# argsim/argsim

Hardware: AMD Instinct MI355X
Metric: sentences/sec per ELBO step (higher is better)
Workload: dtype f32; 1 GPU; BASELINE configs[1]: 1xMI355X fp32, latent_dim 128, vocab 8k, seq_len 64, batch 256 per GPU; FULL synthetic Zipf batches, dim_emb 512, 3 layers, step 20000; global_batch=256, seq_len=64, parallelism=dp1, gru=persistent

## Files before the change

### argsim_amd/csrc/ctx.h

```cpp
#pragma once
#include "../../include/argsim_vae.h"
#include "kernels.h"

#include <fcntl.h>
#include <sys/file.h>
#include <unistd.h>

#include <algorithm>
#include <cmath>
#include <cstdio>
#include <cstring>
#include <initializer_list>
#include <string>
#include <vector>

#pragma GCC visibility push(hidden)
namespace avae { namespace host {

struct ParamEntry {
    std::string name;
    int64_t offset;
    int ndim;
    int64_t shape[4];
    int g16;
    int bucket;
};

struct GruP { int64_t W, R, bW, bR; };

}}
#pragma GCC visibility pop

struct avae_ctx {
    avae_config cfg{};
    int device = 0;
    hipStream_t stream = nullptr;
    std::string err;
    std::vector<avae::host::ParamEntry> params;
    int64_t numel = 0;
    std::vector<std::pair<int64_t, int64_t>> buckets;
    float *P = nullptr, *G = nullptr, *M = nullptr, *Vv = nullptr;
    int64_t step = 0;
    avae_grad_hook hook = nullptr; void* hook_user = nullptr;
    std::vector<int> hook_pending;
    int persistent = 1;
    bool first_step_checked = false;
    int gru_ablate = 0, gru_force_slow = 0, gru_stagger = 0, gru_item = 2;
    int skinny = 1;
    int score_plan[4] = {0, 0, 0, 0};
    const int* expect_ptr[3] = {nullptr, nullptr, nullptr}; int expect_val[3] = {0, 0, 0};
    int compact = 2;
    int skip_pad = 1;
    int shared_device = 0; int lock_fd = -1;
    int dyn_split = 1;
    int dyn_thin = 1;
    int enc_top1 = 1;
    int table_l1 = 1;
    int bf16_act = 1;
    int bf16_sv = 1;
    int bf16_tn = 1;
    int logits16 = 1;
    int bf16_nt8 = 1;
    int bf16_direct = 0;
    int gru_spec = 2;
    int gru_ring = 1;
    int bwd_rs = 2;
    int knn_chunk = 0;
    int agg_chunk = 0;
    int ward_form = 0;
    int probe_chunk = 0;
    int tsne_chunk = 0;
    int kmeans_chunk = 0;
    int gru_bf16 = 1;
    int64_t oE = 0, oKout = 0, oBout = 0, oWmu = 0, oBmu = 0, oWlv = 0, oBlv = 0, oWex = 0, oBex = 0;
    std::vector<avae::host::GruP> enc;
    std::vector<avae::host::GruP> dec;
    float* losses = nullptr;
    float* acc = nullptr;
    int* errw = nullptr;
    unsigned* counters = nullptr;
    float* scratch = nullptr;
    int64_t scratch_n = 0;
    char* ws = nullptr; size_t ws_cap = 0;
    int B = 0, Ss = 0, St = 0;
    int timing = 0, timing_on = 0;
    unsigned short *bfA = nullptr, *bfB = nullptr; size_t bfA_cap = 0, bfB_cap = 0;
    float* slab = nullptr; size_t slab_floats = 0;
    unsigned short* bfP = nullptr; size_t bfP_cap = 0;
    struct Stamp { hipEvent_t a, b; int cls; double flops; const int* dyn; int dyn_max; };
    std::vector<Stamp> stamps; size_t stamps_used = 0;
    int32_t* hint_dev = nullptr; volatile int32_t* hint_host = nullptr;
    const int32_t *cnt_src = nullptr, *cnt_tgt = nullptr;
};

#pragma GCC visibility push(hidden)
namespace avae { namespace host {

#define AV_CHECK(expr)                                                                              \
    do { hipError_t e_ = (expr); if (e_ != hipSuccess) {                                            \
        char b_[512]; snprintf(b_, sizeof b_, "%s:%d: %s -> %s", __FILE__, __LINE__, #expr, hipGetErrorString(e_)); \
        h->err = b_; return 1; } } while (0)
#define AV_TRY(expr) do { int r_ = (expr); if (r_) return r_; } while (0)

inline int fail(avae_ctx* h, const std::string& m) { h->err = m; return 1; }
inline int check_rows(avae_ctx* h, const char* what, int dim, const char* names, std::initializer_list<const void*> ptrs)
{
    if (dim < 4 || dim > 1024 || (dim & 3)) return fail(h, std::string(what) + ": dim must be a multiple of 4 in [4, 1024]");
    uintptr_t bits = 0;
    for (const void* p : ptrs) bits |= (uintptr_t)p;
    if (bits & 15) return fail(h, std::string(what) + ": " + names + " must be 16-byte aligned");
    return 0;
}

#define AV_GRU(expr)                                                                                                \
    do { hipError_t e_ = (expr);                                                                                    \
         if (e_ == hipErrorCooperativeLaunchTooLarge)                                                               \
             return fail(h, "persistent GRU kernel: its workgroups cannot all be resident on this device at once (occupancy query x CU count < grid); " \
                            "run with avae_set_option(\"persistent\", 0)");                                         \
         if (e_ != hipSuccess) { char b_[512]; snprintf(b_, sizeof b_, "%s:%d: %s -> %s", __FILE__, __LINE__, #expr, hipGetErrorString(e_)); \
             h->err = b_; return 1; } } while (0)

struct DeviceTurn {
    avae_ctx* h; bool held = false;
    explicit DeviceTurn(avae_ctx* h_) : h(h_) {
        if (!h->shared_device || !h->persistent) return;
        if (h->lock_fd < 0) {
            char path[64]; snprintf(path, sizeof path, "/tmp/argsim_vae_dev%d.lock", h->device);
            h->lock_fd = open(path, O_CREAT | O_RDWR, 0666);
        }
        if (h->lock_fd >= 0 && flock(h->lock_fd, LOCK_EX) == 0) held = true;
    }
    ~DeviceTurn() { if (held) { (void)hipStreamSynchronize(h->stream); (void)flock(h->lock_fd, LOCK_UN); } }
};

struct Timed {
    avae_ctx* h; avae_ctx::Stamp* s = nullptr;
    Timed(avae_ctx* h_, int cls, double flops, const int* dyn = nullptr, int dyn_max = 0) : h(h_) {
        if (!h->timing) return;
        if (h->stamps_used == h->stamps.size()) {
            avae_ctx::Stamp n{};
            if (hipEventCreate(&n.a) != hipSuccess || hipEventCreate(&n.b) != hipSuccess) return;
            h->stamps.push_back(n);
        }
        s = &h->stamps[h->stamps_used++];
        s->cls = cls; s->flops = flops; s->dyn = dyn; s->dyn_max = dyn_max;
        (void)hipEventRecord(s->a, h->stream);
    }
    ~Timed() { if (s) (void)hipEventRecord(s->b, h->stream); }
};

struct Ws {
    int32_t *src_tm, *lens_src, *lens_tgt, *lead, *gold, *rank, *cidx, *ntok, *pred;
    float *emb_src, *emb_tgt, *ew, *dew;
    std::vector<float*> e_gi, e_hs, e_sv[2], e_hp[2];
    std::vector<float*> d_gi, d_hd, d_sv, d_hp;
    float *hpick, *mu, *lv, *z, *eps, *kld, *h0;
    float *xlast, *gib, *svb, *dgib, *dghb, *dxl;
    float *hc, *ho, *logits;
    float *loss_samp, *errt_samp;
    float *dho, *dhc, *dhd[2], *dgi_d, *dgh_d, *dh0, *carry, *dh0sum, *dz, *dmu, *dlv, *dhpick;
    float *dhs[2], *dgi_e, *dgh_e, *demb_src, *demb_tgt;
    std::vector<unsigned short*> e_hs16, d_hd16, e_hp16[2], d_hp16;
    std::vector<char> act_e, act_d, acth_e, acth_d;
    std::vector<unsigned short*> x16_e, x16_d;
    const unsigned short* x16_kept_e(int i) const { return x16_valid ? x16_e[i] : nullptr; }
    const unsigned short* x16_kept_d(int i) const { return x16_valid ? x16_d[i] : nullptr; }
    bool x16_valid = false;
    unsigned short *dgi16_d, *dgh16_d, *dgi16_e, *dgh16_e;
    int32_t* scat;
    int32_t *grp_src, *grp_tgt;
    int32_t *tokrow_src, *tokrow_tgt;
    float* xbuf; size_t xbuf_floats;
    int32_t *ord_perm[3], *ord_slens[3]; int ord_T[3], ord_cpj[3]; bool ord_ok[3];
    int32_t *map_src, *nact_src, *nsrc; bool compact;
    int32_t *map_tgt, *nact_tgt, *ntgt; bool compact_d;
    int Bx;
    int bx_enc() const { return compact ? Bx : 0; }
    int bx_dec() const { return compact_d ? Bx : 0; }
};

struct Bump {
    char* base; size_t off = 0;
    template <class T> T* take(size_t n) {
        off = (off + 255) & ~(size_t)255;
        T* p = base ? reinterpret_cast<T*>(base + off) : nullptr;
        off += n * sizeof(T);
        return p;
    }
    template <class T> T* opt(bool on, size_t n) { return on ? take<T>(n) : nullptr; }
};

struct Pair { const float* A; const float* B; float* C; const float* bias; };

struct GemmCall {
    const float* A; int lda; bool a_mc;
    const float* B; int ldb; bool b_nc;
    float* C; int ldc;
    int M, N, K;
    float alpha = 1.f; const float* bias = nullptr; int accumulate = 0;
    const int* dyn = nullptr; int dyn_kind = 0;
    const Pair* pair = nullptr;
    bool wgrad = false;
    bool allow_atomic = false;
    bool rows_are_batch = false;
    int thin = -1, split_k = 0;
    const unsigned short* A16 = nullptr; const unsigned short* B16 = nullptr;
    unsigned short* keep_a16 = nullptr;
    unsigned short* c16 = nullptr;

    GemmCall& scaled(float a) { alpha = a; return *this; }
    GemmCall& biased(const float* b) { bias = b; return *this; }
    GemmCall& plus() { accumulate = 1; return *this; }
    GemmCall& rows(const int* d) { dyn = d; dyn_kind = d ? 1 : 0; return *this; }
    GemmCall& depth(const int* d) { dyn = d; dyn_kind = d ? 2 : 0; return *this; }
    GemmCall& with(const Pair* p) { pair = p; return *this; }
    GemmCall& atomic() { allow_atomic = true; return *this; }
    GemmCall& batch_rows() { rows_are_batch = true; return *this; }
    GemmCall& form(int thin_, int split_k_ = 1) { thin = thin_; split_k = split_k_; return *this; }
    GemmCall& a16(const unsigned short* p) { A16 = p; return *this; }
    GemmCall& b16(const unsigned short* p) { B16 = p; return *this; }
    GemmCall& keep(unsigned short* p) { keep_a16 = p; return *this; }
};
inline GemmCall nt(const float* A, int lda, const float* B, int ldb, float* C, int ldc, int M, int N, int K) { return GemmCall{A, lda, false, B, ldb, false, C, ldc, M, N, K}; }
inline GemmCall nn(const float* A, int lda, const float* B, int ldb, float* C, int ldc, int M, int N, int K) { return GemmCall{A, lda, false, B, ldb, true, C, ldc, M, N, K}; }
inline GemmCall tn_grad(const float* A, int lda, const float* B, int ldb, float* C, int ldc, int M, int N, int K)
{
    GemmCall c{A, lda, true, B, ldb, true, C, ldc, M, N, K};
    c.wgrad = true;
    return c;
}

bool use_table(const avae_ctx* h, int rows, int B);
void layout(avae_ctx* h, Bump& b, Ws& w, int B, int Ss, int St, bool train);
int reserve_ws(avae_ctx* h, size_t need);
inline int reserve_named(avae_ctx* h, size_t need, const char* what)
{
    if (reserve_ws(h, need)) {
        (void)hipGetLastError();
        char b[256]; snprintf(b, sizeof b, "%s: the device cannot give the workspace of %zu bytes this call needs", what, need);
        h->err = b;
        return 1;
    }
    return 0;
}
int get_ws(avae_ctx* h, Ws& w, int B, int Ss, int St, bool train);
int gemm(avae_ctx* h, const GemmCall& c);
int gemm_tn16(avae_ctx* h, const GemmCall& c);
void gru_geometry(int D, int njobs, int B, int* G, int* rpg);
void gru_common(avae_ctx* h, const Ws& w, GruArgs& a, int njobs, int S, int B, int ldg, int ldh, const int32_t* lens, int Bx);
int build_row_orders(avae_ctx* h, Ws& w, int B, int Ss, int T, bool with_dec, bool with_enc = true);
int build_compact_dec(avae_ctx* h, Ws& w, int B, int T);
int run_decoder_rnn(avae_ctx* h, Ws& w, int B, int T, const float* state_in, int64_t state_stride, bool save, const int32_t* ids0 = nullptr, bool compact = false,
                    const int32_t* share_rows = nullptr, int share_n = 0);
int run_logits_ce(avae_ctx* h, Ws& w, int rt, bool train, float inv_n);
int encode_ws(avae_ctx* h, Ws& w, const int32_t* src, int b, int t);
inline PrepArgs prep_from_ws(const Ws& w)
{
    PrepArgs p{};
    p.src_tm = w.src_tm; p.lens_src = w.lens_src; p.lens_tgt = w.lens_tgt; p.lead = w.lead; p.gold = w.gold;
    p.rank = w.rank; p.cidx = w.cidx; p.ntok = w.ntok; p.chunk_counts = w.ntok + 4;
    return p;
}

int grow_scratch(avae_ctx* h, size_t need, const char* what);
int check_gru_err(avae_ctx* h);
int dyn_fraction(avae_ctx* h, const avae_ctx::Stamp& s, std::vector<std::pair<const int*, int>>& seen, double* f);
inline int check_bound(avae_ctx* h)
{
    if (!h->P || !h->G || !h->M || !h->Vv) return fail(h, "state buffers not bound (avae_bind_state)");
    return 0;
}
template <class F> int place_scratch(avae_ctx* h, const char* what, F lay)
{
    Bump probe{nullptr};
    lay(probe);
    AV_TRY(grow_scratch(h, probe.off, what));
    Bump real{reinterpret_cast<char*>(h->scratch)};
    lay(real);
    return 0;
}
template <class F> int place_ws(avae_ctx* h, const char* what, F lay, size_t from = 0)
{
    Bump probe{nullptr, from};
    lay(probe);
    AV_TRY(reserve_named(h, probe.off + 4096, what));
    Bump real{h->ws, from};
    lay(real);
    return 0;
}

bool sample_params(avae_ctx* h, const avae_sample_config* sc, int V, SampleParams* sp);
bool sample_params_p(avae_ctx* h, const avae_sample_p_config* sc, int V, SampleParams* sp, float* top_p);

}}
#pragma GCC visibility pop
```

### argsim_amd/csrc/gemm_f32.hip

```cpp
#include "kernels.h"
#include "mfma_tile.h"
#include <algorithm>
#include <cstdlib>
#include <type_traits>

namespace avae {

constexpr int BK = kTileBK, LDK = kTileLDK;

template <bool XC, int ROWS>
struct FastTile {
    const float* base; long long step, valid; unsigned voff[ROWS / 32];
    __device__ __forceinline__ void init(const float* P, int ld, int x0, int X, int kb, int ke, int tid)
    {
        if (XC) {
            base = P + (size_t)kb * ld + x0; step = (long long)BK * ld; valid = (long long)(ke - kb) * ld - x0;
#pragma unroll
            for (int rep = 0; rep < ROWS / 32; ++rep) { const int f = tid + 256 * rep; voff[rep] = (unsigned)(((f / (ROWS / 4)) * ld + ((f % (ROWS / 4)) << 2)) * 4); }
        } else {
            base = P + (size_t)x0 * ld + kb; step = BK; valid = (long long)(X - x0) * ld - kb;
#pragma unroll
            for (int rep = 0; rep < ROWS / 32; ++rep) { const int f = tid + 256 * rep; voff[rep] = (unsigned)(((f >> 3) * ld + ((f & 7) << 2)) * 4); }
        }
    }
    __device__ __forceinline__ void load(float4 (&r)[ROWS / 32], int it) const
    {
        const long long rem = valid - it * step;
        const unsigned bytes = rem <= 0 ? 0u : (rem >= (1ll << 30) ? 0xFFFFFFFFu : (unsigned)(rem * 4));
        const __amdgpu_buffer_rsrc_t rs = __builtin_amdgcn_make_buffer_rsrc(const_cast<float*>(base + it * step), 0, (int)bytes, 0x00020000);
#pragma unroll
        for (int rep = 0; rep < ROWS / 32; ++rep) {
            const u32x4 v = __builtin_amdgcn_raw_buffer_load_b128(rs, (int)voff[rep], 0, 0);
            r[rep] = make_float4(__uint_as_float(v.x), __uint_as_float(v.y), __uint_as_float(v.z), __uint_as_float(v.w));
        }
    }
};

template <int MODE>
__device__ __forceinline__ void put(float* c, float v)
{
    if (MODE == 2) atomicAdd(c, v);
    else if (MODE == 1) *c += v;
    else *c = v;
}
template <int TM, int TN, int WN, int MODE>
__device__ __forceinline__ void epilogue_full(const GemmArgs& g, const f32x16 (&acc)[TM][TN], int m0, int n0, int wm, int wn, int h, int l31, bool add_bias)
{
    float bv[TN];
#pragma unroll
    for (int j = 0; j < TN; ++j) bv[j] = add_bias ? g.bias[n0 + 32 * (wn * TN + j) + l31] : 0.f;
#pragma unroll
    for (int j = 0; j < TN; ++j) {
        const int col = n0 + 32 * (wn * TN + j) + l31;
#pragma unroll
        for (int i = 0; i < TM; ++i) {
            float* c = g.C + (size_t)(m0 + 32 * (wm * TM + i) + 4 * h) * g.ldc + col;
#pragma unroll
            for (int r = 0; r < 16; ++r)
                put<MODE>(c + (size_t)mfma32_row(r, 0) * g.ldc, g.alpha * acc[i][j][r] + bv[j]);
        }
    }
}
template <int TM, int TN, int WN>
__device__ __forceinline__ void epilogue(const GemmArgs& g, const f32x16 (&acc)[TM][TN], int M, int m0, int n0, int BM, int BN,
                                         int wm, int wn, int h, int l31, bool atomic, bool add_bias)
{
    if (!atomic && m0 + BM <= M && n0 + BN <= g.N) {
        if (g.accumulate) epilogue_full<TM, TN, WN, 1>(g, acc, m0, n0, wm, wn, h, l31, add_bias);
        else epilogue_full<TM, TN, WN, 0>(g, acc, m0, n0, wm, wn, h, l31, add_bias);
        return;
    }
    epilogue_generic<TM, TN>(acc, g.C, g.ldc, M, g.N, m0 + 32 * wm * TM, n0 + 32 * wn * TN, h, l31, g.alpha, add_bias ? g.bias : nullptr,
                             atomic ? kEpiAtomic : (g.accumulate ? kEpiAccumulate : kEpiStore));
}

template <bool A_MC, bool B_NC, int WM, int WN, int TM, int TN, bool FAST = false, bool DB = false>
__global__ __launch_bounds__(256, DB ? 2 : 3) void gemm_f32_kernel(GemmArgs g)
{
    constexpr int BM = 32 * WM * TM, BN = 32 * WN * TN;
    constexpr int kStage = (BM + BN) * LDK;
    __shared__ __attribute__((aligned(16))) float smem[kStage * (DB ? 2 : 1)];
    float* As = smem;
    float* Bs = smem + BM * LDK;

    const int tid = threadIdx.x, lane = tid & 63, wave = tid >> 6;
    const int h = lane >> 5, l31 = lane & 31;
    const int wm = wave / WN, wn = wave % WN;

    if (blockIdx.y) { g.A = g.A2; g.B = g.B2; g.C = g.C2; g.bias = g.bias2; }
    int M = g.M, K = g.K;
    if (g.dyn_kind == 1) M = min(M, *g.dyn);
    if (g.dyn_kind == 2) K = min(K, *g.dyn);

    const int tiles_n = (g.N + BN - 1) / BN;
    const int nblk = ((M + BM - 1) / BM) * tiles_n;
    const int bid = xcd_tile(blockIdx.x, nblk);
    if (bid < 0) return;
    const int tm = bid / tiles_n, tn = bid - tm * tiles_n;
    const int m0 = tm * BM, n0 = tn * BN;
    if (m0 >= M) return;

    int kb = 0, ke = K;
    if (g.split_k > 1) {
        int ktiles = (K + BK - 1) / BK;
        int per = (ktiles + g.split_k - 1) / g.split_k;
        kb = blockIdx.z * per * BK;
        ke = min(K, kb + per * BK);
        if (kb >= ke) return;
    }

    f32x16 acc[TM][TN];
    zero_acc(acc);

    float4 ra[BM / 32], rb[BN / 32];
    FastTile<A_MC, BM> fa; FastTile<B_NC, BN> fb;
    if (FAST) {
        fa.init(g.A, g.lda, m0, M, kb, ke, tid); fb.init(g.B, g.ldb, n0, g.N, kb, ke, tid);
        fa.load(ra, 0); fb.load(rb, 0);
    } else {
        load_tile<A_MC, BM>(ra, g.A, g.lda, m0, M, kb, ke, tid);
        load_tile<B_NC, BN>(rb, g.B, g.ldb, n0, g.N, kb, ke, tid);
    }

    if (DB) {
        store_tile<A_MC, BM>(As, ra, tid);
        store_tile<B_NC, BN>(Bs, rb, tid);
        __syncthreads();
    }
    for (int k0 = kb; k0 < ke; k0 += BK) {
        auto next_loads = [&]() __attribute__((always_inline)) {
            if (k0 + BK < ke) {
                if (FAST) { const int it = (k0 - kb) / BK + 1; fa.load(ra, it); fb.load(rb, it); }
                else {
                    load_tile<A_MC, BM>(ra, g.A, g.lda, m0, M, k0 + BK, ke, tid);
                    load_tile<B_NC, BN>(rb, g.B, g.ldb, n0, g.N, k0 + BK, ke, tid);
                }
            }
        };
        if (!DB) {
            store_tile<A_MC, BM>(As, ra, tid);
            store_tile<B_NC, BN>(Bs, rb, tid);
            next_loads();
            __syncthreads();
        } else next_loads();
        __builtin_amdgcn_s_setprio(1);
#pragma unroll
        for (int q = 0; q < 4; ++q) {
            float a[TM][4], b[TN][4];
#pragma unroll
            for (int t = 0; t < TM; ++t) {
                if (A_MC) {
#pragma unroll
                    for (int e = 0; e < 4; ++e) a[t][e] = As[(8 * q + 4 * h + e) * BM + 32 * (wm * TM + t) + l31];
                } else {
                    float4 v = *reinterpret_cast<const float4*>(As + (32 * (wm * TM + t) + l31) * LDK + 8 * q + 4 * h);
                    a[t][0] = v.x; a[t][1] = v.y; a[t][2] = v.z; a[t][3] = v.w;
                }
            }
#pragma unroll
            for (int t = 0; t < TN; ++t) {
                if (B_NC) {
#pragma unroll
                    for (int e = 0; e < 4; ++e) b[t][e] = Bs[(8 * q + 4 * h + e) * BN + 32 * (wn * TN + t) + l31];
                } else {
                    float4 v = *reinterpret_cast<const float4*>(Bs + (32 * (wn * TN + t) + l31) * LDK + 8 * q + 4 * h);
                    b[t][0] = v.x; b[t][1] = v.y; b[t][2] = v.z; b[t][3] = v.w;
                }
            }
#pragma unroll
            for (int e = 0; e < 4; ++e)
#pragma unroll
                for (int i = 0; i < TM; ++i)
#pragma unroll
                    for (int j = 0; j < TN; ++j)
                        acc[i][j] = __builtin_amdgcn_mfma_f32_32x32x2f32(a[i][e], b[j][e], acc[i][j], 0, 0, 0);
        }
        __builtin_amdgcn_s_setprio(0);
        if (DB) {
            As = (As == smem) ? smem + kStage : smem;
            Bs = As + BM * LDK;
            if (k0 + BK < ke) {
                store_tile<A_MC, BM>(As, ra, tid);
                store_tile<B_NC, BN>(Bs, rb, tid);
            }
        }
        __syncthreads();
    }

    const bool atomic = g.split_k > 1;
    const bool add_bias = g.bias != nullptr && (!atomic || blockIdx.z == 0);
    epilogue<TM, TN, WN>(g, acc, M, m0, n0, BM, BN, wm, wn, h, l31, atomic, add_bias);
}

template <bool A_MC, bool B_NC, bool FAST>
__global__ __launch_bounds__(256, 3) void gemm_f32_persist_kernel(GemmArgs g)
{
    static_assert(FAST, "buffer-load staging only (register budget of three workgroups per CU)");
    constexpr int TM = 2, TN = 2, WN = 2, BM = 128, BN = 128;
    __shared__ __attribute__((aligned(16))) float smem[(BM + BN) * LDK];
    float* As = smem;
    float* Bs = smem + BM * LDK;
    const int tid = threadIdx.x, lane = tid & 63, wave = tid >> 6;
    const int h = lane >> 5, l31 = lane & 31;
    const int wm = wave / WN, wn = wave % WN;

    int M = g.M;
    const int K = g.K;
    if (g.dyn_kind == 1) M = min(M, *g.dyn);
    const int tiles_n = (g.N + BN - 1) / BN;
    const int nblk = ((M + BM - 1) / BM) * tiles_n;
    const int per_xcd = gridDim.x >> 3;
    int run0, run_n;
    xcd_run(blockIdx.x & 7, nblk, run0, run_n);
    int local = blockIdx.x >> 3;
    if (local >= run_n) return;

    float4 ra[BM / 32], rb[BN / 32];
    FastTile<A_MC, BM> fa; FastTile<B_NC, BN> fb;
    auto first_tile = [&](int bid) __attribute__((always_inline)) {
        const int tm = bid / tiles_n, tn = bid - tm * tiles_n;
        if (FAST) {
            fa.init(g.A, g.lda, tm * BM, M, 0, K, tid); fb.init(g.B, g.ldb, tn * BN, g.N, 0, K, tid);
            fa.load(ra, 0); fb.load(rb, 0);
        } else {
            load_tile<A_MC, BM>(ra, g.A, g.lda, tm * BM, M, 0, K, tid);
            load_tile<B_NC, BN>(rb, g.B, g.ldb, tn * BN, g.N, 0, K, tid);
        }
    };
    first_tile(run0 + local);
    for (; local < run_n; local += per_xcd) {
        const int bid = run0 + local;
        const int tm = bid / tiles_n, tn = bid - tm * tiles_n;
        const int m0 = tm * BM, n0 = tn * BN;
        const bool more = local + per_xcd < run_n;
        f32x16 acc[TM][TN];
        zero_acc(acc);
        for (int k0 = 0; k0 < K; k0 += BK) {
            store_tile<A_MC, BM>(As, ra, tid);
            store_tile<B_NC, BN>(Bs, rb, tid);
            if (k0 + BK < K) {
                if (FAST) { const int it = k0 / BK + 1; fa.load(ra, it); fb.load(rb, it); }
                else {
                    load_tile<A_MC, BM>(ra, g.A, g.lda, m0, M, k0 + BK, K, tid);
                    load_tile<B_NC, BN>(rb, g.B, g.ldb, n0, g.N, k0 + BK, K, tid);
                }
            } else if (more) {
                first_tile(bid + per_xcd);
            }
            __syncthreads();
            __builtin_amdgcn_s_setprio(1);
            mfma_ktile<A_MC, B_NC, TM, TN, BM, BN>(acc, As, Bs, wm, wn, h, l31);
            __builtin_amdgcn_s_setprio(0);
            __syncthreads();
        }
        epilogue<TM, TN, WN>(g, acc, M, m0, n0, BM, BN, wm, wn, h, l31, false, g.bias != nullptr);
    }
}

template <bool B_NC>
__global__ __launch_bounds__(512) void gemm_f32_skinny_kernel(GemmArgs g)
{
    __shared__ float red[7][16][64];
    if (blockIdx.y) { g.A = g.A2; g.B = g.B2; g.C = g.C2; g.bias = g.bias2; }
    const int tid = threadIdx.x, lane = tid & 63, wave = tid >> 6, l31 = lane & 31, h = lane >> 5;
    const int tiles_n = (g.N + 31) / 32, tm = blockIdx.x / tiles_n, tn = blockIdx.x - tm * tiles_n;
    const int m0 = tm * 32, n0 = tn * 32;
    const int kchunk = ((g.K + 63) / 64) * 8;
    const int k0 = wave * kchunk, k1 = min(g.K, k0 + kchunk);
    const float* __restrict__ ap = g.A + (size_t)min(m0 + l31, g.M - 1) * g.lda;
    const int bcol = min(n0 + l31, g.N - 1);
    const float* __restrict__ bp = B_NC ? g.B + bcol : g.B + (size_t)bcol * g.ldb;
    f32x16 acc;
#pragma unroll
    for (int r = 0; r < 16; ++r) acc[r] = 0.f;
    for (int kk = k0; kk < k1; kk += 32) {
        float4 a[4], b[4];
#pragma unroll
        for (int u = 0; u < 4; ++u) {
            const int k = kk + 8 * u + 4 * h;
            a[u] = make_float4(0.f, 0.f, 0.f, 0.f); b[u] = make_float4(0.f, 0.f, 0.f, 0.f);
            if (k < k1) {
                a[u] = *reinterpret_cast<const float4*>(ap + k);
                if constexpr (B_NC) {
                    b[u].x = bp[(size_t)k * g.ldb]; b[u].y = bp[(size_t)(k + 1) * g.ldb]; b[u].z = bp[(size_t)(k + 2) * g.ldb]; b[u].w = bp[(size_t)(k + 3) * g.ldb];
                } else b[u] = *reinterpret_cast<const float4*>(bp + k);
            }
        }
#pragma unroll
        for (int u = 0; u < 4; ++u) {
            if (kk + 8 * u >= k1) break;
            acc = __builtin_amdgcn_mfma_f32_32x32x2f32(a[u].x, b[u].x, acc, 0, 0, 0);
            acc = __builtin_amdgcn_mfma_f32_32x32x2f32(a[u].y, b[u].y, acc, 0, 0, 0);
            acc = __builtin_amdgcn_mfma_f32_32x32x2f32(a[u].z, b[u].z, acc, 0, 0, 0);
            acc = __builtin_amdgcn_mfma_f32_32x32x2f32(a[u].w, b[u].w, acc, 0, 0, 0);
        }
    }
    if (wave > 0) {
#pragma unroll
        for (int r = 0; r < 16; ++r) red[wave - 1][r][lane] = acc[r];
    }
    __syncthreads();
    if (wave > 0) return;
    const int col = n0 + l31;
    if (col >= g.N) return;
    const float bv = g.bias ? g.bias[col] : 0.f;
#pragma unroll
    for (int r = 0; r < 16; ++r) {
        float v = acc[r];
#pragma unroll
        for (int w = 0; w < 7; ++w) v += red[w][r][lane];
        const int row = m0 + mfma32_row(r, h);
        if (row >= g.M) continue;
        float* c = g.C + (size_t)row * g.ldc + col;
        v = g.alpha * v + bv;
        if (g.accumulate) *c += v; else *c = v;
    }
}
static bool skinny_ok(bool a_mc, const GemmArgs& g)
{
    return !a_mc && g.split_k <= 1 && g.dyn_kind == 0 && (g.K & 3) == 0 && (g.lda & 3) == 0 && g.K >= 64;
}
static void launch_skinny(hipStream_t st, bool b_nc, const GemmArgs& g, const GemmF32Form& f)
{
    const dim3 grid(f.gx, f.gy, f.gz);
    if (b_nc) hipLaunchKernelGGL(gemm_f32_skinny_kernel<true>, grid, dim3(512), 0, st, g);
    else      hipLaunchKernelGGL(gemm_f32_skinny_kernel<false>, grid, dim3(512), 0, st, g);
}

template <class F>
static void with_layouts(bool a_mc, bool b_nc, F&& f)
{
    if (!a_mc && !b_nc)      f(std::false_type{}, std::false_type{});
    else if (!a_mc && b_nc)  f(std::false_type{}, std::true_type{});
    else if (a_mc && b_nc)   f(std::true_type{}, std::true_type{});
    else                     f(std::true_type{}, std::false_type{});
}

GemmF32Form gemm_f32_form(bool a_mc, bool b_nc, const GemmArgs& g)
{
    GemmF32Form f{-1, false, false, false, 0, 0, 0, hipSuccess};
    if (g.M <= 0 || g.N <= 0) return f;
    f.err = hipErrorInvalidValue;
    if ((g.lda | g.ldb) & 3) return f;
    if (((uintptr_t)g.A | (uintptr_t)g.B | (uintptr_t)g.A2 | (uintptr_t)g.B2) & 15) return f;
    if (!a_mc && (g.K & 3)) return f;
    if (a_mc && (g.M & 3)) return f;
    if (!b_nc && (g.K & 3)) return f;
    if (b_nc && (g.N & 3)) return f;
    if (g.dyn_kind == 2 && (!a_mc || !b_nc || (g.split_k > 1 && g.bias))) return f;
    f.err = hipSuccess;
    if (g.thin == 3 && skinny_ok(a_mc, g) && (b_nc || (g.ldb & 3) == 0)) {
        f.tile = 3; f.gx = ((g.M + 31) / 32) * ((g.N + 31) / 32); f.gy = g.A2 ? 2 : 1; f.gz = 1;
        return f;
    }
    f.tile = g.thin == 2 ? 2 : (g.thin ? 1 : 0);
    const int BM = f.tile == 0 ? 128 : (f.tile == 1 ? 32 : 64), BN = f.tile == 2 ? 64 : 128;
    const int tiles = ((g.M + BM - 1) / BM) * ((g.N + BN - 1) / BN);
    f.gx = tiles; f.gy = g.A2 ? 2 : 1; f.gz = g.split_k > 1 ? g.split_k : 1;
    static const bool allow_fast = !getenv("AVAE_F32_NOFAST");
    const int k_per_wg = g.split_k > 1 ? (g.K + g.split_k - 1) / g.split_k : g.K;
    f.fast = allow_fast && (a_mc ? (g.M % BM == 0) : (g.K % BK == 0 && g.dyn_kind != 2)) &&
             (b_nc ? (g.N % BN == 0) : (g.K % BK == 0 && g.dyn_kind != 2)) && (a_mc || b_nc || k_per_wg >= 1536);
    if (f.tile == 1) return f;
    static const char* ps_env = getenv("AVAE_F32_PERSIST");
    const bool aligned = (a_mc ? (g.M % BM == 0) : (g.K % BK == 0)) && (b_nc ? (g.N % BN == 0) : (g.K % BK == 0));
    const bool persist = (ps_env ? atoi(ps_env) != 0 : true) && allow_fast && aligned && !g.A2 && g.split_k <= 1 && g.dyn_kind != 2 && tiles > 1024;
    if (persist) {
        f.tile = 0; f.fast = true; f.persist = true; f.gx = 768; f.gy = f.gz = 1;
        return f;
    }
    static const char* db_env = getenv("AVAE_F32_DB");
    const int eff_tiles = (g.dyn_kind == 1 && g.dyn_expect > 0) ? std::min(tiles, ((g.dyn_expect + BM - 1) / BM) * ((g.N + BN - 1) / BN)) : (g.dyn_kind == 1 ? 0 : tiles);
    f.db = db_env ? atoi(db_env) != 0 && !g.A2 : (!g.A2 && g.split_k <= 1 && eff_tiles > 768 && tiles <= 1024);
    return f;
}

template <int WM, int WN, int TM, int TN>
static void launch_variant(hipStream_t st, bool a_mc, bool b_nc, const GemmArgs& g, const GemmF32Form& f)
{
    const dim3 grid(f.gx, f.gy, f.gz);
    if constexpr (WM == 2 && WN == 2) {
        if (f.persist) {
            with_layouts(a_mc, b_nc, [&](auto A, auto B) { hipLaunchKernelGGL((gemm_f32_persist_kernel<decltype(A)::value, decltype(B)::value, true>), grid, dim3(256), 0, st, g); });
            return;
        }
        if (f.db) {
            if (f.fast) {
                with_layouts(a_mc, b_nc, [&](auto A, auto B) { hipLaunchKernelGGL((gemm_f32_kernel<decltype(A)::value, decltype(B)::value, WM, WN, TM, TN, true, true>), grid, dim3(256), 0, st, g); });
            } else {
                with_layouts(a_mc, b_nc, [&](auto A, auto B) { hipLaunchKernelGGL((gemm_f32_kernel<decltype(A)::value, decltype(B)::value, WM, WN, TM, TN, false, true>), grid, dim3(256), 0, st, g); });
            }
            return;
        }
    }
    if (f.fast) {
        with_layouts(a_mc, b_nc, [&](auto A, auto B) { hipLaunchKernelGGL((gemm_f32_kernel<decltype(A)::value, decltype(B)::value, WM, WN, TM, TN, true>), grid, dim3(256), 0, st, g); });
        return;
    }
    with_layouts(a_mc, b_nc, [&](auto A, auto B) { hipLaunchKernelGGL((gemm_f32_kernel<decltype(A)::value, decltype(B)::value, WM, WN, TM, TN>), grid, dim3(256), 0, st, g); });
}

hipError_t gemm_f32(hipStream_t st, bool a_mc, bool b_nc, const GemmArgs& g)
{
    const GemmF32Form f = gemm_f32_form(a_mc, b_nc, g);
    if (f.err != hipSuccess) return f.err;
    if (f.tile < 0) return hipSuccess;
    if (f.tile == 3) launch_skinny(st, b_nc, g, f);
    else if (f.persist) launch_variant<2, 2, 2, 2>(st, a_mc, b_nc, g, f);
    else if (f.tile == 2) launch_variant<2, 2, 1, 1>(st, a_mc, b_nc, g, f);
    else if (f.tile == 1) launch_variant<1, 4, 1, 1>(st, a_mc, b_nc, g, f);
    else launch_variant<2, 2, 2, 2>(st, a_mc, b_nc, g, f);
    return hipGetLastError();
}

}
```

### argsim_amd/csrc/handle.cpp

```cpp
#include "ctx.h"

using namespace avae;
using namespace avae::host;

static std::string g_create_err;

namespace avae { namespace host {

int grow_scratch(avae_ctx* h, size_t need, const char* what)
{
    if (h->scratch_n >= (int64_t)need) return 0;
    AV_CHECK(hipStreamSynchronize(h->stream));
    if (h->scratch) AV_CHECK(hipFree(h->scratch));
    h->scratch = nullptr; h->scratch_n = 0;
    if (hipMalloc(reinterpret_cast<void**>(&h->scratch), need) != hipSuccess) {
        (void)hipGetLastError();
        h->scratch = nullptr;
        char b_[256]; snprintf(b_, sizeof b_, "%s: %.0f MB of scratch could not be allocated on the device", what, (double)need / 1048576.0);
        return fail(h, b_);
    }
    h->scratch_n = (int64_t)need;
    return 0;
}

static void add_param(avae_ctx* h, const std::string& name, std::initializer_list<int64_t> shape, int g16, int bucket, int64_t* off_out)
{
    ParamEntry e; e.name = name; e.offset = h->numel; e.ndim = (int)shape.size(); e.g16 = g16; e.bucket = bucket;
    int64_t n = 1; int k = 0;
    for (int i = 0; i < 4; ++i) e.shape[i] = 1;
    for (auto s : shape) { e.shape[k++] = s; n *= s; }
    if (off_out) *off_out = e.offset;
    h->numel += (n + 3) / 4 * 4;
    h->params.push_back(e);
}

static void build_params(avae_ctx* h)
{
    const int64_t D = h->cfg.dim_emb, V = h->cfg.dim_tgt, R = h->cfg.dim_rep; const int L = h->cfg.rnn_layers;
    h->enc.resize(L); h->dec.resize(L);
    auto close_bucket = [&](int64_t start) { h->buckets.push_back({start, h->numel - start}); };
    int bucket = 0; int64_t start = 0;
    add_param(h, "decode/out/kernel", {D, D}, 0, bucket, &h->oKout);
    add_param(h, "decode/out/bias", {D}, 0, bucket, &h->oBout);
    close_bucket(start);
    for (int i = L - 1; i >= 0; --i) {
        ++bucket; start = h->numel;
        std::string p = "decode/rnn/l" + std::to_string(i + 1) + "/";
        add_param(h, p + "W", {3 * D, D}, 1, bucket, &h->dec[i].W);
        add_param(h, p + "R", {3 * D, D}, 1, bucket, &h->dec[i].R);
        add_param(h, p + "bW", {3 * D}, 1, bucket, &h->dec[i].bW);
        add_param(h, p + "bR", {3 * D}, 1, bucket, &h->dec[i].bR);
        close_bucket(start);
    }
    ++bucket; start = h->numel;
    add_param(h, "latent/ex/kernel", {R, D}, 0, bucket, &h->oWex);
    add_param(h, "latent/ex/bias", {D}, 0, bucket, &h->oBex);
    add_param(h, "latent/mu/kernel", {2 * D, R}, 0, bucket, &h->oWmu);
    add_param(h, "latent/mu/bias", {R}, 0, bucket, &h->oBmu);
    add_param(h, "latent/lv/kernel", {2 * D, R}, 0, bucket, &h->oWlv);
    add_param(h, "latent/lv/bias", {R}, 0, bucket, &h->oBlv);
    close_bucket(start);
    for (int i = L - 1; i >= 0; --i) {
        ++bucket; start = h->numel;
        const int64_t In = i == 0 ? D : 2 * D;
        std::string p = "encode/rnn" + std::to_string(i + 1) + "/";
        int64_t o;
        add_param(h, p + "fwd/W", {3 * D, In}, 1, bucket, &h->enc[i].W);
        add_param(h, p + "bwd/W", {3 * D, In}, 1, bucket, &o);
        add_param(h, p + "fwd/R", {3 * D, D}, 1, bucket, &h->enc[i].R);
        add_param(h, p + "bwd/R", {3 * D, D}, 1, bucket, &o);
        add_param(h, p + "fwd/bW", {3 * D}, 1, bucket, &h->enc[i].bW);
        add_param(h, p + "bwd/bW", {3 * D}, 1, bucket, &o);
        add_param(h, p + "fwd/bR", {3 * D}, 1, bucket, &h->enc[i].bR);
        add_param(h, p + "bwd/bR", {3 * D}, 1, bucket, &o);
        close_bucket(start);
    }
    ++bucket; start = h->numel;
    add_param(h, "embed/embedding", {V, D}, 0, bucket, &h->oE);
    close_bucket(start);
}

static const ParamEntry* find_param(avae_ctx* h, const char* name)
{
    for (auto& e : h->params) if (e.name == name) return &e;
    return nullptr;
}

static float* state_buf(avae_ctx* h, int kind)
{
    switch (kind) { case AVAE_PARAM: return h->P; case AVAE_GRAD: return h->G; case AVAE_ADAM_M: return h->M; case AVAE_ADAM_V: return h->Vv; }
    return nullptr;
}

int check_gru_err(avae_ctx* h)
{
    int e = 0;
    AV_CHECK(hipMemcpyAsync(&e, h->errw, sizeof(int), hipMemcpyDeviceToHost, h->stream));
    AV_CHECK(hipStreamSynchronize(h->stream));
    if (e) {
        (void)hipMemsetAsync(h->errw, 0, sizeof(int), h->stream);
        return fail(h, "GRU persistent kernel: an exchange wait timed out -- its workgroups were not all resident at once.  A persistent "
                       "launch needs every CU of the device (one handle = one GPU = one process, include/argsim_vae.h): another process or "
                       "stream computing on this GPU holds CUs the launch is waiting for.  Give the handle the device to itself, or "
                       "run with avae_set_option(\"persistent\", 0) (one launch per time step)");
    }
    return 0;
}
int dyn_fraction(avae_ctx* h, const avae_ctx::Stamp& s, std::vector<std::pair<const int*, int>>& seen, double* f)
{
    *f = 1.0;
    if (!s.dyn || s.dyn_max <= 0) return 0;
    int c = -1;
    for (auto& e : seen) if (e.first == s.dyn) c = e.second;
    if (c < 0) {
        AV_CHECK(hipMemcpy(&c, s.dyn, sizeof(int), hipMemcpyDeviceToHost));
        if (c < 0) c = 0;
        seen.push_back({s.dyn, c});
    }
    *f = (double)std::min(c, s.dyn_max) / (double)s.dyn_max;
    return 0;
}

}}

extern "C" {

int avae_create(const avae_config* cfg, int device, avae_handle* out)
{
    if (!cfg || !out) { g_create_err = "null argument"; return 1; }
    *out = nullptr;
    if (!gru_dim_supported(cfg->dim_emb)) { g_create_err = "dim_emb must be one of 16, 32, 64, 128, 256, 512 (the GRU kernels are instantiated for these widths only; the reference leaves dim_emb free, config.json uses 512)"; return 1; }
    if (cfg->compute_dtype < 0 || cfg->compute_dtype > 2) { g_create_err = "compute_dtype must be 0 (fp32 MFMA), 1 (bf16 GEMM operands) or 2 (fp32 via split bf16 MFMA)"; return 1; }
    if (cfg->dim_rep % 4 || cfg->dim_tgt % 4 || cfg->rnn_layers < 1 || cfg->rnn_layers > 8) { g_create_err = "dim_rep and dim_tgt must be multiples of 4 (16-byte rows); 1 <= rnn_layers <= 8"; return 1; }
    int ndev = 0;
    if (hipGetDeviceCount(&ndev) != hipSuccess || ndev <= 0) { g_create_err = "no HIP device available: the gfx950 kernels cannot run (no CPU fallback)"; return 1; }
    if (device < 0 || device >= ndev) { g_create_err = "bad device index"; return 1; }
    avae_ctx* h = new avae_ctx();
    h->cfg = *cfg; h->device = device;
    if (h->cfg.kl_beta == 0.f) h->cfg.kl_beta = 1.f;
    build_params(h);
    hipError_t e = hipSetDevice(device);
    if (e == hipSuccess) e = hipMalloc(reinterpret_cast<void**>(&h->losses), 64 * sizeof(float));
    if (e == hipSuccess) e = hipMalloc(reinterpret_cast<void**>(&h->errw), 128 * sizeof(int));
    if (e == hipSuccess) e = hipMalloc(reinterpret_cast<void**>(&h->counters), 2048 * sizeof(unsigned));
    if (e == hipSuccess) e = hipMemset(h->losses, 0, 64 * sizeof(float));
    if (e == hipSuccess) e = hipMemset(h->errw, 0, 128 * sizeof(int));
    if (e == hipSuccess) e = hipMemset(h->counters, 0, 2048 * sizeof(unsigned));
    if (e != hipSuccess) { g_create_err = std::string("hip init failed: ") + hipGetErrorString(e); delete h; return 1; }
    h->acc = h->losses + 8;
    *out = h;
    return 0;
}

void avae_destroy(avae_handle h)
{
    if (!h) return;
    (void)hipSetDevice(h->device);
    if (h->stream) (void)hipStreamSynchronize(h->stream); else (void)hipDeviceSynchronize();
    if (h->ws) (void)hipFree(h->ws);
    if (h->losses) (void)hipFree(h->losses);
    if (h->errw) (void)hipFree(h->errw);
    if (h->hint_host) (void)hipHostFree(const_cast<int32_t*>(h->hint_host));
    if (h->counters) (void)hipFree(h->counters);
    if (h->scratch) (void)hipFree(h->scratch);
    if (h->bfA) (void)hipFree(h->bfA);
    if (h->slab) (void)hipFree(h->slab);
    if (h->bfP) (void)hipFree(h->bfP);
    if (h->bfB) (void)hipFree(h->bfB);
    if (h->lock_fd >= 0) (void)close(h->lock_fd);
    delete h;
}

const char* avae_last_error(avae_handle h) { return h ? h->err.c_str() : g_create_err.c_str(); }

int avae_set_stream(avae_handle h, void* s) { if (!h) return 1; h->stream = reinterpret_cast<hipStream_t>(s); return 0; }

int avae_get_dims(avae_handle h, int32_t* V, int32_t* D, int32_t* R, int32_t* L)
{
    if (!h) return 1;
    if (V) *V = h->cfg.dim_tgt; if (D) *D = h->cfg.dim_emb; if (R) *R = h->cfg.dim_rep; if (L) *L = h->cfg.rnn_layers;
    return 0;
}

int64_t avae_state_numel(avae_handle h) { return h ? h->numel : 0; }

int avae_bind_state(avae_handle h, float* p, float* g, float* m, float* v)
{
    if (!h) return 1;
    if (((uintptr_t)p | (uintptr_t)g | (uintptr_t)m | (uintptr_t)v) & 15) return fail(h, "state buffers must be 16-byte aligned");
    h->P = p; h->G = g; h->M = m; h->Vv = v;
    return 0;
}

int avae_param_count(avae_handle h) { return h ? (int)h->params.size() : 0; }
const char* avae_param_name(avae_handle h, int i) { return (h && i >= 0 && i < (int)h->params.size()) ? h->params[i].name.c_str() : nullptr; }

int avae_param_info(avae_handle h, const char* name, int64_t* offset, int32_t* ndim, int64_t shape[4])
{
    if (!h) return 1;
    const ParamEntry* e = find_param(h, name);
    if (!e) return fail(h, std::string("unknown variable: ") + (name ? name : "(null)"));
    if (offset) *offset = e->offset; if (ndim) *ndim = e->ndim;
    if (shape) for (int i = 0; i < 4; ++i) shape[i] = e->shape[i];
    return 0;
}

static int xfer_tensor(avae_handle h, const char* name, int kind, float* buf, bool get)
{
    if (!h) return 1;
    AV_TRY(check_bound(h));
    const ParamEntry* e = find_param(h, name);
    if (!e) return fail(h, std::string("unknown variable: ") + (name ? name : "(null)"));
    float* base = state_buf(h, kind);
    if (!base) return fail(h, "bad tensor kind");
    float* flat = base + e->offset;
    int64_t n = e->shape[0] * e->shape[1] * e->shape[2] * e->shape[3];
    if (!e->g16) {
        AV_CHECK(hipMemcpyAsync(get ? buf : flat, get ? flat : buf, n * sizeof(float), hipMemcpyDeviceToDevice, h->stream));
    } else {
        int D = h->cfg.dim_emb, cols = (int)(e->ndim == 2 ? e->shape[1] : 1);
        if (get) AV_CHECK(g16_permute(h->stream, buf, flat, D, cols, false));
        else     AV_CHECK(g16_permute(h->stream, flat, buf, D, cols, true));
    }
    return 0;
}
int avae_get_tensor(avae_handle h, const char* name, int kind, float* buf) { return xfer_tensor(h, name, kind, buf, true); }
int avae_set_tensor(avae_handle h, const char* name, int kind, const float* buf) { return xfer_tensor(h, name, kind, const_cast<float*>(buf), false); }

int avae_get_step(avae_handle h, int64_t* s) { if (!h || !s) return 1; *s = h->step; return 0; }
int avae_set_step(avae_handle h, int64_t s) { if (!h) return 1; h->step = s; return 0; }

int avae_set_grad_hook(avae_handle h, avae_grad_hook hook, void* user) { if (!h) return 1; h->hook = hook; h->hook_user = user; return 0; }

int avae_set_option(avae_handle h, const char* key, int value)
{
    if (!h || !key) return 1;
    if (!strcmp(key, "persistent")) { h->persistent = value; return 0; }
    if (!strcmp(key, "gru_item")) { h->gru_item = value; return 0; }
    if (!strcmp(key, "gru_stagger")) { h->gru_stagger = value; return 0; }
    if (!strcmp(key, "gru_force_slow")) { h->gru_force_slow = value; return 0; }
    if (!strcmp(key, "gru_bf16")) { h->gru_bf16 = value != 0; return 0; }
    if (!strcmp(key, "bwd_rs")) { h->bwd_rs = value; return 0; }
    if (!strcmp(key, "dyn_split")) { h->dyn_split = value != 0; return 0; }
    if (!strcmp(key, "shared_device")) { h->shared_device = value != 0; return 0; }
    if (!strcmp(key, "gru_spec")) { h->gru_spec = value; return 0; }
    if (!strcmp(key, "gru_ring")) { h->gru_ring = value != 0; return 0; }
    if (!strcmp(key, "bf16_nt8")) { h->bf16_nt8 = value != 0; return 0; }
    if (!strcmp(key, "logits16")) { h->logits16 = value != 0; return 0; }
    if (!strcmp(key, "bf16_direct")) { h->bf16_direct = value != 0; return 0; }
    if (!strcmp(key, "bf16_tn")) { h->bf16_tn = value != 0; return 0; }
    if (!strcmp(key, "bf16_sv")) { h->bf16_sv = value != 0; return 0; }
    if (!strcmp(key, "bf16_act")) { h->bf16_act = value != 0; return 0; }
    if (!strcmp(key, "table_l1")) { h->table_l1 = value != 0; return 0; }
    if (!strcmp(key, "enc_top1")) { h->enc_top1 = value != 0; return 0; }
    if (!strcmp(key, "dyn_thin")) { h->dyn_thin = value != 0; return 0; }
    if (!strcmp(key, "skip_pad")) { h->skip_pad = value != 0; return 0; }
    if (!strcmp(key, "compact")) { h->compact = value; return 0; }
    if (!strcmp(key, "skinny")) { h->skinny = value; return 0; }
    if (!strcmp(key, "knn_chunk")) { if (value < 0) return fail(h, "knn_chunk must be >= 0"); h->knn_chunk = value; return 0; }
    if (!strcmp(key, "agg_chunk")) { if (value < 0) return fail(h, "agg_chunk must be >= 0"); h->agg_chunk = value; return 0; }
    if (!strcmp(key, "ward_form")) { if (value < 0 || value > 2) return fail(h, "ward_form must be 0 (planner), 1 (one-workgroup) or 2 (launch-per-merge)"); h->ward_form = value; return 0; }
    if (!strcmp(key, "probe_chunk")) { if (value < 0) return fail(h, "probe_chunk must be >= 0"); h->probe_chunk = value; return 0; }
    if (!strcmp(key, "kmeans_chunk")) { if (value < 0) return fail(h, "kmeans_chunk must be >= 0"); h->kmeans_chunk = value; return 0; }
    if (!strcmp(key, "tsne_chunk")) { if (value < 0) return fail(h, "tsne_chunk must be >= 0"); h->tsne_chunk = value; return 0; }
    if (!strcmp(key, "gru_ablate")) {
        if (value && !gru_diag_build()) return fail(h, "gru_ablate needs the diagnostic build of libargsim_vae.so (make -C argsim_amd/csrc DIAG=1)");
        h->gru_ablate = value; return 0;
    }
    if (!strcmp(key, "timing")) { h->timing = value; h->timing_on = value; h->stamps_used = 0; return 0; }
    if (!strcmp(key, "timing_pause")) { h->timing = value ? 0 : h->timing_on; return 0; }
    return fail(h, "unknown option");
}
int avae_timing_collect(avae_handle h, double* out)
{
    if (!h || !out) return 1;
    AV_CHECK(hipStreamSynchronize(h->stream));
    for (int i = 0; i < 9; ++i) out[i] = 0.0;
    std::vector<std::pair<const int*, int>> seen;
    for (size_t i = 0; i < h->stamps_used; ++i) {
        float ms = 0.f;
        AV_CHECK(hipEventElapsedTime(&ms, h->stamps[i].a, h->stamps[i].b));
        double f = 1.0;
        AV_TRY(dyn_fraction(h, h->stamps[i], seen, &f));
        int c = h->stamps[i].cls;
        out[3 * c] += ms; out[3 * c + 1] += 1.0; out[3 * c + 2] += h->stamps[i].flops * f;
    }
    h->stamps_used = 0;
    return 0;
}
int avae_bucket_count(avae_handle h) { return h ? (int)h->buckets.size() : 0; }
int avae_bucket_info(avae_handle h, int i, int64_t* offset, int64_t* count)
{
    if (!h || i < 0 || i >= (int)h->buckets.size()) return 1;
    *offset = h->buckets[i].first; *count = h->buckets[i].second; return 0;
}

}
```

### argsim_amd/csrc/hooks.cpp

```cpp
#include "ctx.h"

using namespace avae;
using namespace avae::host;

extern "C" {

int avae_debug_team_batch(int32_t B) { return B > 0 ? gru_team_batch(B) : 0; }
int avae_debug_gemm_plan(const int32_t* in, int32_t n, int32_t* out)
{
    if (!in || !out || n < 0) return 1;
    for (int r = 0; r < n; ++r, in += 19, out += 15) {
        const GemmShape s{in[0] != 0, in[1] != 0, in[2], in[3], in[4], in[5], in[6], in[7], in[8], in[9], in[10], in[11] != 0, in[12] != 0,
                          in[13] != 0, in[14] != 0, in[15], in[16] != 0, in[17] != 0, in[18] != 0};
        const GemmPlan p = gemm_plan(s);
        out[0] = p.n;
        for (int i = 0; i < 2; ++i) {
            const GemmLaunch l = i < p.n ? p.launch[i] : GemmLaunch{0, 0, 0, 0, 0, 0, 0};
            const int32_t f[7] = {l.row0, l.rows, l.thin, l.split_k, l.accumulate, l.zero, l.dyn};
            std::copy(f, f + 7, out + 1 + 7 * i);
        }
    }
    return 0;
}
int avae_debug_gemm_call(avae_handle h, int a_mc, int b_nc, const float* A, const float* Bm, float* Cm, const float* bias, int M, int N, int K,
                         int lda, int ldb, int ldc, float alpha, int accumulate, int flags, const int* count, int expect,
                         const float* A2, const float* B2, float* C2, unsigned short* keep16)
{
    if (!h) return 1;
    GemmCall c{A, lda, a_mc != 0, Bm, ldb, b_nc != 0, Cm, ldc, M, N, K};
    c.alpha = alpha; c.bias = bias; c.accumulate = accumulate; c.keep_a16 = keep16;
    c.allow_atomic = (flags & 1) != 0; c.rows_are_batch = (flags & 2) != 0; c.wgrad = (flags & 4) != 0;
    if (c.wgrad) c.depth(count); else c.rows(count);
    const Pair second{A2, B2, C2, nullptr};
    if (A2) c.pair = &second;
    const int* const was_ptr = h->expect_ptr[0]; const int was_val = h->expect_val[0];
    h->expect_ptr[0] = count; h->expect_val[0] = expect;
    const int r = gemm(h, c);
    h->expect_ptr[0] = was_ptr; h->expect_val[0] = was_val;
    return r;
}
int avae_debug_gemm_forced(avae_handle h, int a_mc, int b_nc, const float* A, const float* Bm, float* Cm, const float* bias, int M, int N, int K,
                           int lda, int ldb, int ldc, float alpha, int accumulate, int thin, int split_k, const int* count, int dyn_kind, int expect,
                           const float* A2, const float* B2, float* C2, const float* bias2)
{
    if (!h) return 1;
    if (thin < 0 || thin > 3 || split_k < 1 || dyn_kind < 0 || dyn_kind > 2 || (dyn_kind != 0) != (count != nullptr))
        return fail(h, "avae_debug_gemm_forced: thin in 0..3, split_k >= 1, dyn_kind in 0..2 with a count exactly where it is not 0");
    GemmCall c{A, lda, a_mc != 0, Bm, ldb, b_nc != 0, Cm, ldc, M, N, K};
    c.alpha = alpha; c.bias = bias; c.accumulate = accumulate;
    if (dyn_kind == 2) c.depth(count); else c.rows(count);
    c.form(thin, split_k);
    const Pair second{A2, B2, C2, bias2};
    if (A2) c.pair = &second;
    const int* const was_ptr = h->expect_ptr[0]; const int was_val = h->expect_val[0];
    h->expect_ptr[0] = count; h->expect_val[0] = expect;
    const int r = gemm(h, c);
    h->expect_ptr[0] = was_ptr; h->expect_val[0] = was_val;
    return r;
}
int avae_debug_gemm_f32_form(int a_mc, int b_nc, int M, int N, int K, int lda, int ldb, int ldc, int accumulate, int thin, int split_k, int dyn_kind,
                             int expect, int pair, int32_t out[8])
{
    if (!out) return 1;
    alignas(16) static const float other[4] = {0.f, 0.f, 0.f, 0.f};
    const GemmArgs g{nullptr, nullptr, nullptr, nullptr, M, N, K, lda, ldb, ldc, 1.f, accumulate, split_k, nullptr, dyn_kind, expect, thin,
                     pair ? other : nullptr, pair ? other : nullptr, nullptr, nullptr};
    const GemmF32Form f = gemm_f32_form(a_mc != 0, b_nc != 0, g);
    const int32_t v[8] = {f.tile, f.fast, f.db, f.persist, (int32_t)f.gx, (int32_t)f.gy, (int32_t)f.gz, f.err != hipSuccess};
    std::copy(v, v + 8, out);
    return 0;
}
int avae_debug_score_plan(avae_handle h, int32_t out[4])
{
    if (!h || !out) return 1;
    for (int i = 0; i < 4; ++i) out[i] = h->score_plan[i];
    return 0;
}
int avae_debug_present_ids(avae_handle h, int32_t out[2])
{
    if (!h || !out) return 1;
    AV_CHECK(hipStreamSynchronize(h->stream));
    out[0] = out[1] = -1;
    if (h->cnt_src) AV_CHECK(hipMemcpy(&out[0], h->cnt_src, sizeof(int), hipMemcpyDeviceToHost));
    if (h->cnt_tgt) AV_CHECK(hipMemcpy(&out[1], h->cnt_tgt, sizeof(int), hipMemcpyDeviceToHost));
    return 0;
}
int avae_debug_train_ce(avae_handle h, float* out, int32_t max_n, int32_t* n_out)
{
    if (!h || !out || !n_out) return 1;
    if (h->B < 1) return fail(h, "avae_debug_train_ce: no training forward has run on this handle");
    Ws w;
    AV_TRY(get_ws(h, w, h->B, h->Ss, h->St, true));
    int n = 0;
    AV_CHECK(hipMemcpyAsync(&n, w.ntok, sizeof(int), hipMemcpyDeviceToHost, h->stream));
    AV_CHECK(hipStreamSynchronize(h->stream));
    n = std::min(n, (int)max_n);
    AV_CHECK(hipMemcpyAsync(out, w.loss_samp, (size_t)n * sizeof(float), hipMemcpyDeviceToDevice, h->stream));
    *n_out = n;
    return 0;
}
int avae_debug_timing(avae_handle h, double* out, int max_n, int* n)
{
    if (!h || !out || !n) return 1;
    AV_CHECK(hipStreamSynchronize(h->stream));
    *n = (int)std::min<size_t>(h->stamps_used, (size_t)max_n);
    std::vector<std::pair<const int*, int>> seen;
    for (int i = 0; i < *n; ++i) {
        float ms = 0.f;
        AV_CHECK(hipEventElapsedTime(&ms, h->stamps[i].a, h->stamps[i].b));
        double f = 1.0;
        AV_TRY(dyn_fraction(h, h->stamps[i], seen, &f));
        const double fl = h->stamps[i].flops * f;
        out[3 * i] = h->stamps[i].cls; out[3 * i + 1] = ms; out[3 * i + 2] = fl;
    }
    return 0;
}
int avae_debug_stamps(avae_handle h, unsigned long long* out)
{
    if (!h || !out) return 1;
    AV_CHECK(hipStreamSynchronize(h->stream));
    AV_CHECK(hipMemcpy(out, h->errw + 16, 32 * sizeof(unsigned long long), hipMemcpyDeviceToHost));
    AV_CHECK(hipMemset(h->errw + 16, 0, 32 * sizeof(unsigned long long)));
    return 0;
}
int avae_debug_gemm(avae_handle h, int a_mc, int b_nc, const float* A, const float* Bm, float* Cm, const float* bias,
                    int M, int N, int K, int lda, int ldb, int ldc, float alpha, int accumulate, int split_k)
{
    if (!h) return 1;
    GemmCall c{A, lda, a_mc != 0, Bm, ldb, b_nc != 0, Cm, ldc, M, N, K};
    c.alpha = alpha; c.bias = bias; c.accumulate = accumulate;
    return gemm(h, c.form(split_k == -3 ? 3 : (split_k < 0 ? 1 : (split_k >= 1000 ? 2 : 0)), split_k < 0 ? 1 : (split_k >= 1000 ? split_k - 1000 : split_k)));
}
int avae_debug_gemm_dyn(avae_handle h, const float* A, const float* Bm, float* Cm, int M, int N, int K, const int* rows)
{
    if (!h) return 1;
    return gemm(h, nt(A, K, Bm, K, Cm, N, M, N, K).rows(rows).form(0));
}
int avae_debug_gemm_c16(avae_handle h, const float* A, const float* Bm, unsigned short* C16, int M, int N, int K, float alpha, const int* rows)
{
    if (!h) return 1;
    if (h->cfg.compute_dtype != 1 || !gemm_bf16_c16_takes(M, N, K, rows, h->bf16_nt8)) return 3;
    GemmCall c = nt(A, K, Bm, K, nullptr, N, M, N, K).scaled(alpha).rows(rows).form(0);
    c.c16 = C16;
    return gemm(h, c);
}
int avae_debug_gemm_tn16(avae_handle h, const float* A, const float* Bm, float* Cm, int M, int N, int K, int lda, int ldb, int ldc, float alpha)
{
    if (!h) return 1;
    return gemm_tn16(h, tn_grad(A, lda, Bm, ldb, Cm, ldc, M, N, K).scaled(alpha));
}
int avae_debug_softmax_ce(avae_handle h, float* logits, unsigned short* panel, int logits16, const int32_t* gold, const int32_t* cidx,
                          const int32_t* n_dev, int n_max, int V, int write_grad, float inv_n, float* loss_samp, float* errt,
                          int32_t* pred, int* form_out)
{
    if (!h || !form_out) return 1;
    CeArgs c{};
    c.logits = logits; c.gold = gold; c.cidx = cidx; c.n_dev = n_dev; c.n_max = n_max; c.V = V;
    c.write_grad = write_grad; c.inv_n = inv_n;
    c.loss_samp = loss_samp; c.errt_samp = errt; c.pred = pred; c.loss_acc = nullptr;
    c.grad16 = panel; c.logits16 = logits16;
    *form_out = softmax_ce_form(c);
    AV_CHECK(softmax_ce(h->stream, c));
    return 0;
}
int avae_debug_argmax_rows(avae_handle h, const float* logits, int32_t* pred, int n, int V)
{
    if (!h) return 1;
    AV_CHECK(argmax_rows(h->stream, logits, pred, n, V));
    return 0;
}
int avae_debug_op_layout(int64_t n, int64_t V, int64_t out[6])
{
    if (!out || n < 0 || V < 0) return 1;
    int32_t base[1];
    out[0] = (int64_t)embed_scatter_scratch_ints((size_t)n, (size_t)V);
    out[1] = (int64_t)id_groups_ints((size_t)n, (size_t)V);
    out[2] = id_groups_rank(base, (int)n, (int)V) - base;
    out[3] = id_groups_uid(base, (int)n, (int)V) - base;
    out[4] = id_groups_count(base, (int)n, (int)V) - base;
    out[5] = id_groups_supported((int)V) ? 1 : 0;
    return 0;
}
int avae_debug_op(avae_handle h, const char* op, void* const* p, const int64_t* i, const float* f)
{
    if (!h || !op || !p || !i || !f) return 1;
    const std::string o(op);
    hipStream_t st = h->stream;
    auto F = [&](int k) { return static_cast<float*>(p[k]); };
    auto I = [&](int k) { return static_cast<int32_t*>(p[k]); };
    if (o == "prep_ids") {
        PrepArgs a{};
        a.src = I(0); a.tgt = I(1); a.keep_mask = static_cast<const uint8_t*>(p[2]); a.src_tm = I(3); a.lens_src = I(4); a.lens_tgt = I(5);
        a.lead = I(6); a.gold = I(7); a.rank = I(8); a.cidx = I(9); a.ntok = I(10); a.zero2 = F(11); a.chunk_counts = I(12);
        a.B = (int)i[0]; a.Ss = (int)i[1]; a.St = (int)i[2]; a.eos = (int)i[3]; a.bos = (int)i[4]; a.train = (int)i[5]; a.seed = (uint64_t)i[6];
        a.keepwd = f[0];
        AV_CHECK(prep_ids(st, a));
    } else if (o == "embed_gather") AV_CHECK(embed_gather(st, F(0), I(1), F(2), (int)i[0], (int)i[1], (int)i[2]));
    else if (o == "embed_scatter_add2") AV_CHECK(embed_scatter_add2(st, F(0), I(1), F(2), (int)i[0], I(3), F(4), (int)i[1], (int)i[2], (int)i[3], I(5)));
    else if (o == "id_groups_build") AV_CHECK(id_groups_build(st, I(0), (int)i[0], (int)i[1], I(1), i[2] != 0));
    else if (o == "rank_rows") AV_CHECK(rank_rows(st, I(0), I(1), I(2), (int)i[0], (int)i[1]));
    else if (o == "rows_gather_ranked") AV_CHECK(rows_gather_ranked(st, F(0), F(1), I(2), I(3), (int)i[0], (int)i[1], (int)i[2]));
    else if (o == "rows_group_sum") AV_CHECK(rows_group_sum(st, F(0), I(1), F(2), (int)i[0], (int)i[1], (int)i[2], I(3)));
    else if (o == "rows_add_indexed") AV_CHECK(rows_add_indexed(st, F(0), F(1), I(2), I(3), (int)i[0], (int)i[1]));
    else if (o == "rows_gather") AV_CHECK(rows_gather(st, F(0), F(1), I(2), I(3), (int)i[0], (int)i[1], I(4)));
    else if (o == "rows_expand") AV_CHECK(rows_expand(st, F(0), F(1), I(2), (int)i[0], (int)i[1], I(3)));
    else if (o == "zero_rows_dyn") AV_CHECK(zero_rows_dyn(st, F(0), I(1), (int)i[0], (int)i[1]));
    else if (o == "zero_fill") AV_CHECK(zero_fill(st, p[0], (size_t)i[0]));
    else if (o == "row_order") {
        RowOrder ro[4];
        const int n = (int)i[0];
        for (int k = 0; k < std::min(n, 4); ++k) ro[k] = RowOrder{I(3 * k), (int)i[5 + 3 * k], (int)i[6 + 3 * k], (int)i[7 + 3 * k], I(3 * k + 1), I(3 * k + 2)};
        AV_CHECK(row_order(st, ro, n, (int)i[1], (int)i[2], (int)i[3], I(3 * std::min(std::max(n, 0), 4)), (int)i[4]));
    } else if (o == "row_map") AV_CHECK(row_map(st, I(0), (int)i[0], (int)i[1], (int)i[2], I(1), I(2), I(3)));
    else if (o == "pick_last") AV_CHECK(pick_last(st, F(0), F(1), I(2), (int)i[0], (int)i[1], I(3)));
    else if (o == "pick_last16") AV_CHECK(pick_last16(st, F(0), static_cast<const unsigned short*>(p[1]), I(2), (int)i[0], (int)i[1], I(3)));
    else if (o == "pick_last_add") AV_CHECK(pick_last_add(st, F(0), F(1), I(2), (int)i[0], (int)i[1], I(3)));
    else if (o == "pick_last_bwd") AV_CHECK(pick_last_bwd(st, F(0), F(1), I(2), (int)i[0], (int)i[1], (int)i[2]));
    else if (o == "latent_fwd") AV_CHECK(latent_fwd(st, F(0), F(1), F(2), F(3), F(4), F(5), (int)i[0], (int)i[1], (uint64_t)i[2], f[0], F(6)));
    else if (o == "latent_bwd") AV_CHECK(latent_bwd(st, F(0), F(1), F(2), F(3), F(4), F(5), (int)i[0], (int)i[1], f[0], f[1]));
    else if (o == "colsum") AV_CHECK(colsum(st, F(0), (int)i[0], (int)i[1], (int)i[2], F(1), I(2)));
    else if (o == "add3") AV_CHECK(add3(st, F(0), F(1), F(2), F(3), i[0]));
    else if (o == "finalize_losses") AV_CHECK(finalize_losses(st, F(0), F(1), I(2), (int)i[0], F(3), (int)i[1], f[0], f[1], f[2]));
    else if (o == "adam_tf") {
        const AdamArgs a{F(0), F(1), F(2), F(3), i[0], f[0], f[1], f[2], f[3], static_cast<const int*>(p[4])};
        AV_CHECK(adam_tf(st, a));
    } else if (o == "g16_permute") AV_CHECK(g16_permute(st, F(0), F(1), (int)i[0], (int)i[1], i[2] != 0));
    else if (o == "gru_first_step_fwd") AV_CHECK(gru_first_step_fwd(st, F(0), F(1), F(2), (int)i[0], F(3), (int)i[1], (int)i[2], I(4)));
    else if (o == "gru_first_step_bwd") AV_CHECK(gru_first_step_bwd(st, F(0), (int)i[0], F(1), F(2), F(3), (int)i[1], (int)i[2], I(4)));
    else return fail(h, "avae_debug_op: no such launcher: " + o);
    return 0;
}

static void gru_shape(const int64_t* i, GruArgs& a)
{
    a.njobs = (int)i[0]; a.S = (int)i[1]; a.B = (int)i[2]; a.D = (int)i[3]; a.ldg = (int)i[4]; a.ldh = (int)i[5]; a.Bx = (int)i[6];
    a.G = (int)i[7]; a.rows_per_group = (int)i[8]; a.p_begin = (int)i[9]; a.p_end = (int)i[10]; a.item_pipeline = (int)i[11];
    a.bf16 = (int)i[12]; a.bwd_rs = (int)i[13]; a.xbuf_floats = (size_t)std::max<int64_t>(i[14], 0);
    if (a.G == 0 && a.D >= 16 && a.njobs >= 1 && a.B >= 1) gru_geometry(a.D, a.njobs, a.B, &a.G, &a.rows_per_group);
}
static void gru_plan_out(const GruArgs& a, const GruPlan& p, int64_t out[10])
{
    const int64_t v[10] = {(int64_t)p.form, p.T, p.C, p.cpj, p.Bg, p.pipe, a.G, a.rows_per_group, (int64_t)gru_bwd_rs_xbuf_floats(a.njobs, p.Bg), p.ring};
    std::copy(v, v + 10, out);
}
int avae_debug_gru_plan(const int64_t* i, int fwd, int persistent, int64_t out[10])
{
    if (!i || !out) return 1;
    alignas(16) static float dummy[4] = {0.f, 0.f, 0.f, 0.f};
    GruArgs a{};
    gru_shape(i, a);
    a.xbuf = a.xbuf_floats > 0 ? dummy : nullptr; a.ring = 1;
    gru_plan_out(a, gru_plan(a, fwd != 0, persistent != 0), out);
    return 0;
}
int avae_debug_gru(avae_handle h, int fwd, int persistent, const int64_t* i, void* const* jobs, void* const* shared, int64_t plan_out[10])
{
    if (!h || !i || !jobs || !shared || !plan_out) return 1;
    GruArgs a{};
    gru_shape(i, a);
    if (a.njobs < 1 || a.njobs > kMaxGruJobs) return fail(h, "avae_debug_gru: njobs in 1..3");
    if (a.p_begin != 0 || a.p_end != a.S) return fail(h, "avae_debug_gru: whole-sequence launches only (p_begin = 0, p_end = S)");
    a.stagger = (int)i[15]; a.force_slow = (int)i[16]; a.sv16 = (int)i[17]; a.spec = (int)i[18];
    for (int k = 0; k < a.njobs; ++k) {
        void* const* p = jobs + 19 * k;
        auto F = [&](int q) { return static_cast<float*>(p[q]); };
        auto H = [&](int q) { return static_cast<unsigned short*>(p[q]); };
        GruJob& j = a.job[k];
        j.gi = F(0); j.gi_rows = static_cast<const int32_t*>(p[1]); j.R = F(2); j.bR = F(3); j.h0 = F(4); j.hs = F(5); j.sv = F(6); j.hp = F(7);
        j.hs16 = H(8); j.hp16 = H(9); j.dh_out = F(10); j.dgi = F(11); j.dgh = F(12); j.dgi16 = H(13); j.dgh16 = H(14); j.dh0 = F(15);
        j.carry = F(16); j.dbW = F(17); j.dbR = F(18);
        j.reverse = (int)i[19 + 2 * k]; j.dgi_by_pos = (int)i[20 + 2 * k];
    }
    a.lens = static_cast<const int*>(shared[0]); a.slens = static_cast<const int*>(shared[1]); a.perm = static_cast<const int*>(shared[2]);
    a.rowmap = static_cast<const int*>(shared[3]); a.xbuf = static_cast<float*>(shared[4]);
    a.counters = h->counters; a.err = h->errw; a.stamps = reinterpret_cast<unsigned long long*>(h->errw + 16); a.ablate = 0;
    a.ring = h->gru_ring;
    gru_plan_out(a, gru_plan(a, fwd != 0, persistent != 0), plan_out);
    AV_CHECK(hipSetDevice(h->device));
    AV_GRU(fwd ? gru_forward(h->stream, a, persistent != 0) : gru_backward(h->stream, a, persistent != 0));
    return check_gru_err(h);
}

int avae_debug_sample_rows(avae_handle h, const float* logits, int n, int V, int t0, const avae_sample_config* sc, int32_t* pred, float* logp)
{
    if (!h) return 1;
    SampleParams sp{};
    if (!sample_params(h, sc, V, &sp)) return 1;
    if (n < 1 || V < 1 || t0 < 0 || t0 >= (1 << 20)) return fail(h, "sample rows: bad shape or step");
    AV_CHECK(sample_rows(h->stream, logits, n, V, t0, sp, nullptr, h->cfg.eos, pred, logp));
    return 0;
}

int avae_debug_sample_rows_p(avae_handle h, const float* logits, int n, int V, int t0, const avae_sample_p_config* sc, int32_t* pred, float* logp,
                             int32_t* nkept, const int32_t* lead)
{
    if (!h) return 1;
    SampleParams sp{};
    float top_p = 0.f;
    if (!sample_params_p(h, sc, V, &sp, &top_p)) return 1;
    if (n < 1 || V < 1 || t0 < 0 || t0 >= (1 << 20)) return fail(h, "sample rows: bad shape or step");
    if (top_p > 0.f) AV_CHECK(sample_rows_p(h->stream, logits, n, V, t0, sp, top_p, lead, h->cfg.eos, pred, logp, nkept));
    else {
        AV_CHECK(sample_rows(h->stream, logits, n, V, t0, sp, lead, h->cfg.eos, pred, logp));
        if (nkept) AV_CHECK(hipMemsetAsync(nkept, 0xff, (size_t)n * sizeof(int32_t), h->stream));
    }
    return 0;
}

int avae_debug_beam_select(avae_handle h, const float* logits, int n, int width, int V, const float* cum, const int32_t* fin,
                           int32_t* parent, int32_t* token, float* cum_out, int32_t* fin_out)
{
    if (!h) return 1;
    if (!logits || !cum || !fin || !parent || !token || !cum_out || !fin_out) return fail(h, "beam select: every array must be given");
    if (n < 1 || n > (1 << 20) || V < 1 || width < 1 || width > 32 || width > V) return fail(h, "beam select: bad shape or width");
    AV_CHECK(hipSetDevice(h->device));
    const size_t rows = (size_t)n * width;
    float *cand_sc, *lat_cum; int32_t *cand_tok, *cand_cnt, *len_out, *live;
    AV_TRY(place_scratch(h, "beam select", [&](Bump& b) {
        cand_sc = b.take<float>(rows * width); lat_cum = b.take<float>(rows);
        cand_tok = b.take<int32_t>(rows * width); cand_cnt = b.take<int32_t>(rows); len_out = b.take<int32_t>(rows); live = b.take<int32_t>(1);
    }));
    AV_CHECK(beam_rows(h->stream, logits, (int)rows, V, width, cum, fin, h->cfg.eos, cand_sc, cand_tok, cand_cnt));
    BeamStep a{};
    a.n = n; a.Win = width; a.W = width; a.eos = h->cfg.eos;
    a.cand_sc = cand_sc; a.cand_tok = cand_tok; a.cand_cnt = cand_cnt; a.fin_in = fin; a.len_in = nullptr;
    a.lat_parent = parent; a.lat_token = token; a.lat_cum = lat_cum; a.cum_out = cum_out; a.fin_out = fin_out; a.len_out = len_out;
    a.live = live;
    AV_CHECK(hipMemsetAsync(a.live, 0, sizeof(int32_t), h->stream));
    AV_CHECK(beam_select(h->stream, a));
    return 0;
}
int avae_debug_latent_plan(int kind, int64_t n, int64_t N, int k_or_P, int dim, int chunk_opt, int32_t out[5])
{
    if (!out || kind < 0 || kind > 2 || n < 0 || n > 0x7fffffff || N < 0 || N > 0x7fffffff) return 1;
    if (kind == 0) { const KnnPlan p = knn_plan((int)n, (int)N, k_or_P, chunk_opt); const int32_t f[5] = {p.qrows, p.qtiles, 0, p.parts, p.chunk}; std::copy(f, f + 5, out); }
    else if (kind == 1) { const AggPlan p = agg_plan((int)n, (int)N, dim, chunk_opt); const int32_t f[5] = {0, p.qtiles, 0, p.parts, p.chunk}; std::copy(f, f + 5, out); }
    else { const ProbePlan p = probe_plan((int)N, k_or_P, dim, chunk_opt); const int32_t f[5] = {p.ptiles, p.Ppad, p.LD, p.parts, p.chunk}; std::copy(f, f + 5, out); }
    return 0;
}

}
```

### argsim_amd/csrc/kernels.h

```cpp
#pragma once
#include <hip/hip_runtime.h>
#include <stdint.h>

#include "gemm_plan.h"

namespace avae {

struct GemmArgs {
    const float* A; const float* B; float* C; const float* bias;
    int M, N, K, lda, ldb, ldc;
    float alpha;
    int accumulate;
    int split_k;
    const int* dyn; int dyn_kind;
    int dyn_expect;
    int thin;
    const float* A2; const float* B2; float* C2; const float* bias2;
    float* slab = nullptr; size_t slab_floats = 0;
    unsigned short* c16 = nullptr;
    int nt8 = 1;
};
hipError_t gemm_f32(hipStream_t st, bool a_mc, bool b_nc, const GemmArgs& g);
struct GemmF32Form { int tile; bool fast, db, persist; unsigned gx, gy, gz; hipError_t err; };
GemmF32Form gemm_f32_form(bool a_mc, bool b_nc, const GemmArgs& g);
hipError_t gemm_f32s(hipStream_t st, bool a_mc, bool b_nc, const GemmArgs& g);
hipError_t gemm_bf16_direct(hipStream_t st, bool a_mc, bool b_nc, const GemmArgs& g);

hipError_t cvt_bf16(hipStream_t st, const float* src, int ld, bool transpose, int rows_or_K, int cols_or_X,
                    unsigned short* dst, int ldd);
hipError_t gemm_bf16_nt(hipStream_t st, const unsigned short* A, int lda, const unsigned short* B, int ldb, const GemmArgs& g);
bool gemm_bf16_p8_ok(const GemmArgs& g, int lda, int ldb);
hipError_t gemm_bf16_p8(hipStream_t st, const unsigned short* A, int lda, const unsigned short* B, int ldb, const GemmArgs& g, int s2);
bool gemm_bf16_c16_ok(const GemmArgs& g, int lda, int ldb);
bool gemm_bf16_c16_takes(int M, int N, int K, const int* rows, int nt8);
bool gemm_bf16_p8_tn_ok(const GemmArgs& g, int lda, int ldb);
hipError_t gemm_bf16_p8_tn(hipStream_t st, const unsigned short* A, int lda, const unsigned short* B, int ldb, const GemmArgs& g, int s2);
hipError_t gemm_bf16_tn(hipStream_t st, const unsigned short* A, int lda, const unsigned short* B, int ldb, const GemmArgs& g);
hipError_t transpose_bf16(hipStream_t st, const unsigned short* src, int ld, int K, int X, unsigned short* dst, int ldk);

constexpr int kMaxGruJobs = 3;
struct GruJob {
    const float* gi;
    const int32_t* gi_rows;
    const float* R;
    const float* bR;
    const float* h0;
    float* hs;
    float* sv;
    float* hp;
    int reverse;
    unsigned short* hs16;
    unsigned short* hp16;
    const float* dh_out;
    float* dgi;
    float* dgh;
    unsigned short* dgi16;
    unsigned short* dgh16;
    float* dh0;
    float* carry;
    int dgi_by_pos;
    float* dbW;
    float* dbR;
};
struct GruArgs {
    GruJob job[kMaxGruJobs];
    int njobs, S, B, D, ldg, ldh;
    const int* lens;
    const int* slens;
    const int* perm;
    const int* rowmap;
    int Bx;
    int G;
    int rows_per_group;
    int p_begin, p_end;
    unsigned* counters;
    int* err;
    unsigned long long* stamps;
    int item_pipeline;
    float* xbuf;
    size_t xbuf_floats;
    int stagger;
    int force_slow;
    int sv16;
    int bf16;
    int spec;
    int bwd_rs;
    int ring;
    int ablate;
};
constexpr int kGruRing = 4;
enum class GruForm { stepwise, persistent, item, team, team_rs };
struct GruPlan {
    GruForm form;
    int T, C, cpj, Bg;
    bool pipe, diag;
    int ring;
    bool team() const { return form == GruForm::team || form == GruForm::team_rs; }
    bool full() const { return team() && !diag; }
};
GruPlan gru_plan(const GruArgs& a, bool fwd, bool persistent);
hipError_t gru_forward(hipStream_t st, const GruArgs& a, bool persistent);
hipError_t gru_backward(hipStream_t st, const GruArgs& a, bool persistent);
int gru_team_batch(int B);
bool gru_dim_supported(int D);
size_t gru_bwd_rs_xbuf_floats(int njobs, int rows);
hipError_t gru_bwd_rs_launch(hipStream_t st, const GruArgs& a, const GruPlan& p);
hipError_t gru_fwd_team_launch(hipStream_t st, const GruArgs& a, const GruPlan& p);
hipError_t gru_bwd_team_launch(hipStream_t st, const GruArgs& a, const GruPlan& p);
hipError_t gru_reg_launch(hipStream_t st, const GruArgs& a, bool fwd, int grid, bool need_resident);
hipError_t gru_fwd_item_launch(hipStream_t st, const GruArgs& a, int grid);
hipError_t gru_first_step_fwd(hipStream_t st, const float* gi, const float* bR, float* h_out, int ldo, float* sv, int B, int D, const int32_t* lens = nullptr);
hipError_t gru_first_step_bwd(hipStream_t st, const float* dh, int ldd, const float* sv, float* dgi, float* dgh, int B, int D, const int32_t* lens = nullptr);
bool gru_diag_build();

struct PrepArgs {
    const int32_t* src; const int32_t* tgt;
    int B, Ss, St, eos, bos;
    int train; float keepwd; uint64_t seed; const uint8_t* keep_mask;
    int32_t* src_tm;
    int32_t* lens_src;
    int32_t* lens_tgt;
    int32_t* lead;
    int32_t* gold;
    int32_t* rank;
    int32_t* cidx;
    int32_t* ntok;
    float* zero2;
    int32_t* chunk_counts;
};
constexpr int kPrepChunks = 1024;
hipError_t prep_ids(hipStream_t st, const PrepArgs& p);

hipError_t embed_gather(hipStream_t st, const float* E, const int32_t* ids, float* out, int n, int D, int V);
hipError_t embed_scatter_add2(hipStream_t st, float* dE, const int32_t* ids0, const float* dout0, int n0, const int32_t* ids1,
                              const float* dout1, int n1, int D, int V, int32_t* scratch);
bool id_groups_supported(int V);
inline size_t id_groups_ints(size_t n, size_t V) { return 4 * V + 2 + n + (n / 32 + V + 1) + 2 * V + 4; }
hipError_t id_groups_build(hipStream_t st, const int32_t* ids, int n, int V, int32_t* scratch, bool lists);
const int32_t* id_groups_rank(int32_t* scratch, int n, int V);
const int32_t* id_groups_uid(int32_t* scratch, int n, int V);
const int32_t* id_groups_count(int32_t* scratch, int n, int V);
hipError_t rank_rows(hipStream_t st, int32_t* out, const int32_t* ids, const int32_t* rank, int n, int V);
hipError_t rows_gather_ranked(hipStream_t st, float* dst, const float* src, const int32_t* ids, const int32_t* rank, int n, int W, int V);
hipError_t rows_group_sum(hipStream_t st, float* dst, const int32_t* ids, const float* src, int n, int W, int V, int32_t* scratch);
hipError_t rows_add_indexed(hipStream_t st, float* dst, const float* src, const int32_t* uid, const int32_t* nuniq, int n_max, int D);
inline size_t embed_scatter_scratch_ints(size_t n, size_t V) { return 4 * V + 2 + n + (n / 32 + V + 1); }
struct RowOrder { const int32_t* lens; int add, T, cpj; int32_t* perm; int32_t* slens; };
hipError_t row_order(hipStream_t st, const RowOrder* orders, int n, int Breal, int B, int S, int32_t* steps_sum = nullptr, int sum_rows = 0);
hipError_t rows_gather(hipStream_t st, float* dst, const float* src, const int32_t* idx, const int32_t* n_dev, int n_max, int D, const int32_t* map = nullptr);
hipError_t rows_expand(hipStream_t st, float* dst, const float* src, const int32_t* rank, int rows, int D, const int32_t* map = nullptr);
hipError_t pick_last(hipStream_t st, float* h, const float* hs, const int32_t* lens, int B, int W, const int32_t* map = nullptr);
hipError_t pick_last16(hipStream_t st, float* h, const unsigned short* hs16, const int32_t* lens, int B, int W, const int32_t* map = nullptr);
hipError_t pick_last_add(hipStream_t st, float* dhs, const float* d, const int32_t* lens, int B, int W, const int32_t* map = nullptr);
hipError_t row_map(hipStream_t st, const int32_t* lens, int add, int S, int B, int32_t* map, int32_t* nact, int32_t* count);
hipError_t zero_rows_dyn(hipStream_t st, float* X, const int32_t* count, int rows_max, int W);
hipError_t pick_last_bwd(hipStream_t st, float* dhs, const float* dh, const int32_t* lens, int S, int B, int W);

hipError_t latent_fwd(hipStream_t st, const float* mu, const float* lv, const float* eps_in, float* eps_out, float* z,
                      float* kld, int n, int train, uint64_t seed, float free_bits, float* acc);
hipError_t latent_bwd(hipStream_t st, const float* dz, const float* mu, const float* lv, const float* eps_used,
                      float* dmu, float* dlv, int B, int R, float coef, float free_bits);

struct CeArgs {
    float* logits;
    const int32_t* gold;
    const int32_t* cidx;
    const int32_t* n_dev;
    int n_max, V;
    int write_grad; float inv_n;
    float* loss_samp; float* errt_samp; int32_t* pred;
    float* loss_acc;
    unsigned short* grad16;
    int logits16;
};
int softmax_ce_form(const CeArgs& a);
hipError_t softmax_ce(hipStream_t st, const CeArgs& a);
hipError_t argmax_rows(hipStream_t st, const float* logits, int32_t* pred, int n, int V);
struct SampleParams { float inv_t; int top_k; int noise; uint64_t seed; };
hipError_t sample_rows(hipStream_t st, const float* logits, int n, int V, int t, const SampleParams& sp, const int32_t* lead, int eos,
                       int32_t* pred, float* logp);
hipError_t sample_rows_p(hipStream_t st, const float* logits, int n, int V, int t, const SampleParams& sp, float top_p, const int32_t* lead,
                         int eos, int32_t* pred, float* logp, int32_t* nkept);

hipError_t colsum(hipStream_t st, const float* X, int M, int N, int ldx, float* out, const int32_t* m_dev);
hipError_t add3(hipStream_t st, float* out, const float* a, const float* b, const float* c, int64_t n);
hipError_t zero_fill(hipStream_t st, void* p, size_t bytes);

struct AdamArgs { float* p; const float* g; float* m; float* v; int64_t n; float lr_t, b1, b2, eps;
                  const int* skip_if; };
hipError_t adam_tf(hipStream_t st, const AdamArgs& a);

struct ScoreDraw {
    const float* mu; const float* lv;
    const float* eps_in;
    float* eps_out;
    float* z;
    float* lat;
    int* err;
    int k, B, R, rc; uint64_t seed;
};
hipError_t score_draw(hipStream_t st, const ScoreDraw& a);
hipError_t tile_ids(hipStream_t st, int32_t* dst, const int32_t* src, int n, int rc, int S);
hipError_t lead_rows(hipStream_t st, const int32_t* lead, int T, int n, int rc, int32_t* ids0, int32_t* tokrow);
struct ScoreRows {
    const float* loss;
    const int32_t* rank;
    int T, n, rc, k0, r0, B;
    float* logpx;
    int32_t* ntok;
};
hipError_t score_rows(hipStream_t st, const ScoreRows& a);
hipError_t score_bound(hipStream_t st, const float* logpx, const float* lat, int k, int B, float* logw, float* bound);

hipError_t beam_rows(hipStream_t st, const float* logits, int rows, int V, int W, const float* cum, const int32_t* fin, int eos,
                     float* cand_sc, int32_t* cand_tok, int32_t* cand_cnt);
struct BeamStep {
    int n, Win, W, eos;
    const float* cand_sc; const int32_t* cand_tok; const int32_t* cand_cnt;
    const int32_t* fin_in; const int32_t* len_in;
    int32_t* lat_parent; int32_t* lat_token; float* lat_cum;
    float* cum_out; int32_t* fin_out; int32_t* len_out;
    int32_t* live;
};
hipError_t beam_select(hipStream_t st, const BeamStep& a);
hipError_t beam_gather(hipStream_t st, const float* const* hd, int L, int n, int Win, int W, int D, const int32_t* parent, float* state_out);
struct BeamEnd {
    int n, W, n_run, steps, eos;
    const int32_t* lat_parent; const int32_t* lat_token; const float* lat_cum;
    const float* cum; const int32_t* len;
    const float* lenpow;
    int32_t* out_ids;
    float* score_out; float* cum_out; int32_t* len_out;
    int32_t* o_parent; int32_t* o_token; float* o_cum; size_t out_step;
};
hipError_t beam_backtrack(hipStream_t st, const BeamEnd& a);

struct KnnArgs {
    const float* q; const float* bank;
    int n, N, dim, k, metric;
    int64_t idx_base, self_base; int carry;
    int64_t* out_idx; float* out_score;
};
struct KnnPlan { int qrows, qtiles, parts, chunk; };
KnnPlan knn_plan(int n, int N, int k, int chunk_opt);
struct KnnWs { float *qn, *bn; unsigned long long* lists; };
hipError_t knn_search(hipStream_t st, const KnnArgs& g, const KnnPlan& p, const KnnWs& w);

struct AggArgs {
    const float* z; const float* mu; const float* lv;
    int n, N, dim;
    int64_t self_base;
    float* logq; float* logqx;
};
struct AggPlan { int qtiles, parts, chunk; };
AggPlan agg_plan(int n, int N, int dim, int chunk_opt);
hipError_t agg_logq(hipStream_t st, const AggArgs& g, const AggPlan& p, float2* parts_ms);
int moments_blocks(int N);
hipError_t latent_moments(hipStream_t st, const float* mu, const float* lv, int N, int dim, float* out, double* mean, double* part);

constexpr int kProbeTile = 32;
constexpr int kProbeAlphas = 7;
constexpr int kProbeMaxParts = 256;
struct ProbePlan { int ptiles, Ppad, LD, parts, chunk; };
ProbePlan probe_plan(int N, int P, int dim, int chunk_opt);
struct ProbeWs {
    float *sT, *z, *D, *u;
    float *W, *G, *Dv, *Rv, *Pv;
    float *gp, *lp;
    double* tp;
    int* is; float* fs; double* ds;
    int N, dim, LD, Ppad, parts, chunk;
    float *Yv, *Hd, *Hy;
    float* xs;
};
struct ProbeAlphas { int n, last; float a[kProbeAlphas]; };
hipError_t probe_prepare(hipStream_t st, const ProbeWs& b, const float* s, int P);
hipError_t probe_pass(hipStream_t st, const ProbeWs& b, const float* x, int mode);
hipError_t probe_vec(hipStream_t st, const ProbeWs& b, int P, int phase, int k, int max_newton, int max_cg, float tol, const ProbeAlphas& al);
hipError_t probe_trial(hipStream_t st, const ProbeWs& b, const ProbeAlphas& al);
hipError_t probe_finish(hipStream_t st, const ProbeWs& b, int P, float* w, float* stats);
hipError_t probe_l1_prepare(hipStream_t st, const ProbeWs& b, const float* x, const float* s, int P);
hipError_t probe_l1_curv(hipStream_t st, const ProbeWs& b);
hipError_t probe_l1_vec(hipStream_t st, const ProbeWs& b, int P, int phase, int k, int max_newton, int max_inner, float tol, const ProbeAlphas& al);
hipError_t probe_decision(hipStream_t st, const ProbePlan& p, const float* x, int n, int dim, const float* w, int P, float* W, float* out);

constexpr int kWardOneWgMax = 128;
struct WardGroup {
    int off, n, mrg, pad;
    float* D;
    double* S;
    int* cnt;
    unsigned long long* nn;
    int* st;
};
struct WardCutGroup { int off, n, mrg, m; };
hipError_t ward_init(hipStream_t st, const WardGroup* gs, int G, int nmax, const float* x, int dim);
hipError_t ward_tree(hipStream_t st, const WardGroup* gs, int G, int nmax, int dim, int32_t* pair, float* delta, int32_t* size);
hipError_t ward_round(hipStream_t st, const WardGroup* gs, int G, int nmax, int dim, int t, int32_t* pair, float* delta, int32_t* size);
hipError_t ward_cut(hipStream_t st, const WardCutGroup* gs, int G, int nmax, const int32_t* pair, int32_t* p , int32_t* label);

constexpr int kApMaxN = 1 << 14;
constexpr int kApMaxRB = 16;
struct ApState {
    int stop_at;
    int iters, conv, K;
    int cnt[2][2];
    float pref;
    unsigned prefix[2], rank[2];
    unsigned hist[512];
};
struct ApBuffers {
    float *S, *A, *R;
    double* part;
    double* cv;
    int *E, *run, *E2;
    int32_t* c;
    unsigned long long* best;
    ApState* st;
};
int ap_row_block(int N);
hipError_t ap_single(hipStream_t st, int32_t* label, int32_t* stat);
hipError_t ap_similarity(hipStream_t st, const float* x, int N, int dim, int metric, float* S);
hipError_t ap_prepare(hipStream_t st, float* S, int N, int use_pref, float pref, int noise, uint64_t seed, ApState* state);
hipError_t ap_iteration(hipStream_t st, const ApBuffers& b, int N, float lam, int it, int conv_iter);
hipError_t ap_labels(hipStream_t st, const ApBuffers& b, int N, int32_t* label, int32_t* stat);

constexpr int kTsneMaxN = 1 << 14;
constexpr int kTsneMaxChunk = 4096;
struct TsneState {
    int stop_at;
    int phase, best_iter;
    int last_it, how, p1_last;
    int pad[2];
    double best_error, last_err, p1_err;
};
struct TsnePlan { int rs, parts, chunk; };
struct TsneArgs {
    const double* P;
    float *y, *upd, *gains;
    float* grad;
    double* trace;
    double *part, *errp;
    TsneState* st;
    int N, rs, parts, chunk;
    int max_iter, X, exag_iter, nic, nwp;
    float lr; double ee, min_gn;
};
TsnePlan tsne_plan(int N, int chunk_opt);
hipError_t tsne_conditionals(hipStream_t st, const float* S , int N, double perplexity, double* C, double* beta);
hipError_t tsne_joint(hipStream_t st, double* P , int N, double* rowsum );
hipError_t tsne_init(hipStream_t st, const TsneArgs& a, int it0, int warm, int init, uint64_t seed, const double* prog);
hipError_t tsne_iteration(hipStream_t st, const TsneArgs& a, int it);
hipError_t tsne_finish(hipStream_t st, const TsneArgs& a, double* kl, int32_t* stat, double* prog);

constexpr int kKmMaxN = 1 << 22;
constexpr int kKmMaxK = 4096, kKmMaxInit = 64, kKmMaxParts = 16, kKmMaxBlocks = 256, kKmMaxTrials = 10;
constexpr int kKmTile = 64;
constexpr int kKmScanRows = 1024;
struct KmState {
    int stop_at;
    int how, reloc;
    int changed, nempty;
    int chosen;
    int pad[2];
    double tol_abs, total;
};
struct KmPlan { int tile, tiles, parts, chunk, slice, slices, blk, blks, scan, scans; };
struct KmArgs {
    const float* x; const double* rnorm;
    int N, dim, k, R, max_iter, T;
    uint64_t seed;
    KmPlan p;
    KmState* st;
    double* C;
    double* pd; int* pi;
    int* lab; double* dist;
    int *hist, *off;
    int* start;
    int* order;
    double* psum;
    int* rel;
    double *shiftp, *ipart;
    double *vpart, *mean;
    int* best;
    double *closest, *D, *candC, *tsum, *ppart;
    int* cand;
};
KmPlan km_plan(int N, int k, int R, int chunk_opt);
hipError_t km_prepare(hipStream_t st, const KmArgs& a, double tol);
hipError_t km_load(hipStream_t st, const KmArgs& a, const float* centers_in);
hipError_t km_seed(hipStream_t st, const KmArgs& a);
hipError_t km_iteration(hipStream_t st, const KmArgs& a, int it);
hipError_t km_finish(hipStream_t st, const KmArgs& a, int32_t* label, float* centers, int32_t* stat, double* inertia, int32_t* label_all,
                     double* centers_all, int32_t* stat_all);

struct DecodeArgs {
    const float* E;
    const float *W[8], *R[8], *bW[8], *bR[8];
    const float *Kout, *bout;
    float* state[2];
    float* o;
    float* part_val; int32_t* part_idx;
    int32_t* ids_tm;
    int32_t* out_ids;
    int32_t* kept;
    unsigned* bar;
    int* err;
    int b, steps, D, V, L, eos, cache_e; float isd;
    SampleParams sp;
    float *part_x, *part_m, *part_s;
    float* logits;
    float* logp_tm;
    float* logp_out;
    float top_p;
    int32_t* nkept_tm;
    int32_t* nkept_out;
};
hipError_t decode_greedy(hipStream_t st, DecodeArgs a, int* grid_out);
hipError_t decode_sample(hipStream_t st, DecodeArgs a, int* grid_out);
int decode_workgroups();

hipError_t g16_permute(hipStream_t st, float* dst, const float* src, int D, int cols, bool to_g16);

hipError_t finalize_losses(hipStream_t st, float* losses, const float* loss_samp, const int32_t* n_dev, int n_max,
                           const float* kld, int nk, float free_bits, float inv_br, float anneal);

}
```

### argsim_amd/csrc/model.cpp

```cpp
#include "ctx.h"

using namespace avae;

namespace avae { namespace host {

static bool phantom_batch(const avae_ctx* h, int B)
{
    return h->compact && h->skip_pad && h->persistent && h->cfg.dim_emb == 512 && gru_team_batch(B) > B;
}
bool use_table(const avae_ctx* h, int rows, int B)
{
    if (!h->table_l1 || !id_groups_supported(h->cfg.dim_tgt)) return false;
    return rows >= h->cfg.dim_tgt || (rows >= 1024 && phantom_batch(h, B));
}

void layout(avae_ctx* h, Bump& b, Ws& w, int B, int Ss, int St, bool train)
{
    const int D = h->cfg.dim_emb, V = h->cfg.dim_tgt, R = h->cfg.dim_rep, L = h->cfg.rnn_layers;
    const size_t T = St + 1, rs = (size_t)Ss * B, rt = T * B;
    w.src_tm = b.take<int32_t>(rs); w.lens_src = b.take<int32_t>(B); w.lens_tgt = b.take<int32_t>(B);
    w.lead = b.take<int32_t>(rt); w.gold = b.take<int32_t>(rt); w.rank = b.take<int32_t>(rt);
    w.cidx = b.take<int32_t>(rt); w.ntok = b.take<int32_t>(4 + kPrepChunks); w.pred = b.take<int32_t>(rt);
    w.emb_src = b.take<float>(rs * D); w.emb_tgt = b.take<float>(rt * D);
    const bool tab_s = use_table(h, (int)rs, B), tab_t = use_table(h, (int)rt, B);
    w.ew = b.take<float>(tab_s ? (size_t)V * 6 * D : (tab_t ? (size_t)V * 3 * D : 0));
    w.grp_src = b.take<int32_t>(tab_s ? id_groups_ints(rs, V) : 0); w.grp_tgt = b.take<int32_t>(tab_t ? id_groups_ints(rt, V) : 0);
    w.tokrow_src = b.take<int32_t>(tab_s ? rs : 0); w.tokrow_tgt = b.take<int32_t>(tab_t ? rt : 0);
    w.e_gi.resize(L); w.e_hs.resize(L);
    for (int d = 0; d < 2; ++d) { w.e_sv[d].resize(L); w.e_hp[d].resize(L); }
    w.d_gi.resize(L); w.d_hd.resize(L); w.d_sv.resize(L); w.d_hp.resize(L);
    w.e_hs16.assign(L, nullptr); w.d_hd16.assign(L, nullptr); w.e_hp16[0].assign(L, nullptr); w.e_hp16[1].assign(L, nullptr); w.d_hp16.assign(L, nullptr);
    w.act_e.assign(L, 0); w.act_d.assign(L, 0); w.acth_e.assign(L, 0); w.acth_d.assign(L, 0);
    if (train && h->cfg.compute_dtype == 1 && h->bf16_act && h->bf16_tn && D % 8 == 0)
        for (int i = 0; i < L; ++i) {
            w.e_hs16[i] = b.take<unsigned short>(rs * 2 * D); w.e_hp16[0][i] = b.take<unsigned short>(rs * D); w.e_hp16[1][i] = b.take<unsigned short>(rs * D);
            if (i < L - 1) w.d_hd16[i] = b.take<unsigned short>(rt * D);
            w.d_hp16[i] = b.take<unsigned short>(rt * D);
        }
    w.x16_e.assign(L, nullptr); w.x16_d.assign(L, nullptr);
    w.x16_valid = train && h->cfg.compute_dtype == 1 && h->bf16_tn && !h->bf16_direct && D % 8 == 0;
    if (w.x16_valid)
        for (int i = 1; i < L; ++i) { w.x16_e[i] = b.take<unsigned short>(rs * 2 * D); w.x16_d[i] = b.take<unsigned short>(rt * D); }
    for (int i = 0; i < L; ++i) {
        w.e_gi[i] = b.take<float>(rs * 6 * D);
        w.e_hs[i] = b.take<float>(rs * 2 * D);
        for (int d = 0; d < 2; ++d) {
            w.e_sv[d][i] = train ? b.take<float>(rs * 4 * D) : nullptr;
            w.e_hp[d][i] = train ? b.take<float>(rs * D) : nullptr;
        }
    }
    for (int i = 0; i < L; ++i) {
        w.d_gi[i] = b.take<float>(rt * 3 * D);
        w.d_hd[i] = b.take<float>(rt * D);
        w.d_sv[i] = train ? b.take<float>(rt * 4 * D) : nullptr;
        w.d_hp[i] = train ? b.take<float>(rt * D) : nullptr;
    }
    {
        const int bx = gru_team_batch(B);
        w.Bx = bx > 0 ? bx : B;
        const size_t rows = std::max<size_t>(2 * Ss, T) * (size_t)w.Bx;
        w.xbuf_floats = rows * D * (train ? 3 : 1);
        if (train && D == 512 && h->bwd_rs) w.xbuf_floats = std::max(w.xbuf_floats, gru_bwd_rs_xbuf_floats(2, w.Bx));
        w.xbuf = b.take<float>(w.xbuf_floats);
    }
    w.map_src = b.take<int32_t>(rs); w.nact_src = b.take<int32_t>(Ss + 1); w.nsrc = b.take<int32_t>(4); w.compact = false;
    w.map_tgt = b.take<int32_t>(rt); w.nact_tgt = b.take<int32_t>(T + 1); w.ntgt = b.take<int32_t>(4); w.compact_d = false;
    for (int k = 0; k < 3; ++k) { w.ord_perm[k] = b.take<int32_t>(w.Bx); w.ord_slens[k] = b.take<int32_t>(w.Bx); w.ord_ok[k] = false; w.ord_T[k] = w.ord_cpj[k] = 0; }
    w.hpick = b.take<float>((size_t)B * 2 * D);
    w.xlast = b.take<float>((size_t)B * 2 * D); w.gib = b.take<float>((size_t)B * 3 * D); w.svb = b.take<float>((size_t)B * 4 * D);
    w.dgib = b.take<float>(train ? (size_t)B * 3 * D : 0); w.dghb = b.take<float>(train ? (size_t)B * 3 * D : 0); w.dxl = b.take<float>(train ? (size_t)B * 2 * D : 0);
    w.mu = b.take<float>((size_t)B * R); w.lv = b.take<float>((size_t)B * R); w.z = b.take<float>((size_t)B * R);
    w.eps = b.take<float>((size_t)B * R); w.kld = b.take<float>((size_t)B * R);
    w.h0 = b.take<float>((size_t)B * D);
    w.hc = b.take<float>(rt * D); w.ho = b.take<float>(rt * D); w.logits = b.take<float>(rt * V);
    w.loss_samp = b.take<float>(rt); w.errt_samp = b.take<float>(rt);
    if (train) {
        w.dho = b.take<float>(rt * D); w.dhc = b.take<float>(rt * D);
        w.dhd[0] = b.take<float>(rt * D); w.dhd[1] = b.take<float>(rt * D);
        w.dgi_d = b.take<float>(rt * 3 * D); w.dgh_d = b.take<float>(rt * 3 * D);
        w.dh0 = b.take<float>((size_t)L * B * D); w.carry = b.take<float>((size_t)3 * w.Bx * D);
        w.dh0sum = b.take<float>((size_t)B * D);
        w.dz = b.take<float>((size_t)B * R); w.dmu = b.take<float>((size_t)B * R); w.dlv = b.take<float>((size_t)B * R);
        w.dhpick = b.take<float>((size_t)B * 2 * D);
        w.dhs[0] = b.take<float>(rs * 2 * D); w.dhs[1] = b.take<float>(rs * 2 * D);
        w.dgi_e = b.take<float>(rs * 6 * D); w.dgh_e = b.take<float>(rs * 6 * D);
        w.demb_src = b.take<float>(rs * D); w.demb_tgt = b.take<float>(rt * D);
        const bool g16 = h->cfg.compute_dtype == 1;
        w.dgi16_d = b.take<unsigned short>(g16 ? rt * 3 * D : 0); w.dgh16_d = b.take<unsigned short>(g16 ? rt * 3 * D : 0);
        w.dgi16_e = b.take<unsigned short>(g16 ? rs * 6 * D : 0); w.dgh16_e = b.take<unsigned short>(g16 ? rs * 6 * D : 0);
        w.scat = b.take<int32_t>(embed_scatter_scratch_ints(rs + rt, V));
        w.dew = b.take<float>(tab_s ? (size_t)V * 6 * D : (tab_t ? (size_t)V * 3 * D : 0));
    }
}

int reserve_ws(avae_ctx* h, size_t need)
{
    if (need > h->ws_cap) {
        AV_CHECK(hipStreamSynchronize(h->stream));
        if (h->ws) AV_CHECK(hipFree(h->ws));
        h->ws = nullptr; h->ws_cap = 0;
        h->cnt_src = h->cnt_tgt = nullptr;
        for (auto& sp : h->stamps) sp.dyn = nullptr;
        size_t cap = need + need / 8;
        AV_CHECK(hipMalloc(reinterpret_cast<void**>(&h->ws), cap));
        h->ws_cap = cap;
    }
    return 0;
}

int get_ws(avae_ctx* h, Ws& w, int B, int Ss, int St, bool train)
{
    return place_ws(h, "step", [&](Bump& b) { layout(h, b, w, B, Ss, St, train); });
}

static int grow_bf16(avae_ctx* h, unsigned short** buf, size_t* cap, size_t need)
{
    if (need <= *cap) return 0;
    AV_CHECK(hipStreamSynchronize(h->stream));
    if (*buf) AV_CHECK(hipFree(*buf));
    *buf = nullptr; *cap = 0;
    size_t n = need + need / 8;
    AV_CHECK(hipMalloc(reinterpret_cast<void**>(buf), n * sizeof(unsigned short)));
    *cap = n;
    return 0;
}

static int dyn_expected(const avae_ctx* h, const int* dyn, int dyn_kind)
{
    if (dyn_kind != 1 || !dyn) return 0;
    for (int i = 0; i < 3; ++i) if (dyn == h->expect_ptr[i]) return h->expect_val[i];
    return 0;
}

static GemmShape gemm_shape(const avae_ctx* h, const GemmCall& c)
{
    return GemmShape{c.a_mc, c.b_nc, c.M, c.N, c.K, c.ldc, c.accumulate, c.split_k, c.thin, c.dyn_kind, dyn_expected(h, c.dyn, c.dyn_kind),
                     c.allow_atomic, c.rows_are_batch, c.pair != nullptr, c.wgrad, h->cfg.compute_dtype, h->skinny != 0, h->dyn_split != 0, h->dyn_thin != 0};
}
static GemmLaunch bf16_launch(const avae_ctx* h, const GemmCall& c)
{
    if (!c.wgrad) return GemmLaunch{0, c.M, 0, 1, c.accumulate, kZeroNone, c.dyn_kind ? 1 : 0};
    GemmShape s = gemm_shape(h, c);
    s.compute_dtype = 1;
    return gemm_plan(s).launch[0];
}

static int gemm_launch(avae_ctx* h, const GemmCall& c, const GemmLaunch& l)
{
    if (c.pair && h->cfg.compute_dtype != 0) {
        GemmCall one = c, two = c;
        one.pair = two.pair = nullptr; two.keep_a16 = nullptr;
        two.A = c.pair->A; two.B = c.pair->B; two.C = c.pair->C; two.bias = c.pair->bias;
        AV_TRY(gemm_launch(h, one, l));
        return gemm_launch(h, two, l);
    }
    const float* A = c.A + (size_t)l.row0 * c.lda; float* C = c.C + (size_t)l.row0 * c.ldc;
    const int M = l.rows, N = c.N, K = c.K;
    const int* dyn = l.dyn ? c.dyn : nullptr; const int dyn_kind = l.dyn ? c.dyn_kind : 0;
    const Pair* pair = c.pair;
    GemmArgs g{A, c.B, C, c.bias, M, N, K, c.lda, c.ldb, c.ldc, c.alpha, l.accumulate, l.split_k, dyn, dyn_kind, dyn_expected(h, dyn, dyn_kind), l.thin,
               pair ? pair->A : nullptr, pair ? pair->B : nullptr, pair ? pair->C : nullptr, pair ? pair->bias : nullptr};
    Timed t(h, 0, 2.0 * M * N * K * (pair ? 2 : 1), dyn, dyn_kind == 1 ? M : (dyn_kind == 2 ? K : 0));
    if (h->cfg.compute_dtype == 1 && h->bf16_direct) {
        AV_CHECK(gemm_bf16_direct(h->stream, c.a_mc, c.b_nc, g));
        return 0;
    }
    if (h->cfg.compute_dtype == 1) {
        const int Kp = (K + 7) & ~7;
        unsigned short* a16 = nullptr;
        if (c.keep_a16 && !c.a_mc && Kp == K) a16 = c.keep_a16 + (size_t)l.row0 * K;
        if (!a16) { AV_TRY(grow_bf16(h, &h->bfA, &h->bfA_cap, (size_t)M * Kp)); a16 = h->bfA; }
        AV_TRY(grow_bf16(h, &h->bfB, &h->bfB_cap, (size_t)N * Kp));
        AV_CHECK(cvt_bf16(h->stream, A, c.lda, c.a_mc, c.a_mc ? K : M, c.a_mc ? M : K, a16, Kp));
        AV_CHECK(cvt_bf16(h->stream, c.B, c.ldb, c.b_nc, c.b_nc ? K : N, c.b_nc ? N : K, h->bfB, Kp));
        g.nt8 = h->bf16_nt8;
        g.c16 = c.c16;
        AV_CHECK(gemm_bf16_nt(h->stream, a16, Kp, h->bfB, Kp, g));
        return 0;
    }
    if (c.c16) return fail(h, "the fp16 output panel exists in compute_dtype 1 only");
    if (h->cfg.compute_dtype == 2 && !l.thin) AV_CHECK(gemm_f32s(h->stream, c.a_mc, c.b_nc, g));
    else AV_CHECK(gemm_f32(h->stream, c.a_mc, c.b_nc, g));
    return 0;
}

int gemm(avae_ctx* h, const GemmCall& c)
{
    const GemmPlan p = gemm_plan(gemm_shape(h, c));
    for (int i = 0; i < p.n; ++i) {
        const GemmLaunch& l = p.launch[i];
        float* C = c.C + (size_t)l.row0 * c.ldc;
        if (l.zero == kZeroAll) AV_CHECK(zero_fill(h->stream, C, sizeof(float) * (size_t)l.rows * c.N));
        if (l.zero == kZeroDynRows) AV_CHECK(zero_rows_dyn(h->stream, C, c.dyn, l.rows, c.N));
        AV_TRY(gemm_launch(h, c, l));
    }
    return 0;
}

static int gemm_bf16_pre(avae_ctx* h, const GemmCall& c)
{
    const GemmLaunch l = bf16_launch(h, c);
    const int M = c.M, N = c.N, K = c.K;
    GemmArgs g{nullptr, c.B, c.C, c.bias, M, N, K, c.lda, c.ldb, c.ldc, c.alpha, l.accumulate, l.split_k, c.dyn, c.dyn_kind, 0, 0, nullptr, nullptr, nullptr, nullptr};
    Timed t(h, 0, 2.0 * M * N * K, c.dyn, c.dyn_kind == 1 ? M : (c.dyn_kind == 2 ? K : 0));
    const int Kp = (K + 7) & ~7;
    const unsigned short* Ap = c.A16; int lda_p = c.lda;
    if (c.a_mc) {
        AV_TRY(grow_bf16(h, &h->bfA, &h->bfA_cap, (size_t)M * Kp));
        AV_CHECK(transpose_bf16(h->stream, c.A16, c.lda, K, M, h->bfA, Kp));
        Ap = h->bfA; lda_p = Kp;
    }
    AV_TRY(grow_bf16(h, &h->bfB, &h->bfB_cap, (size_t)N * Kp));
    AV_CHECK(cvt_bf16(h->stream, c.B, c.ldb, c.b_nc, c.b_nc ? K : N, c.b_nc ? N : K, h->bfB, Kp));
    g.nt8 = h->bf16_nt8;
    AV_CHECK(gemm_bf16_nt(h->stream, Ap, lda_p, h->bfB, Kp, g));
    return 0;
}

int gemm_tn16(avae_ctx* h, const GemmCall& c)
{
    const GemmLaunch l = bf16_launch(h, c);
    const int M = c.M, N = c.N, K = c.K;
    GemmArgs g{nullptr, nullptr, c.C, nullptr, M, N, K, c.lda, c.ldb, c.ldc, c.alpha, l.accumulate, l.split_k, c.dyn, c.dyn_kind, 0, 0, nullptr, nullptr, nullptr, nullptr};
    Timed t(h, 0, 2.0 * M * N * K, c.dyn, c.dyn ? K : 0);
    const unsigned short* A16 = c.A16; const unsigned short* B16 = c.B16;
    int la = c.lda, lb = c.ldb;
    if (!A16) {
        la = (M + 7) & ~7;
        AV_TRY(grow_bf16(h, &h->bfA, &h->bfA_cap, (size_t)K * la));
        AV_CHECK(cvt_bf16(h->stream, c.A, c.lda, false, K, M, h->bfA, la));
        A16 = h->bfA;
    }
    if (!B16) {
        lb = (N + 7) & ~7;
        AV_TRY(grow_bf16(h, &h->bfB, &h->bfB_cap, (size_t)K * lb));
        AV_CHECK(cvt_bf16(h->stream, c.B, c.ldb, false, K, N, h->bfB, lb));
        B16 = h->bfB;
    }
    g.nt8 = h->bf16_nt8;
    if (h->bf16_nt8 && l.split_k > 1) {
        if (!h->slab) {
            const size_t n = (size_t)512 << 16;
            AV_CHECK(hipMalloc(reinterpret_cast<void**>(&h->slab), n * sizeof(float)));
            h->slab_floats = n;
        }
        g.slab = h->slab; g.slab_floats = h->slab_floats;
    }
    AV_CHECK(gemm_bf16_tn(h->stream, A16, la, B16, lb, g));
    return 0;
}
static bool tn16_ok(const avae_ctx* h, int M, int N) { return h->cfg.compute_dtype == 1 && h->bf16_tn && gemm_tn16_shape(M, N); }

void gru_geometry(int D, int njobs, int B, int* G, int* rpg)
{
    int HT = D / 16;
    int gmax = 512 / (njobs * HT); if (gmax < 1) gmax = 1; if (gmax > 16) gmax = 16;
    int g = (B + 15) / 16; if (g > gmax) g = gmax; if (g < 1) g = 1;
    int r = (B + g - 1) / g; r = (r + 15) / 16 * 16;
    g = (B + r - 1) / r;
    *G = g; *rpg = r;
}

struct Sched { float keepwd, anneal, lr; };
static Sched schedule(const avae_ctx* h)
{
    float rate = h->cfg.accelerate * (float)h->step;
    Sched s;
    s.keepwd = 1.f / (1.f + expf(-rate));
    s.anneal = tanhf(rate);
    s.lr = h->cfg.learn_rate / (sqrtf(rate) + 1.f);
    return s;
}

static bool top_one_step(const avae_ctx* h) { return h->enc_top1 && h->cfg.rnn_layers >= 2; }

struct FillHint { int32_t real, rows; };
static FillHint fill_hint(const avae_ctx* h)
{
    const uint64_t pair = h->hint_host ? *reinterpret_cast<const volatile uint64_t*>(h->hint_host) : 0xffffffffull;
    return {(int32_t)(uint32_t)(pair & 0xffffffffull), (int32_t)(uint32_t)(pair >> 32)};
}
static double expected_fill(const avae_ctx* h)
{
    const FillHint f = fill_hint(h);
    return (f.real > 0 && f.rows > 0) ? std::min(1.0, (double)f.real / (double)f.rows) : 1.0;
}
static int rs_pick(const avae_ctx* h)
{
    if (h->bwd_rs != 2) return h->bwd_rs;
    return expected_fill(h) < 0.40 ? 1 : 0;
}
static int spec_pick(const avae_ctx* h)
{
    if (h->gru_spec != 2) return h->gru_spec;
    return expected_fill(h) < 0.60 ? 1 : 0;
}

void gru_common(avae_ctx* h, const Ws& w, GruArgs& a, int njobs, int S, int B, int ldg, int ldh, const int32_t* lens, int Bx)
{
    const int D = h->cfg.dim_emb;
    a.njobs = njobs; a.S = S; a.B = B; a.D = D; a.ldg = ldg; a.ldh = ldh; a.lens = lens;
    a.Bx = Bx;
    gru_geometry(D, njobs, B, &a.G, &a.rows_per_group);
    a.p_begin = 0; a.p_end = S; a.counters = h->counters; a.err = h->errw; a.ablate = h->gru_ablate; a.force_slow = h->gru_force_slow;
    a.bf16 = h->cfg.compute_dtype == 1 && h->gru_bf16; a.stagger = h->gru_stagger; a.item_pipeline = h->gru_item;
    a.xbuf = w.xbuf; a.xbuf_floats = w.xbuf_floats; a.stamps = reinterpret_cast<unsigned long long*>(h->errw + 16); a.bwd_rs = h->bwd_rs != 0;
    a.ring = h->gru_ring;
}
int build_row_orders(avae_ctx* h, Ws& w, int B, int Ss, int T, bool with_dec, bool with_enc)
{
    if (!h->skip_pad || !h->persistent || w.Bx % 16) return 0;
    if (w.Bx != B && !h->compact) return 0;
    const int D = h->cfg.dim_emb;
    RowOrder ord[3]; int n = 0, which[3];
    auto want = [&](int k, int njobs, int S, int ldg, int ldh, const int32_t* lens, int add) {
        GruArgs a{};
        gru_common(h, w, a, njobs, S, B, ldg, ldh, lens, w.Bx);
        const GruPlan p = gru_plan(a, true, true);
        if (p.form != GruForm::team) return;
        ord[n] = RowOrder{lens, add, p.T, p.cpj, w.ord_perm[k], w.ord_slens[k]};
        which[n++] = k; w.ord_T[k] = p.T; w.ord_cpj[k] = p.cpj;
    };
    if (with_enc) want(0, 2, Ss, 6 * D, 2 * D, w.lens_src, 0);
    if (with_enc && top_one_step(h)) want(1, 1, Ss, 6 * D, 2 * D, w.lens_src, 0);
    if (with_dec) want(2, 1, T, 3 * D, D, w.lens_tgt, 1);
    if (!n) return 0;
    const bool hint = which[0] == 0 && h->compact == 2;
    if (hint && !h->hint_host) {
        int32_t* hp = nullptr;
        if (hipHostMalloc(reinterpret_cast<void**>(&hp), 64, hipHostMallocDefault) == hipSuccess) { hp[0] = -1; hp[1] = 0; h->hint_host = hp; }
    }
    h->hint_dev = reinterpret_cast<int32_t*>(h->errw + 100);
    hipError_t e = row_order(h->stream, ord, n, B, w.Bx, std::max(Ss, T), hint ? h->hint_dev : nullptr, Ss * B);
    if (e == hipErrorInvalidValue) return 0;
    AV_CHECK(e);
    if (hint && h->hint_host) {
        AV_CHECK(hipMemcpyAsync(const_cast<int32_t*>(h->hint_host), h->hint_dev, 2 * sizeof(int32_t), hipMemcpyDeviceToHost, h->stream));
    }
    for (int i = 0; i < n; ++i) w.ord_ok[which[i]] = true;
    return 0;
}
static bool both_team_bf16(avae_ctx* h, const GruArgs& a, bool train)
{
    return train && a.bf16 && gru_plan(a, true, h->persistent != 0).full() && gru_plan(a, false, h->persistent != 0).full();
}
static void attach_sv16(avae_ctx* h, GruArgs& a, bool train) { a.sv16 = h->bf16_sv && both_team_bf16(h, a, train); }
static void attach_order(avae_ctx* h, const Ws& w, GruArgs& a, bool fwd, int k)
{
    const GruPlan p = gru_plan(a, fwd, h->persistent != 0);
    if (!w.ord_ok[k] || !p.team() || p.T != w.ord_T[k] || p.cpj != w.ord_cpj[k]) return;
    a.slens = w.ord_slens[k]; a.perm = w.ord_perm[k];
}

static int build_compact(avae_ctx* h, Ws& w, int B, int Ss, int T, bool train)
{
    w.compact = false; w.compact_d = false;
    h->expect_ptr[0] = h->expect_ptr[1] = h->expect_ptr[2] = nullptr;
    if (!h->compact || !h->persistent || Ss < 2 || !use_table(h, Ss * B, B)) return 0;
    const bool phantom = w.Bx != B;
    if (phantom && !(w.ord_ok[0] && (w.ord_ok[1] || !top_one_step(h)))) return 0;
    if (h->compact == 2 && !phantom) {
        const FillHint f = fill_hint(h);
        if (f.real < 0 || f.rows <= 0 || (double)f.real >= 0.92 * (double)f.rows) return 0;
    }
    const int D = h->cfg.dim_emb;
    auto team = [&](int njobs, int S, int ldg, int ldh, const int32_t* lens) {
        GruArgs q{};
        gru_common(h, w, q, njobs, S, B, ldg, ldh, lens, w.Bx);
        return gru_plan(q, true, true).full() && (!train || gru_plan(q, false, true).full());
    };
    if (!team(2, Ss, 6 * D, 2 * D, w.lens_src) || (top_one_step(h) && !team(1, Ss, 6 * D, 2 * D, w.lens_src))) return 0;
    AV_CHECK(row_map(h->stream, w.lens_src, 0, Ss, B, w.map_src, w.nact_src, w.nsrc));
    w.compact = true;
    {
        const FillHint f = fill_hint(h);
        const double fill = (f.real > 0 && f.rows > 0) ? std::min(1.0, (double)f.real / (double)f.rows) : 0.0;
        h->expect_ptr[0] = w.nsrc; h->expect_val[0] = (int)(fill * Ss * B);
        h->expect_ptr[1] = w.ntgt; h->expect_val[1] = (int)(fill * T * B);
        h->expect_ptr[2] = w.ntok; h->expect_val[2] = (int)(fill * T * B);
    }
    if (T < 2 || !use_table(h, T * B, B) || h->compact == 3) return 0;
    if ((phantom && !w.ord_ok[2]) || !team(1, T, 3 * D, D, nullptr)) return 0;
    AV_CHECK(row_map(h->stream, w.lens_tgt, 1, T, B, w.map_tgt, w.nact_tgt, w.ntgt));
    w.compact_d = true;
    return 0;
}
int build_compact_dec(avae_ctx* h, Ws& w, int B, int T)
{
    w.compact = false; w.compact_d = false;
    h->expect_ptr[0] = h->expect_ptr[1] = h->expect_ptr[2] = nullptr;
    if (!h->compact || h->compact == 3 || !h->persistent || T < 2 || !use_table(h, T * B, B)) return 0;
    if (w.Bx == B || !w.ord_ok[2]) return 0;
    GruArgs q{};
    gru_common(h, w, q, 1, T, B, 3 * h->cfg.dim_emb, h->cfg.dim_emb, nullptr, w.Bx);
    if (!gru_plan(q, true, true).full()) return 0;
    AV_CHECK(row_map(h->stream, w.lens_tgt, 1, T, B, w.map_tgt, w.nact_tgt, w.ntgt));
    w.compact_d = true;
    return 0;
}

static int run_encoder(avae_ctx* h, Ws& w, int B, int Ss, bool save)
{
    const int D = h->cfg.dim_emb, V = h->cfg.dim_tgt, L = h->cfg.rnn_layers;
    const int rs = Ss * B;
    const bool table = use_table(h, rs, B);
    h->cnt_src = table ? id_groups_count(w.grp_src, rs, V) : nullptr;
    const int32_t* const cdyn = w.compact ? w.nsrc : nullptr;
    const int32_t* const cmap = w.compact ? w.map_src : nullptr;
    if (!table) AV_CHECK(embed_gather(h->stream, h->P + h->oE, w.src_tm, w.emb_src, rs, D, V));
    const float* x = w.emb_src; int In = D;
    for (int i = 0; i < L; ++i) {
        const GruP& p = h->enc[i];
        const bool top1 = i == L - 1 && top_one_step(h);
        if (i == 0 && table) {
            const int32_t* cnt = id_groups_count(w.grp_src, rs, V);
            AV_CHECK(id_groups_build(h->stream, w.src_tm, rs, V, w.grp_src, save));
            AV_CHECK(rows_gather(h->stream, w.emb_src, h->P + h->oE, id_groups_uid(w.grp_src, rs, V), cnt, std::min(V, rs), D));
            AV_TRY(gemm(h, nt(w.emb_src, D, h->P + p.W, D, w.ew, 6 * D, std::min(V, rs), 6 * D, D).biased(h->P + p.bW).rows(cnt)));
        } else if (i > 0 && w.act_e[i - 1]) {
            AV_TRY(gemm_bf16_pre(h, nt(nullptr, In, h->P + p.W, In, w.e_gi[i], 6 * D, rs, top1 ? 3 * D : 6 * D, In).a16(w.e_hs16[i - 1]).biased(h->P + p.bW).rows(cdyn)));
        } else {
        AV_TRY(gemm(h, nt(x, In, h->P + p.W, In, w.e_gi[i], 6 * D, rs, top1 ? 3 * D : 6 * D, In).biased(h->P + p.bW).rows(cdyn).keep(save ? w.x16_e[i] : nullptr)));
        }
        GruArgs a{};
        gru_common(h, w, a, top1 ? 1 : 2, Ss, B, 6 * D, 2 * D, w.lens_src, w.bx_enc());
        const bool table0 = i == 0 && table, indirect = table0 && gru_plan(a, true, h->persistent != 0).form == GruForm::team;
        if (indirect) AV_CHECK(rank_rows(h->stream, w.tokrow_src, w.src_tm, id_groups_rank(w.grp_src, rs, V), rs, V));
        else if (table0) AV_CHECK(rows_gather_ranked(h->stream, w.e_gi[0], w.ew, w.src_tm, id_groups_rank(w.grp_src, rs, V), rs, 6 * D, V));
        for (int d = 0; d < a.njobs; ++d) {
            GruJob& j = a.job[d];
            j.gi = (indirect ? w.ew : w.e_gi[i]) + d * 3 * D;
            j.gi_rows = indirect ? w.tokrow_src : nullptr;
            j.R = h->P + p.R + (int64_t)d * 3 * D * D;
            j.bR = h->P + p.bR + d * 3 * D;
            j.h0 = nullptr;
            j.hs = w.e_hs[i] + d * D;
            j.sv = save ? w.e_sv[d][i] : nullptr;
            j.hp = save ? w.e_hp[d][i] : nullptr;
            j.reverse = d;
        }
        attach_sv16(h, a, save);
        if (w.e_hs16[i] && tn16_ok(h, 3 * D, D) && both_team_bf16(h, a, save)) {
            w.act_e[i] = 1; w.acth_e[i] = 1;
            for (int d = 0; d < a.njobs; ++d) { a.job[d].hs16 = w.e_hs16[i] + d * D; a.job[d].hp16 = w.e_hp16[d][i]; }
        }
        attach_order(h, w, a, true, top1 ? 1 : 0);
        a.rowmap = cmap;
        a.spec = spec_pick(h);
        { Timed t(h, 1, 2.0 * a.njobs * Ss * (double)B * D * 3 * D);
          DeviceTurn turn(h);
          AV_GRU(gru_forward(h->stream, a, h->persistent != 0)); }
        if (top1) {
            const int64_t oWb = p.W + (int64_t)3 * D * In;
            if (w.act_e[i - 1]) AV_CHECK(pick_last16(h->stream, w.xlast, w.e_hs16[i - 1], w.lens_src, B, In, cmap));
            else
            AV_CHECK(pick_last(h->stream, w.xlast, x, w.lens_src, B, In, cmap));
            AV_TRY(gemm(h, nt(w.xlast, In, h->P + oWb, In, w.gib, 3 * D, B, 3 * D, In).biased(h->P + p.bW + 3 * D).batch_rows()));
        }
        x = w.e_hs[i]; In = 2 * D;
    }
    if (w.act_e[L - 1]) AV_CHECK(pick_last16(h->stream, w.hpick, w.e_hs16[L - 1], w.lens_src, B, 2 * D, cmap));
    else
    AV_CHECK(pick_last(h->stream, w.hpick, w.e_hs[L - 1], w.lens_src, B, 2 * D, cmap));
    if (top_one_step(h))
        AV_CHECK(gru_first_step_fwd(h->stream, w.gib, h->P + h->enc[L - 1].bR + 3 * D, w.hpick + D, 2 * D, save ? w.svb : nullptr, B, D, w.lens_src));
    return 0;
}

static int run_latent(avae_ctx* h, Ws& w, int B, bool train, uint64_t seed, const float* eps)
{
    const int D = h->cfg.dim_emb, R = h->cfg.dim_rep;
    {
        const Pair lv{w.hpick, h->P + h->oWlv, w.lv, h->P + h->oBlv};
        AV_TRY(gemm(h, nn(w.hpick, 2 * D, h->P + h->oWmu, R, w.mu, R, B, R, 2 * D).biased(h->P + h->oBmu).with(&lv)));
    }
    AV_CHECK(latent_fwd(h->stream, w.mu, w.lv, eps, w.eps, w.z, w.kld, B * R, train ? 1 : 0, seed, h->cfg.free_bits, nullptr));
    return 0;
}

int run_decoder_rnn(avae_ctx* h, Ws& w, int B, int T, const float* state_in, int64_t state_stride, bool save, const int32_t* ids0, bool compact, const int32_t* share_rows, int share_n)
{
    const int32_t* const cdyn = compact ? w.ntgt : nullptr;
    const int32_t* const cmap = compact ? w.map_tgt : nullptr;
    const int D = h->cfg.dim_emb, L = h->cfg.rnn_layers;
    const int rt = T * B;
    const float* x = w.emb_tgt;
    h->cnt_tgt = ids0 ? id_groups_count(w.grp_tgt, rt, h->cfg.dim_tgt) : nullptr;
    for (int i = 0; i < L; ++i) {
        const GruP& p = h->dec[i];
        if (i == 0 && ids0) {
            const int V = h->cfg.dim_tgt;
            const int32_t* cnt = id_groups_count(w.grp_tgt, rt, V);
            AV_CHECK(id_groups_build(h->stream, ids0, rt, V, w.grp_tgt, save));
            AV_CHECK(rows_gather(h->stream, w.emb_tgt, h->P + h->oE, id_groups_uid(w.grp_tgt, rt, V), cnt, std::min(V, rt), D));
            AV_TRY(gemm(h, nt(w.emb_tgt, D, h->P + p.W, D, w.ew, 3 * D, std::min(V, rt), 3 * D, D).biased(h->P + p.bW).rows(cnt)));
        } else if (i == 0 && share_rows) {
            AV_TRY(gemm(h, nt(x, D, h->P + p.W, D, w.d_gi[0], 3 * D, share_n, 3 * D, D).biased(h->P + p.bW)));
        } else if (i > 0 && w.act_d[i - 1]) {
            AV_TRY(gemm_bf16_pre(h, nt(nullptr, D, h->P + p.W, D, w.d_gi[i], 3 * D, rt, 3 * D, D).a16(w.d_hd16[i - 1]).biased(h->P + p.bW).rows(cdyn)));
        } else {
        AV_TRY(gemm(h, nt(x, D, h->P + p.W, D, w.d_gi[i], 3 * D, rt, 3 * D, D).biased(h->P + p.bW).rows(cdyn).keep(save ? w.x16_d[i] : nullptr)));
        }
        GruArgs a{};
        gru_common(h, w, a, 1, T, B, 3 * D, D, nullptr, compact ? w.Bx : 0);
        GruJob& j = a.job[0];
        const bool table0 = i == 0 && ids0, indirect = table0 && gru_plan(a, true, h->persistent != 0).form == GruForm::team;
        if (indirect) AV_CHECK(rank_rows(h->stream, w.tokrow_tgt, ids0, id_groups_rank(w.grp_tgt, rt, h->cfg.dim_tgt), rt, h->cfg.dim_tgt));
        else if (table0) AV_CHECK(rows_gather_ranked(h->stream, w.d_gi[0], w.ew, ids0, id_groups_rank(w.grp_tgt, rt, h->cfg.dim_tgt), rt, 3 * D, h->cfg.dim_tgt));
        j.gi = indirect ? w.ew : w.d_gi[i]; j.gi_rows = indirect ? w.tokrow_tgt : nullptr;
        if (i == 0 && share_rows) j.gi_rows = share_rows;
        j.R = h->P + p.R; j.bR = h->P + p.bR;
        j.h0 = state_in + state_stride * i;
        j.hs = w.d_hd[i];
        j.sv = save ? w.d_sv[i] : nullptr;
        j.hp = save ? w.d_hp[i] : nullptr;
        j.reverse = 0;
        attach_sv16(h, a, save);
        if (w.d_hp16[i] && tn16_ok(h, 3 * D, D) && both_team_bf16(h, a, save)) {
            if (i < L - 1) { w.act_d[i] = 1; j.hs16 = w.d_hd16[i]; }
            w.acth_d[i] = 1; j.hp16 = w.d_hp16[i];
        }
        if (T > 1) attach_order(h, w, a, true, 2);
        a.rowmap = cmap;
        a.spec = spec_pick(h);
        { Timed t(h, 1, 2.0 * T * (double)B * D * 3 * D);
          DeviceTurn turn(h);
          AV_GRU(gru_forward(h->stream, a, h->persistent != 0)); }
        x = w.d_hd[i];
    }
    return 0;
}

static int forward(avae_ctx* h, Ws& w, const int32_t* src, const int32_t* tgt, int B, int Ss, int St, bool train,
            uint64_t seed, const uint8_t* keep_mask, const float* eps, float inv_n)
{
    const int D = h->cfg.dim_emb, V = h->cfg.dim_tgt, R = h->cfg.dim_rep;
    const int T = St + 1, rt = T * B;
    Sched sc = schedule(h);
    PrepArgs p = prep_from_ws(w);
    p.src = src; p.tgt = tgt; p.B = B; p.Ss = Ss; p.St = St; p.eos = h->cfg.eos; p.bos = h->cfg.bos;
    p.train = train ? 1 : 0; p.keepwd = sc.keepwd; p.seed = seed; p.keep_mask = keep_mask;
    AV_CHECK(prep_ids(h->stream, p));
    AV_TRY(build_row_orders(h, w, B, Ss, T, true));
    AV_TRY(build_compact(h, w, B, Ss, T, train));
    AV_TRY(run_encoder(h, w, B, Ss, train));
    AV_TRY(run_latent(h, w, B, train, seed, eps));
    AV_TRY(gemm(h, nn(w.z, R, h->P + h->oWex, D, w.h0, D, B, D, R).biased(h->P + h->oBex).batch_rows()));
    if (use_table(h, rt, B)) AV_TRY(run_decoder_rnn(h, w, B, T, w.h0, 0, train, w.lead, w.compact_d));
    else {
        AV_CHECK(embed_gather(h->stream, h->P + h->oE, w.lead, w.emb_tgt, rt, D, V));
        AV_TRY(run_decoder_rnn(h, w, B, T, w.h0, 0, train));
    }
    AV_TRY(run_logits_ce(h, w, rt, train, inv_n));
    float beta = h->cfg.kl_beta;
    AV_CHECK(finalize_losses(h->stream, h->losses, w.loss_samp, w.ntok, rt, w.kld, B * R, h->cfg.free_bits, 1.f / ((float)B * R), sc.anneal * beta));
    return 0;
}

int run_logits_ce(avae_ctx* h, Ws& w, int rt, bool train, float inv_n)
{
    const int D = h->cfg.dim_emb, V = h->cfg.dim_tgt, L = h->cfg.rnn_layers;
    AV_CHECK(rows_gather(h->stream, w.hc, w.d_hd[L - 1], w.cidx, w.ntok, rt, D, w.compact_d ? w.map_tgt : nullptr));
    AV_TRY(gemm(h, nn(w.hc, D, h->P + h->oKout, D, w.ho, D, rt, D, D).biased(h->P + h->oBout).rows(w.ntok)));
    CeArgs c{};
    c.logits = w.logits; c.gold = w.gold; c.cidx = w.cidx; c.n_dev = w.ntok; c.n_max = rt; c.V = V;
    c.write_grad = train ? 1 : 0; c.inv_n = inv_n;
    if (train && h->cfg.compute_dtype == 1 && (V & 7) == 0) {
        AV_TRY(grow_bf16(h, &h->bfP, &h->bfP_cap, (size_t)rt * V));
        c.grad16 = h->bfP;
        if (h->logits16 && !h->bf16_direct && gemm_bf16_c16_takes(rt, V, D, w.ntok, h->bf16_nt8)) c.logits16 = 1;
    }
    GemmCall lg = nt(w.ho, D, h->P + h->oE, D, w.logits, V, rt, V, D).scaled(1.f / sqrtf((float)D)).rows(w.ntok);
    if (c.logits16) lg.form(0).c16 = h->bfP;
    AV_TRY(gemm(h, lg));
    c.loss_samp = w.loss_samp; c.errt_samp = w.errt_samp; c.pred = w.pred; c.loss_acc = nullptr;
    AV_CHECK(softmax_ce(h->stream, c));
    return 0;
}

static void fire_hook(avae_ctx* h, int bucket)
{
    if (h->hook && bucket >= 0 && bucket < (int)h->buckets.size()) h->hook_pending.push_back(bucket);
}
static void hook_fence(avae_ctx* h)
{
    if (h->hook) h->hook(h->hook_user, AVAE_HOOK_FENCE, 0, 0);
}
static void hook_flush(avae_ctx* h)
{
    for (int b : h->hook_pending) h->hook(h->hook_user, b, h->buckets[b].first, h->buckets[b].second);
    h->hook_pending.clear();
}

static int backward(avae_ctx* h, Ws& w, int B, int Ss, int St, float b_global)
{
    const int D = h->cfg.dim_emb, V = h->cfg.dim_tgt, R = h->cfg.dim_rep, L = h->cfg.rnn_layers;
    const int T = St + 1, rt = T * B, rs = Ss * B;
    const float isd = 1.f / sqrtf((float)D);
    Sched sc = schedule(h);
    hipStream_t st = h->stream;
    float* G = h->G; const float* P = h->P;
    h->hook_pending.clear();
    AV_CHECK(zero_fill(st, G, sizeof(float) * h->numel));

    if (h->cfg.compute_dtype == 1 && (V & 7) == 0) {
        AV_TRY(gemm_bf16_pre(h, nn(nullptr, V, P + h->oE, D, w.dho, D, rt, D, V).a16(h->bfP).scaled(isd).rows(w.ntok)));
        const GemmCall dE = tn_grad(nullptr, V, w.ho, D, G + h->oE, D, V, D, rt).a16(h->bfP).scaled(isd).depth(w.ntok);
        AV_TRY(tn16_ok(h, V, D) ? gemm_tn16(h, dE) : gemm_bf16_pre(h, dE));
    } else {
    AV_TRY(gemm(h, nn(w.logits, V, P + h->oE, D, w.dho, D, rt, D, V).scaled(isd).rows(w.ntok).atomic()));
    AV_TRY(gemm(h, tn_grad(w.logits, V, w.ho, D, G + h->oE, D, V, D, rt).scaled(isd).depth(w.ntok)));
    }
    AV_TRY(gemm(h, tn_grad(w.hc, D, w.dho, D, G + h->oKout, D, D, D, rt).depth(w.ntok)));
    AV_CHECK(colsum(st, w.dho, rt, D, D, G + h->oBout, w.ntok));
    AV_TRY(gemm(h, nt(w.dho, D, P + h->oKout, D, w.dhc, D, rt, D, D).rows(w.ntok).atomic()));
    fire_hook(h, 0);
    const int32_t* const ddyn = w.compact_d ? w.ntgt : nullptr;
    const int32_t* const dmap = w.compact_d ? w.map_tgt : nullptr;
    AV_CHECK(rows_expand(st, w.dhd[0], w.dhc, w.rank, rt, D, dmap));

    int cur = 0;
    for (int i = L - 1; i >= 0; --i) {
        const GruP& p = h->dec[i];
        GruArgs a{};
        gru_common(h, w, a, 1, T, B, 3 * D, D, nullptr, w.bx_dec());
        GruJob& j = a.job[0];
        j.R = P + p.R; j.sv = w.d_sv[i]; j.hp = w.d_hp[i]; j.reverse = 0;
        j.dh_out = w.dhd[cur]; j.dgi = w.dgi_d; j.dgh = w.dgh_d;
        j.dh0 = w.dh0 + (size_t)i * B * D; j.carry = w.carry;
        j.dbW = G + p.bW; j.dbR = G + p.bR;
        const bool team16 = tn16_ok(h, 3 * D, D) && a.bf16 && gru_plan(a, false, h->persistent != 0).full();
        const bool g16 = team16 && !(i == 0 && use_table(h, rt, B));
        const bool gh16 = !g16 && w.dgh16_d && team16 && w.acth_d[i];
        if (g16) { j.dgi16 = w.dgi16_d; j.dgh16 = w.dgh16_d; }
        if (gh16) j.dgh16 = w.dgh16_d;
        if (!g16 && !gh16 && w.acth_d[i]) return fail(h, "internal: the forward kept this layer's h_prev as bf16 only and the backward cannot read it");
        if (w.acth_d[i]) j.hp16 = w.d_hp16[i];
        attach_sv16(h, a, true);
        attach_order(h, w, a, false, 2);
        a.rowmap = dmap;
        if (dmap && i == 0) j.dgi_by_pos = 1;
        a.bwd_rs = rs_pick(h); a.spec = spec_pick(h);
        hook_fence(h);
        { Timed t(h, 2, 2.0 * T * (double)B * D * 3 * D);
          DeviceTurn turn(h);
          AV_GRU(gru_backward(st, a, h->persistent != 0)); }
        hook_flush(h);
        if (i == 0 && use_table(h, rt, B)) {
            const int32_t* cnt = id_groups_count(w.grp_tgt, rt, V); const int U = std::min(V, rt);
            AV_CHECK(rows_group_sum(st, w.dew, w.lead, w.dgi_d, rt, 3 * D, V, w.grp_tgt));
            AV_TRY(gemm(h, tn_grad(w.dew, 3 * D, w.emb_tgt, D, G + p.W, D, 3 * D, D, U).depth(cnt)));
            if (gh16) AV_TRY(gemm_tn16(h, tn_grad(nullptr, 3 * D, nullptr, D, G + p.R, D, 3 * D, D, rt).a16(w.dgh16_d).b16(w.d_hp16[i]).depth(ddyn)));
            else
            AV_TRY(gemm(h, tn_grad(w.dgh_d, 3 * D, w.d_hp[i], D, G + p.R, D, 3 * D, D, rt).depth(ddyn)));
            AV_TRY(gemm(h, nn(w.dew, 3 * D, P + p.W, D, w.demb_tgt, D, U, D, 3 * D).rows(cnt).atomic()));
            AV_CHECK(rows_add_indexed(st, G + h->oE, w.demb_tgt, id_groups_uid(w.grp_tgt, rt, V), cnt, U, D));
        } else if (g16) {
            const float* x = i == 0 ? w.emb_tgt : w.d_hd[i - 1];
            AV_TRY(gemm_tn16(h, tn_grad(nullptr, 3 * D, x, D, G + p.W, D, 3 * D, D, rt).a16(w.dgi16_d).b16((i > 0 && w.act_d[i - 1]) ? w.d_hd16[i - 1] : w.x16_kept_d(i)).depth(ddyn)));
            AV_TRY(gemm_tn16(h, tn_grad(nullptr, 3 * D, w.d_hp[i], D, G + p.R, D, 3 * D, D, rt).a16(w.dgh16_d).b16(w.acth_d[i] ? w.d_hp16[i] : nullptr).depth(ddyn)));
            float* dx = i == 0 ? w.demb_tgt : w.dhd[cur ^ 1];
            AV_TRY(gemm_bf16_pre(h, nn(nullptr, 3 * D, P + p.W, D, dx, D, rt, D, 3 * D).a16(w.dgi16_d).rows(ddyn)));
        } else {
        const float* x = i == 0 ? w.emb_tgt : w.d_hd[i - 1];
        {
            const Pair dR{w.dgh_d, w.d_hp[i], G + p.R, nullptr};
            AV_TRY(gemm(h, tn_grad(w.dgi_d, 3 * D, x, D, G + p.W, D, 3 * D, D, rt).depth(ddyn).with(&dR)));
        }
        float* dx = i == 0 ? w.demb_tgt : w.dhd[cur ^ 1];
        AV_TRY(gemm(h, nn(w.dgi_d, 3 * D, P + p.W, D, dx, D, rt, D, 3 * D).rows(ddyn).atomic()));
        }
        cur ^= 1;
        fire_hook(h, 1 + (L - 1 - i));
    }

    AV_CHECK(add3(st, w.dh0sum, w.dh0, L > 1 ? w.dh0 + (size_t)B * D : nullptr, L > 2 ? w.dh0 + (size_t)2 * B * D : nullptr, (int64_t)B * D));
    for (int i = 3; i < L; ++i) AV_CHECK(add3(st, w.dh0sum, w.dh0sum, w.dh0 + (size_t)i * B * D, nullptr, (int64_t)B * D));
    AV_TRY(gemm(h, tn_grad(w.z, R, w.dh0sum, D, G + h->oWex, D, R, D, B)));
    AV_CHECK(colsum(st, w.dh0sum, B, D, D, G + h->oBex, nullptr));
    AV_TRY(gemm(h, nt(w.dh0sum, D, P + h->oWex, D, w.dz, R, B, R, D)));
    float bg = b_global > 0.f ? b_global : (float)B;
    AV_CHECK(latent_bwd(st, w.dz, w.mu, w.lv, w.eps, w.dmu, w.dlv, B, R, sc.anneal * h->cfg.kl_beta / (bg * R), h->cfg.free_bits));
    {
        const Pair dlv{w.hpick, w.dlv, G + h->oWlv, nullptr};
        AV_TRY(gemm(h, tn_grad(w.hpick, 2 * D, w.dmu, R, G + h->oWmu, R, 2 * D, R, B).with(&dlv)));
    }
    AV_CHECK(colsum(st, w.dmu, B, R, R, G + h->oBmu, nullptr));
    AV_CHECK(colsum(st, w.dlv, B, R, R, G + h->oBlv, nullptr));
    AV_TRY(gemm(h, nt(w.dmu, R, P + h->oWmu, R, w.dhpick, 2 * D, B, 2 * D, R)));
    AV_TRY(gemm(h, nt(w.dlv, R, P + h->oWlv, R, w.dhpick, 2 * D, B, 2 * D, R).plus()));
    fire_hook(h, 1 + L);
    const int32_t* const cdyn = w.compact ? w.nsrc : nullptr;
    const int32_t* const cmap = w.compact ? w.map_src : nullptr;
    if (w.compact) {
        AV_CHECK(zero_rows_dyn(st, w.dhs[0], w.nsrc, rs, 2 * D));
        AV_CHECK(pick_last_add(st, w.dhs[0], w.dhpick, w.lens_src, B, 2 * D, cmap));
    } else
    AV_CHECK(pick_last_bwd(st, w.dhs[0], w.dhpick, w.lens_src, Ss, B, 2 * D));

    cur = 0;
    for (int i = L - 1; i >= 0; --i) {
        const GruP& p = h->enc[i];
        const int In = i == 0 ? D : 2 * D;
        const bool top1 = i == L - 1 && top_one_step(h);
        const int64_t oWb = p.W + (int64_t)3 * D * In;
        if (top1) {
            AV_CHECK(gru_first_step_bwd(st, w.dhpick + D, 2 * D, w.svb, w.dgib, w.dghb, B, D, w.lens_src));
            AV_CHECK(colsum(st, w.dgib, B, 3 * D, 3 * D, G + p.bW + 3 * D, nullptr));
            AV_CHECK(colsum(st, w.dghb, B, 3 * D, 3 * D, G + p.bR + 3 * D, nullptr));
        }
        GruArgs a{};
        gru_common(h, w, a, top1 ? 1 : 2, Ss, B, 6 * D, 2 * D, w.lens_src, w.bx_enc());
        for (int d = 0; d < a.njobs; ++d) {
            GruJob& j = a.job[d];
            j.R = P + p.R + (int64_t)d * 3 * D * D; j.sv = w.e_sv[d][i]; j.hp = w.e_hp[d][i]; j.reverse = d;
            j.dh_out = w.dhs[cur] + d * D; j.dgi = w.dgi_e + d * 3 * D; j.dgh = w.dgh_e + d * 3 * D;
            j.dh0 = nullptr; j.carry = w.carry + (size_t)d * w.Bx * D;
            j.dbW = G + p.bW + d * 3 * D; j.dbR = G + p.bR + d * 3 * D;
        }
        const bool team16 = tn16_ok(h, 3 * D, D) && a.bf16 && gru_plan(a, false, h->persistent != 0).full();
        const bool g16 = team16 && !(i == 0 && use_table(h, rs, B));
        const bool gh16 = !g16 && w.dgh16_e && team16 && w.acth_e[i];
        if (g16) for (int d = 0; d < a.njobs; ++d) { a.job[d].dgi16 = w.dgi16_e + d * 3 * D; a.job[d].dgh16 = w.dgh16_e + d * 3 * D; }
        if (gh16) for (int d = 0; d < a.njobs; ++d) a.job[d].dgh16 = w.dgh16_e + d * 3 * D;
        if (!g16 && !gh16 && w.acth_e[i]) return fail(h, "internal: the forward kept this layer's h_prev as bf16 only and the backward cannot read it");
        if (w.acth_e[i]) for (int d = 0; d < a.njobs; ++d) a.job[d].hp16 = w.e_hp16[d][i];
        attach_sv16(h, a, true);
        attach_order(h, w, a, false, top1 ? 1 : 0);
        a.rowmap = cmap;
        if (cmap && i == 0) for (int d = 0; d < a.njobs; ++d) a.job[d].dgi_by_pos = 1;
        a.bwd_rs = rs_pick(h); a.spec = spec_pick(h);
        hook_fence(h);
        { Timed t(h, 2, 2.0 * a.njobs * (Ss - 1) * (double)B * D * 3 * D);
          DeviceTurn turn(h);
          AV_GRU(gru_backward(st, a, h->persistent != 0)); }
        hook_flush(h);
        const bool table = i == 0 && use_table(h, rs, B);
        const float* x = i == 0 ? w.emb_src : w.e_hs[i - 1];
        float* dx = i == 0 ? w.demb_src : w.dhs[cur ^ 1];
        if (g16) {
            const int Gc = a.njobs * 3 * D;
            if (i == 0) {
                AV_TRY(gemm_bf16_pre(h, nn(nullptr, 6 * D, P + p.W, In, dx, In, rs, In, Gc).a16(w.dgi16_e)));
                AV_CHECK(embed_scatter_add2(st, G + h->oE, w.src_tm, w.demb_src, rs, w.lead, w.demb_tgt, use_table(h, rt, B) ? 0 : rt, D, V, w.scat));
                fire_hook(h, 2 + 2 * L);
                hook_flush(h);
            }
            AV_TRY(gemm_tn16(h, tn_grad(nullptr, 6 * D, x, In, G + p.W, In, Gc, In, rs).a16(w.dgi16_e).b16((i > 0 && w.act_e[i - 1]) ? w.e_hs16[i - 1] : w.x16_kept_e(i)).depth(cdyn)));
            if (top1) AV_TRY(gemm(h, tn_grad(w.dgib, 3 * D, w.xlast, In, G + oWb, In, 3 * D, In, B)));
            for (int d = 0; d < a.njobs; ++d)
                AV_TRY(gemm_tn16(h, tn_grad(nullptr, 6 * D, w.e_hp[d][i], D, G + p.R + (int64_t)d * 3 * D * D, D, 3 * D, D, rs).a16(w.dgh16_e + d * 3 * D).b16(w.acth_e[i] ? w.e_hp16[d][i] : nullptr).depth(cdyn)));
            if (i > 0) AV_TRY(gemm_bf16_pre(h, nn(nullptr, 6 * D, P + p.W, In, dx, In, rs, In, Gc).a16(w.dgi16_e).rows(cdyn)));
            if (top1) {
                AV_TRY(gemm(h, nn(w.dgib, 3 * D, P + oWb, In, w.dxl, In, B, In, 3 * D).atomic()));
                AV_CHECK(pick_last_add(st, dx, w.dxl, w.lens_src, B, In, cmap));
            }
            cur ^= 1;
            fire_hook(h, 2 + L + (L - 1 - i));
            continue;
        }
        if (i == 0) {
            if (table) {
                const int32_t* cnt = id_groups_count(w.grp_src, rs, V); const int U = std::min(V, rs);
                AV_CHECK(rows_group_sum(st, w.dew, w.src_tm, w.dgi_e, rs, 6 * D, V, w.grp_src));
                AV_TRY(gemm(h, nn(w.dew, 6 * D, P + p.W, D, w.demb_src, D, U, D, 6 * D).rows(cnt).atomic()));
                AV_CHECK(rows_add_indexed(st, G + h->oE, w.demb_src, id_groups_uid(w.grp_src, rs, V), cnt, U, D));
            } else
            AV_TRY(gemm(h, nn(w.dgi_e, 6 * D, P + p.W, In, dx, In, rs, In, 6 * D).atomic()));
            AV_CHECK(embed_scatter_add2(st, G + h->oE, w.src_tm, w.demb_src, table ? 0 : rs, w.lead, w.demb_tgt, use_table(h, rt, B) ? 0 : rt, D, V, w.scat));
            fire_hook(h, 2 + 2 * L);
            hook_flush(h);
            if (table) {
                const int32_t* cnt = id_groups_count(w.grp_src, rs, V); const int U = std::min(V, rs);
                AV_TRY(gemm(h, tn_grad(w.dew, 6 * D, w.emb_src, D, G + p.W, D, 6 * D, D, U).depth(cnt)));
            } else
            AV_TRY(gemm(h, tn_grad(w.dgi_e, 6 * D, x, In, G + p.W, In, 6 * D, In, rs)));
        } else if (top1) {
            AV_TRY(gemm(h, tn_grad(w.dgi_e, 6 * D, x, In, G + p.W, In, 3 * D, In, rs).depth(cdyn)));
            AV_TRY(gemm(h, tn_grad(w.dgib, 3 * D, w.xlast, In, G + oWb, In, 3 * D, In, B)));
        } else
        AV_TRY(gemm(h, tn_grad(w.dgi_e, 6 * D, x, In, G + p.W, In, 6 * D, In, rs).depth(cdyn)));
        if (gh16) {
            for (int d = 0; d < a.njobs; ++d)
                AV_TRY(gemm_tn16(h, tn_grad(nullptr, 6 * D, nullptr, D, G + p.R + (int64_t)d * 3 * D * D, D, 3 * D, D, rs).a16(w.dgh16_e + d * 3 * D).b16(w.e_hp16[d][i]).depth(cdyn)));
        } else if (top1) AV_TRY(gemm(h, tn_grad(w.dgh_e, 6 * D, w.e_hp[0][i], D, G + p.R, D, 3 * D, D, rs).depth(cdyn)));
        else {
            const Pair bwd{w.dgh_e + 3 * D, w.e_hp[1][i], G + p.R + (int64_t)3 * D * D, nullptr};
            AV_TRY(gemm(h, tn_grad(w.dgh_e, 6 * D, w.e_hp[0][i], D, G + p.R, D, 3 * D, D, rs).depth(cdyn).with(&bwd)));
        }
        if (i > 0)
        AV_TRY(gemm(h, nn(w.dgi_e, 6 * D, P + p.W, In, dx, In, rs, In, top1 ? 3 * D : 6 * D).rows(cdyn).atomic()));
        if (top1) {
            AV_TRY(gemm(h, nn(w.dgib, 3 * D, P + oWb, In, w.dxl, In, B, In, 3 * D).atomic()));
            AV_CHECK(pick_last_add(st, dx, w.dxl, w.lens_src, B, In, cmap));
        }
        cur ^= 1;
        fire_hook(h, 2 + L + (L - 1 - i));
    }
    hook_flush(h);
    return 0;
}

int encode_ws(avae_ctx* h, Ws& w, const int32_t* src, int b, int t)
{
    PrepArgs p = prep_from_ws(w);
    p.src = src; p.tgt = src; p.B = b; p.Ss = t; p.St = 1; p.eos = h->cfg.eos; p.bos = h->cfg.bos;
    AV_CHECK(prep_ids(h->stream, p));
    AV_TRY(build_row_orders(h, w, b, t, 2, false));
    AV_TRY(build_compact(h, w, b, t, 0, false));
    AV_TRY(run_encoder(h, w, b, t, false));
    AV_TRY(run_latent(h, w, b, false, 0, nullptr));
    return 0;
}

}}

using namespace avae::host;

extern "C" {

int avae_get_schedule(avae_handle h, float out[3])
{
    if (!h || !out) return 1;
    Sched s = schedule(h); out[0] = s.keepwd; out[1] = s.anneal; out[2] = s.lr;
    return 0;
}

int avae_forward_backward(avae_handle h, const int32_t* src, const int32_t* tgt, int32_t B, int32_t Ss, int32_t St,
                          uint64_t seed, const uint8_t* keep_mask, const float* eps, float n_tok_global, float b_global)
{
    if (!h) return 1;
    AV_TRY(check_bound(h));
    if (B < 1 || Ss < 1 || St < 1) return fail(h, "empty batch");
    AV_CHECK(hipSetDevice(h->device));
    Ws w;
    AV_TRY(get_ws(h, w, B, Ss, St, true));
    h->B = B; h->Ss = Ss; h->St = St;
    AV_TRY(forward(h, w, src, tgt, B, Ss, St, true, seed, keep_mask, eps, n_tok_global > 0.f ? 1.f / n_tok_global : 0.f));
    AV_TRY(backward(h, w, B, Ss, St, b_global));
    if (h->persistent && !h->first_step_checked) {
        h->first_step_checked = true;
        AV_TRY(check_gru_err(h));
    }
    return 0;
}

int avae_adam_step(avae_handle h)
{
    if (!h) return 1;
    AV_TRY(check_bound(h));
    Sched sc = schedule(h);
    const double b1 = 0.9, b2 = 0.999;
    double t = (double)h->step + 1.0;
    AdamArgs a{h->P, h->G, h->M, h->Vv, h->numel, (float)(sc.lr * std::sqrt(1.0 - std::pow(b2, t)) / (1.0 - std::pow(b1, t))), 0.9f, 0.999f, 1e-8f, h->errw};
    AV_CHECK(adam_tf(h->stream, a));
    h->step += 1;
    return 0;
}

int avae_train_step(avae_handle h, const int32_t* src, const int32_t* tgt, int32_t B, int32_t Ss, int32_t St,
                    uint64_t seed, const uint8_t* keep_mask, const float* eps)
{
    AV_TRY(avae_forward_backward(h, src, tgt, B, Ss, St, seed, keep_mask, eps, 0.f, 0.f));
    return avae_adam_step(h);
}

int avae_get_losses(avae_handle h, float out[3])
{
    if (!h || !out) return 1;
    AV_CHECK(hipMemcpyAsync(out, h->losses, 3 * sizeof(float), hipMemcpyDeviceToHost, h->stream));
    AV_TRY(check_gru_err(h));
    return 0;
}

int avae_eval(avae_handle h, const int32_t* src, const int32_t* tgt, int32_t B, int32_t Ss, int32_t St,
              float* errt_samp, float* loss_gen_samp, float* loss_kld_samp, int32_t* n_out)
{
    if (!h) return 1;
    AV_TRY(check_bound(h));
    if (B < 1 || Ss < 1 || St < 1) return fail(h, "empty batch");
    AV_CHECK(hipSetDevice(h->device));
    Ws w;
    AV_TRY(get_ws(h, w, B, Ss, St, false));
    AV_TRY(forward(h, w, src, tgt, B, Ss, St, false, 0, nullptr, nullptr, 0.f));
    const size_t rt = (size_t)(St + 1) * B;
    if (errt_samp) AV_CHECK(hipMemcpyAsync(errt_samp, w.errt_samp, rt * sizeof(float), hipMemcpyDeviceToDevice, h->stream));
    if (loss_gen_samp) AV_CHECK(hipMemcpyAsync(loss_gen_samp, w.loss_samp, rt * sizeof(float), hipMemcpyDeviceToDevice, h->stream));
    if (loss_kld_samp) AV_CHECK(hipMemcpyAsync(loss_kld_samp, w.kld, (size_t)B * h->cfg.dim_rep * sizeof(float), hipMemcpyDeviceToDevice, h->stream));
    int n = 0;
    AV_CHECK(hipMemcpyAsync(&n, w.ntok, sizeof(int), hipMemcpyDeviceToHost, h->stream));
    AV_TRY(check_gru_err(h));
    if (n_out) *n_out = n;
    return 0;
}

int avae_encode(avae_handle h, const int32_t* src, int32_t b, int32_t t, float* z_out, float* lv_out)
{
    if (!h) return 1;
    AV_TRY(check_bound(h));
    if (b < 1 || t < 1) return fail(h, "empty batch");
    AV_CHECK(hipSetDevice(h->device));
    Ws w;
    AV_TRY(get_ws(h, w, b, t, 1, false));
    AV_TRY(encode_ws(h, w, src, b, t));
    const size_t n = (size_t)b * h->cfg.dim_rep * sizeof(float);
    if (z_out) AV_CHECK(hipMemcpyAsync(z_out, w.mu, n, hipMemcpyDeviceToDevice, h->stream));
    if (lv_out) AV_CHECK(hipMemcpyAsync(lv_out, w.lv, n, hipMemcpyDeviceToDevice, h->stream));
    return check_gru_err(h);
}

}
```

### argsim_amd/lib.py

```python
import ctypes as C
import os
import subprocess

_HERE = os.path.dirname(os.path.abspath(__file__))
LIB_PATH = os.path.join(_HERE, 'libargsim_vae.so')
CSRC = os.path.join(_HERE, 'csrc')


def source_digest():
    import glob
    import hashlib
    h = hashlib.sha1()
    files = sorted(glob.glob(os.path.join(CSRC, '*.hip')) + glob.glob(os.path.join(CSRC, '*.cpp')) + glob.glob(os.path.join(CSRC, '*.h')))
    files.append(os.path.join(os.path.dirname(_HERE), 'include', 'argsim_vae.h'))
    for f in files:
        h.update(os.path.basename(f).encode())
        with open(f, 'rb') as fh:
            h.update(fh.read())
    return h.hexdigest()[:16]


class AvaeConfig(C.Structure):
    _fields_ = [('dim_tgt', C.c_int32), ('dim_emb', C.c_int32), ('dim_rep', C.c_int32), ('rnn_layers', C.c_int32),
                ('accelerate', C.c_float), ('learn_rate', C.c_float), ('bos', C.c_int32), ('eos', C.c_int32),
                ('max_batch', C.c_int32), ('max_len', C.c_int32), ('kl_beta', C.c_float), ('free_bits', C.c_float),
                ('compute_dtype', C.c_int32)]


GRAD_HOOK = C.CFUNCTYPE(None, C.c_void_p, C.c_int, C.c_int64, C.c_int64)

class AvaeSampleConfig(C.Structure):
    _fields_ = [('temperature', C.c_float), ('top_k', C.c_int32), ('seed', C.c_uint64)]


class AvaeSamplePConfig(C.Structure):
    _fields_ = [('temperature', C.c_float), ('top_k', C.c_int32), ('seed', C.c_uint64), ('top_p', C.c_float), ('reserved', C.c_int32)]


class AvaeBeamConfig(C.Structure):
    _fields_ = [('width', C.c_int32), ('length_alpha', C.c_float)]


class AvaeScoreConfig(C.Structure):
    _fields_ = [('k', C.c_int32), ('seed', C.c_uint64)]


class AvaeKnnConfig(C.Structure):
    _fields_ = [('k', C.c_int32), ('metric', C.c_int32), ('idx_base', C.c_int64), ('self_base', C.c_int64), ('carry', C.c_int32),
                ('reserved', C.c_int32)]


class AvaeAggConfig(C.Structure):
    _fields_ = [('self_base', C.c_int64), ('reserved', C.c_int32 * 2)]


class AvaeProbeConfig(C.Structure):
    _fields_ = [('max_newton', C.c_int32), ('max_cg', C.c_int32), ('tol', C.c_float), ('reserved', C.c_int32)]


class AvaeProbeL1Config(C.Structure):
    _fields_ = [('max_newton', C.c_int32), ('max_inner', C.c_int32), ('tol', C.c_float), ('reserved', C.c_int32)]


class AvaeWardConfig(C.Structure):
    _fields_ = [('reserved', C.c_int32 * 2)]


class AvaeAffinityConfig(C.Structure):
    _fields_ = [('metric', C.c_int32), ('max_iter', C.c_int32), ('convergence_iter', C.c_int32), ('use_preference', C.c_int32),
                ('noise', C.c_int32), ('warm', C.c_int32), ('damping', C.c_float), ('preference', C.c_float), ('seed', C.c_uint64),
                ('reserved', C.c_int32 * 2)]


class AvaeTsneConfig(C.Structure):
    _fields_ = [('perplexity', C.c_double), ('early_exaggeration', C.c_double), ('min_grad_norm', C.c_double), ('learning_rate', C.c_float),
                ('max_iter', C.c_int32), ('it0', C.c_int32), ('exaggeration_iter', C.c_int32), ('n_iter_check', C.c_int32),
                ('n_iter_without_progress', C.c_int32), ('init', C.c_int32), ('warm', C.c_int32), ('seed', C.c_uint64),
                ('reserved', C.c_int32 * 2)]


class AvaeKmeansConfig(C.Structure):
    _fields_ = [('k', C.c_int32), ('n_init', C.c_int32), ('max_iter', C.c_int32), ('metric', C.c_int32), ('init', C.c_int32),
                ('reserved', C.c_int32), ('tol', C.c_double), ('seed', C.c_uint64)]


_P = C.c_void_p
SIGNATURES = {
    'avae_create': (C.c_int, [C.POINTER(AvaeConfig), C.c_int, C.POINTER(_P)]),
    'avae_destroy': (None, [_P]),
    'avae_last_error': (C.c_char_p, [_P]),
    'avae_set_stream': (C.c_int, [_P, _P]),
    'avae_get_dims': (C.c_int, [_P] + [C.POINTER(C.c_int32)] * 4),
    'avae_state_numel': (C.c_int64, [_P]),
    'avae_bind_state': (C.c_int, [_P, _P, _P, _P, _P]),
    'avae_param_count': (C.c_int, [_P]),
    'avae_param_name': (C.c_char_p, [_P, C.c_int]),
    'avae_param_info': (C.c_int, [_P, C.c_char_p, C.POINTER(C.c_int64), C.POINTER(C.c_int32), C.POINTER(C.c_int64)]),
    'avae_get_tensor': (C.c_int, [_P, C.c_char_p, C.c_int, _P]),
    'avae_set_tensor': (C.c_int, [_P, C.c_char_p, C.c_int, _P]),
    'avae_get_step': (C.c_int, [_P, C.POINTER(C.c_int64)]),
    'avae_set_step': (C.c_int, [_P, C.c_int64]),
    'avae_get_schedule': (C.c_int, [_P, C.POINTER(C.c_float)]),
    'avae_forward_backward': (C.c_int, [_P, _P, _P, C.c_int32, C.c_int32, C.c_int32, C.c_uint64, _P, _P, C.c_float, C.c_float]),
    'avae_adam_step': (C.c_int, [_P]),
    'avae_train_step': (C.c_int, [_P, _P, _P, C.c_int32, C.c_int32, C.c_int32, C.c_uint64, _P, _P]),
    'avae_get_losses': (C.c_int, [_P, C.POINTER(C.c_float)]),
    'avae_set_grad_hook': (C.c_int, [_P, GRAD_HOOK, _P]),
    'avae_eval': (C.c_int, [_P, _P, _P, C.c_int32, C.c_int32, C.c_int32, _P, _P, _P, C.POINTER(C.c_int32)]),
    'avae_encode': (C.c_int, [_P, _P, C.c_int32, C.c_int32, _P, _P]),
    'avae_decode_init': (C.c_int, [_P, _P, C.c_int32, _P]),
    'avae_decode_step': (C.c_int, [_P, _P, _P, C.c_int32, _P, _P]),
    'avae_decode_greedy': (C.c_int, [_P, _P, C.c_int32, C.c_int32, _P, C.POINTER(C.c_int32)]),
    'avae_decode_sample': (C.c_int, [_P, _P, C.c_int32, C.c_int32, C.POINTER(AvaeSampleConfig), _P, _P, C.POINTER(C.c_int32)]),
    'avae_decode_sample_p': (C.c_int, [_P, _P, C.c_int32, C.c_int32, C.POINTER(AvaeSamplePConfig), _P, _P, _P, C.POINTER(C.c_int32)]),
    'avae_decode_beam': (C.c_int, [_P, _P, C.c_int32, C.c_int32, C.POINTER(AvaeBeamConfig), _P, _P, _P, _P, _P, _P, _P, C.POINTER(C.c_int32)]),
    'avae_score': (C.c_int, [_P, _P, _P, C.c_int32, C.c_int32, C.c_int32, C.POINTER(AvaeScoreConfig), _P, _P, _P, _P, _P, _P]),
    'avae_score_z': (C.c_int, [_P, _P, _P, C.c_int32, C.c_int32, _P, _P]),
    'avae_knn': (C.c_int, [_P, _P, C.c_int32, _P, C.c_int32, C.c_int32, C.POINTER(AvaeKnnConfig), _P, _P]),
    'avae_agg_logq': (C.c_int, [_P, _P, C.c_int32, _P, _P, C.c_int32, C.c_int32, C.POINTER(AvaeAggConfig), _P, _P]),
    'avae_latent_moments': (C.c_int, [_P, _P, _P, C.c_int32, C.c_int32, _P]),
    'avae_probe_fit': (C.c_int, [_P, _P, C.c_int32, C.c_int32, _P, C.c_int32, C.POINTER(AvaeProbeConfig), _P, _P]),
    'avae_probe_decision': (C.c_int, [_P, _P, C.c_int32, C.c_int32, _P, C.c_int32, _P]),
    'avae_probe_fit_l1': (C.c_int, [_P, _P, C.c_int32, C.c_int32, _P, C.c_int32, C.POINTER(AvaeProbeL1Config), _P, _P]),
    'avae_ward': (C.c_int, [_P, _P, C.c_int32, C.POINTER(C.c_int32), C.c_int32, C.POINTER(AvaeWardConfig), _P, _P, _P]),
    'avae_ward_cut': (C.c_int, [_P, _P, C.POINTER(C.c_int32), C.c_int32, C.POINTER(C.c_int32), _P]),
    'avae_affinity': (C.c_int, [_P, _P, C.c_int32, C.c_int32, C.POINTER(AvaeAffinityConfig), _P, _P, _P, _P, _P]),
    'avae_tsne': (C.c_int, [_P, _P, C.c_int32, C.c_int32, C.POINTER(AvaeTsneConfig)] + [_P] * 10),
    'avae_kmeans': (C.c_int, [_P, _P, C.c_int32, C.c_int32, C.POINTER(AvaeKmeansConfig)] + [_P] * 8),
    'avae_set_option': (C.c_int, [_P, C.c_char_p, C.c_int]),
    'avae_debug_gemm': (C.c_int, [_P, C.c_int, C.c_int, _P, _P, _P, _P] + [C.c_int] * 6 + [C.c_float, C.c_int, C.c_int]),
    'avae_debug_gemm_dyn': (C.c_int, [_P, _P, _P, _P, C.c_int, C.c_int, C.c_int, _P]),
    'avae_debug_gemm_c16': (C.c_int, [_P, _P, _P, _P, C.c_int, C.c_int, C.c_int, C.c_float, _P]),
    'avae_debug_gemm_tn16': (C.c_int, [_P, _P, _P, _P] + [C.c_int] * 6 + [C.c_float]),
    'avae_debug_softmax_ce': (C.c_int, [_P, _P, _P, C.c_int, _P, _P, _P, C.c_int, C.c_int, C.c_int, C.c_float, _P, _P, _P, C.POINTER(C.c_int)]),
    'avae_debug_argmax_rows': (C.c_int, [_P, _P, _P, C.c_int, C.c_int]),
    'avae_debug_op': (C.c_int, [_P, C.c_char_p, C.POINTER(_P), C.POINTER(C.c_int64), C.POINTER(C.c_float)]),
    'avae_debug_op_layout': (C.c_int, [C.c_int64, C.c_int64, C.POINTER(C.c_int64)]),
    'avae_debug_sample_rows': (C.c_int, [_P, _P, C.c_int, C.c_int, C.c_int, C.POINTER(AvaeSampleConfig), _P, _P]),
    'avae_debug_sample_rows_p': (C.c_int, [_P, _P, C.c_int, C.c_int, C.c_int, C.POINTER(AvaeSamplePConfig), _P, _P, _P, _P]),
    'avae_debug_beam_select': (C.c_int, [_P, _P, C.c_int, C.c_int, C.c_int, _P, _P, _P, _P, _P, _P]),
    'avae_timing_collect': (C.c_int, [_P, C.POINTER(C.c_double)]),
    'avae_debug_timing': (C.c_int, [_P, C.POINTER(C.c_double), C.c_int, C.POINTER(C.c_int)]),
    'avae_debug_train_ce': (C.c_int, [_P, _P, C.c_int32, C.POINTER(C.c_int32)]),
    'avae_debug_stamps': (C.c_int, [_P, C.POINTER(C.c_uint64)]),
    'avae_debug_present_ids': (C.c_int, [_P, C.POINTER(C.c_int32)]),
    'avae_debug_score_plan': (C.c_int, [_P, C.POINTER(C.c_int32)]),
    'avae_debug_team_batch': (C.c_int, [C.c_int32]),
    'avae_debug_gemm_plan': (C.c_int, [_P, C.c_int32, _P]),
    'avae_debug_gemm_call': (C.c_int, [_P, C.c_int, C.c_int, _P, _P, _P, _P] + [C.c_int] * 6 + [C.c_float, C.c_int, C.c_int, _P, C.c_int, _P, _P, _P, _P]),
    'avae_debug_gemm_forced': (C.c_int, [_P, C.c_int, C.c_int, _P, _P, _P, _P] + [C.c_int] * 6 + [C.c_float, C.c_int, C.c_int, C.c_int, _P, C.c_int, C.c_int,
                                         _P, _P, _P, _P]),
    'avae_debug_gemm_f32_form': (C.c_int, [C.c_int] * 14 + [C.POINTER(C.c_int32)]),
    'avae_debug_gru_plan': (C.c_int, [C.POINTER(C.c_int64), C.c_int, C.c_int, C.POINTER(C.c_int64)]),
    'avae_debug_gru': (C.c_int, [_P, C.c_int, C.c_int, C.POINTER(C.c_int64), C.POINTER(_P), C.POINTER(_P), C.POINTER(C.c_int64)]),
    'avae_bucket_count': (C.c_int, [_P]),
    'avae_bucket_info': (C.c_int, [_P, C.c_int, C.POINTER(C.c_int64), C.POINTER(C.c_int64)]),
}

_lib = None


def build(force=False, jobs=4):
    if force:
        subprocess.run(['make', '-C', CSRC, 'clean'], check=True, stdout=subprocess.DEVNULL)
    subprocess.run(['make', '-C', CSRC, '-j%d' % jobs], check=True, stdout=subprocess.DEVNULL)
    return LIB_PATH


def load():
    global _lib
    if _lib is not None:
        return _lib
    if not os.path.exists(LIB_PATH):
        raise RuntimeError("libargsim_vae.so is not built: run `python -c 'import __graft_entry__ as g; g.build()'` "
                           "(there is no CPU fallback for the HIP path)")
    lib = C.CDLL(LIB_PATH)
    for name, (res, args) in SIGNATURES.items():
        fn = getattr(lib, name)
        fn.restype = res
        fn.argtypes = args
    _lib = lib
    return lib
```

Measured before the change: 16000 sentences/sec.

## Group independent backward GEMMs into a single multi-problem f32 kernel launch

```diff
diff --git a/argsim_amd/csrc/ctx.h b/argsim_amd/csrc/ctx.h
--- a/argsim_amd/csrc/ctx.h
+++ b/argsim_amd/csrc/ctx.h
@@ -52,6 +52,8 @@
     int compact = 2;
     int skip_pad = 1;
     int shared_device = 0; int lock_fd = -1;
+    int gemm_group = 1;
+    int gemm_group_stages = 0x7f;
     int dyn_split = 1;
     int dyn_thin = 1;
     int enc_top1 = 1;
@@ -87,7 +89,8 @@
     unsigned short *bfA = nullptr, *bfB = nullptr; size_t bfA_cap = 0, bfB_cap = 0;
     float* slab = nullptr; size_t slab_floats = 0;
     unsigned short* bfP = nullptr; size_t bfP_cap = 0;
-    struct Stamp { hipEvent_t a, b; int cls; double flops; const int* dyn; int dyn_max; };
+    struct StampPart { double flops; const int* dyn; int dyn_max; };
+    struct Stamp { hipEvent_t a, b; int cls; double flops; const int* dyn; int dyn_max; StampPart part[avae::kGemmGroupMax]; };
     std::vector<Stamp> stamps; size_t stamps_used = 0;
     int32_t* hint_dev = nullptr; volatile int32_t* hint_host = nullptr;
     const int32_t *cnt_src = nullptr, *cnt_tgt = nullptr;
@@ -144,6 +147,7 @@
         }
         s = &h->stamps[h->stamps_used++];
         s->cls = cls; s->flops = flops; s->dyn = dyn; s->dyn_max = dyn_max;
+        for (avae_ctx::StampPart& p : s->part) p = avae_ctx::StampPart{0.0, nullptr, 0};
         (void)hipEventRecord(s->a, h->stream);
     }
     ~Timed() { if (s) (void)hipEventRecord(s->b, h->stream); }
@@ -245,6 +249,8 @@
 }
 int get_ws(avae_ctx* h, Ws& w, int B, int Ss, int St, bool train);
 int gemm(avae_ctx* h, const GemmCall& c);
+int gemm_group(avae_ctx* h, const GemmCall* calls, int n, int* grouped = nullptr);
+int gemm_group(avae_ctx* h, std::initializer_list<GemmCall> calls);
 int gemm_tn16(avae_ctx* h, const GemmCall& c);
 void gru_geometry(int D, int njobs, int B, int* G, int* rpg);
 void gru_common(avae_ctx* h, const Ws& w, GruArgs& a, int njobs, int S, int B, int ldg, int ldh, const int32_t* lens, int Bx);
@@ -264,7 +270,7 @@
 
 int grow_scratch(avae_ctx* h, size_t need, const char* what);
 int check_gru_err(avae_ctx* h);
-int dyn_fraction(avae_ctx* h, const avae_ctx::Stamp& s, std::vector<std::pair<const int*, int>>& seen, double* f);
+int stamp_flops(avae_ctx* h, const avae_ctx::Stamp& s, std::vector<std::pair<const int*, int>>& seen, double* flops);
 inline int check_bound(avae_ctx* h)
 {
     if (!h->P || !h->G || !h->M || !h->Vv) return fail(h, "state buffers not bound (avae_bind_state)");
diff --git a/argsim_amd/csrc/gemm_f32.hip b/argsim_amd/csrc/gemm_f32.hip
--- a/argsim_amd/csrc/gemm_f32.hip
+++ b/argsim_amd/csrc/gemm_f32.hip
@@ -74,12 +74,11 @@
                              atomic ? kEpiAtomic : (g.accumulate ? kEpiAccumulate : kEpiStore));
 }
 
-template <bool A_MC, bool B_NC, int WM, int WN, int TM, int TN, bool FAST = false, bool DB = false>
-__global__ __launch_bounds__(256, DB ? 2 : 3) void gemm_f32_kernel(GemmArgs g)
+template <bool A_MC, bool B_NC, int WM, int WN, int TM, int TN, bool FAST, bool DB>
+__device__ __forceinline__ void gemm_f32_tile(GemmArgs g, const unsigned bx, const unsigned by, const unsigned bz, float* const smem)
 {
     constexpr int BM = 32 * WM * TM, BN = 32 * WN * TN;
     constexpr int kStage = (BM + BN) * LDK;
-    __shared__ __attribute__((aligned(16))) float smem[kStage * (DB ? 2 : 1)];
     float* As = smem;
     float* Bs = smem + BM * LDK;
 
@@ -87,14 +86,14 @@
     const int h = lane >> 5, l31 = lane & 31;
     const int wm = wave / WN, wn = wave % WN;
 
-    if (blockIdx.y) { g.A = g.A2; g.B = g.B2; g.C = g.C2; g.bias = g.bias2; }
+    if (by) { g.A = g.A2; g.B = g.B2; g.C = g.C2; g.bias = g.bias2; }
     int M = g.M, K = g.K;
     if (g.dyn_kind == 1) M = min(M, *g.dyn);
     if (g.dyn_kind == 2) K = min(K, *g.dyn);
 
     const int tiles_n = (g.N + BN - 1) / BN;
     const int nblk = ((M + BM - 1) / BM) * tiles_n;
-    const int bid = xcd_tile(blockIdx.x, nblk);
+    const int bid = xcd_tile(bx, nblk);
     if (bid < 0) return;
     const int tm = bid / tiles_n, tn = bid - tm * tiles_n;
     const int m0 = tm * BM, n0 = tn * BN;
@@ -104,7 +103,7 @@
     if (g.split_k > 1) {
         int ktiles = (K + BK - 1) / BK;
         int per = (ktiles + g.split_k - 1) / g.split_k;
-        kb = blockIdx.z * per * BK;
+        kb = bz * per * BK;
         ke = min(K, kb + per * BK);
         if (kb >= ke) return;
     }
@@ -188,8 +187,46 @@
     }
 
     const bool atomic = g.split_k > 1;
-    const bool add_bias = g.bias != nullptr && (!atomic || blockIdx.z == 0);
+    const bool add_bias = g.bias != nullptr && (!atomic || bz == 0);
     epilogue<TM, TN, WN>(g, acc, M, m0, n0, BM, BN, wm, wn, h, l31, atomic, add_bias);
+}
+
+template <bool A_MC, bool B_NC, int WM, int WN, int TM, int TN, bool FAST = false, bool DB = false>
+__global__ __launch_bounds__(256, DB ? 2 : 3) void gemm_f32_kernel(GemmArgs g)
+{
+    __shared__ __attribute__((aligned(16))) float smem[32 * (WM * TM + WN * TN) * LDK * (DB ? 2 : 1)];
+    gemm_f32_tile<A_MC, B_NC, WM, WN, TM, TN, FAST, DB>(g, blockIdx.x, blockIdx.y, blockIdx.z, smem);
+}
+
+template <bool BIG>
+__global__ __launch_bounds__(256, 3) void gemm_f32_group_kernel(GemmGroup grp)
+{
+    extern __shared__ __attribute__((aligned(16))) float gsmem[];
+    const int w = blockIdx.x;
+    int m = 0;
+#pragma unroll
+    for (int i = 1; i < kGemmGroupMax; ++i) if (i < grp.n && w >= grp.first[i]) m = i;
+    const unsigned local = w - grp.first[m];
+    if (local >= (unsigned)grp.count[m]) return;
+    const unsigned gx = grp.gx[m], gy = grp.gy[m];
+    const unsigned bx = local % gx, rest = local / gx, by = rest % gy, bz = rest / gy;
+    const GemmArgs& g = grp.m[m];
+    if (BIG) {
+        switch (grp.form[m]) {
+        case kGfNN128:  gemm_f32_tile<false, true, 2, 2, 2, 2, true, false>(g, bx, by, bz, gsmem); break;
+        case kGfTN128:  gemm_f32_tile<true, true, 2, 2, 2, 2, true, false>(g, bx, by, bz, gsmem); break;
+        case kGfNT128p: gemm_f32_tile<false, false, 2, 2, 2, 2, false, false>(g, bx, by, bz, gsmem); break;
+        default: break;
+        }
+    } else {
+        switch (grp.form[m]) {
+        case kGfTN64:   gemm_f32_tile<true, true, 2, 2, 1, 1, true, false>(g, bx, by, bz, gsmem); break;
+        case kGfNN64:   gemm_f32_tile<false, true, 2, 2, 1, 1, true, false>(g, bx, by, bz, gsmem); break;
+        case kGfTN32:   gemm_f32_tile<true, true, 1, 4, 1, 1, true, false>(g, bx, by, bz, gsmem); break;
+        case kGfNN32:   gemm_f32_tile<false, true, 1, 4, 1, 1, true, false>(g, bx, by, bz, gsmem); break;
+        default: break;
+        }
+    }
 }
 
 template <bool A_MC, bool B_NC, bool FAST>
@@ -400,6 +437,46 @@
     with_layouts(a_mc, b_nc, [&](auto A, auto B) { hipLaunchKernelGGL((gemm_f32_kernel<decltype(A)::value, decltype(B)::value, WM, WN, TM, TN>), grid, dim3(256), 0, st, g); });
 }
 
+int gemm_f32_group_form(bool a_mc, bool b_nc, const GemmArgs& g)
+{
+    const GemmF32Form f = gemm_f32_form(a_mc, b_nc, g);
+    if (f.err != hipSuccess || f.tile < 0 || f.tile > 2 || f.persist || f.db) return -1;
+    if (!a_mc && !b_nc) return f.tile == 0 && !f.fast ? kGfNT128p : -1;
+    if (!b_nc || !f.fast) return -1;
+    if (f.tile == 0) return a_mc ? kGfTN128 : kGfNN128;
+    if (f.tile == 2) return a_mc ? kGfTN64 : kGfNN64;
+    return a_mc ? kGfTN32 : kGfNN32;
+}
+
+hipError_t gemm_f32_group(hipStream_t st, const bool* a_mc, const bool* b_nc, const GemmArgs* g, int n)
+{
+    if (n < 1 || n > kGemmGroupMax) return hipErrorInvalidValue;
+    int order[kGemmGroupMax];
+    for (int i = 0; i < n; ++i) order[i] = i;
+    auto work = [&](int i) { return (double)g[i].M * g[i].N * g[i].K * (g[i].A2 ? 2 : 1); };
+    std::stable_sort(order, order + n, [&](int a, int b) { return work(a) > work(b); });
+    GemmGroup grp{};
+    const bool big = gemm_group_form_big(gemm_f32_group_form(a_mc[0], b_nc[0], g[0]));
+    size_t lds = 0;
+    int next = 0;
+    for (int o = 0; o < n; ++o) {
+        const int i = order[o];
+        const int form = gemm_f32_group_form(a_mc[i], b_nc[i], g[i]);
+        if (form < 0 || gemm_group_form_big(form) != big) return hipErrorInvalidValue;
+        const GemmF32Form f = gemm_f32_form(a_mc[i], b_nc[i], g[i]);
+        const int k = grp.n++;
+        grp.m[k] = g[i]; grp.form[k] = form; grp.gx[k] = (int)f.gx; grp.gy[k] = (int)f.gy;
+        grp.count[k] = (int)(f.gx * f.gy * f.gz);
+        grp.first[k] = next;
+        next = (next + grp.count[k] + 7) & ~7;
+        lds = std::max(lds, sizeof(float) * LDK * (size_t)(f.tile == 0 ? 256 : (f.tile == 2 ? 128 : 160)));
+    }
+    for (int k = grp.n; k <= kGemmGroupMax; ++k) grp.first[k] = next;
+    if (big) hipLaunchKernelGGL(gemm_f32_group_kernel<true>, dim3(next), dim3(256), lds, st, grp);
+    else     hipLaunchKernelGGL(gemm_f32_group_kernel<false>, dim3(next), dim3(256), lds, st, grp);
+    return hipGetLastError();
+}
+
 hipError_t gemm_f32(hipStream_t st, bool a_mc, bool b_nc, const GemmArgs& g)
 {
     const GemmF32Form f = gemm_f32_form(a_mc, b_nc, g);
diff --git a/argsim_amd/csrc/handle.cpp b/argsim_amd/csrc/handle.cpp
--- a/argsim_amd/csrc/handle.cpp
+++ b/argsim_amd/csrc/handle.cpp
@@ -106,18 +106,30 @@
     }
     return 0;
 }
-int dyn_fraction(avae_ctx* h, const avae_ctx::Stamp& s, std::vector<std::pair<const int*, int>>& seen, double* f)
+static int dyn_fraction(avae_ctx* h, const int* dyn, int dyn_max, std::vector<std::pair<const int*, int>>& seen, double* f)
 {
     *f = 1.0;
-    if (!s.dyn || s.dyn_max <= 0) return 0;
+    if (!dyn || dyn_max <= 0) return 0;
     int c = -1;
-    for (auto& e : seen) if (e.first == s.dyn) c = e.second;
+    for (auto& e : seen) if (e.first == dyn) c = e.second;
     if (c < 0) {
-        AV_CHECK(hipMemcpy(&c, s.dyn, sizeof(int), hipMemcpyDeviceToHost));
+        AV_CHECK(hipMemcpy(&c, dyn, sizeof(int), hipMemcpyDeviceToHost));
         if (c < 0) c = 0;
-        seen.push_back({s.dyn, c});
-    }
-    *f = (double)std::min(c, s.dyn_max) / (double)s.dyn_max;
+        seen.push_back({dyn, c});
+    }
+    *f = (double)std::min(c, dyn_max) / (double)dyn_max;
+    return 0;
+}
+int stamp_flops(avae_ctx* h, const avae_ctx::Stamp& s, std::vector<std::pair<const int*, int>>& seen, double* flops)
+{
+    double f = 1.0;
+    AV_TRY(dyn_fraction(h, s.dyn, s.dyn_max, seen, &f));
+    *flops = s.flops * f;
+    for (const avae_ctx::StampPart& p : s.part) {
+        if (p.flops == 0.0) continue;
+        AV_TRY(dyn_fraction(h, p.dyn, p.dyn_max, seen, &f));
+        *flops += p.flops * f;
+    }
     return 0;
 }
 
@@ -242,6 +254,8 @@
     if (!strcmp(key, "gru_bf16")) { h->gru_bf16 = value != 0; return 0; }
     if (!strcmp(key, "bwd_rs")) { h->bwd_rs = value; return 0; }
     if (!strcmp(key, "dyn_split")) { h->dyn_split = value != 0; return 0; }
+    if (!strcmp(key, "gemm_group")) { h->gemm_group = value != 0; return 0; }
+    if (!strcmp(key, "gemm_group_stages")) { h->gemm_group_stages = value; return 0; }
     if (!strcmp(key, "shared_device")) { h->shared_device = value != 0; return 0; }
     if (!strcmp(key, "gru_spec")) { h->gru_spec = value; return 0; }
     if (!strcmp(key, "gru_ring")) { h->gru_ring = value != 0; return 0; }
@@ -280,10 +294,10 @@
     for (size_t i = 0; i < h->stamps_used; ++i) {
         float ms = 0.f;
         AV_CHECK(hipEventElapsedTime(&ms, h->stamps[i].a, h->stamps[i].b));
-        double f = 1.0;
-        AV_TRY(dyn_fraction(h, h->stamps[i], seen, &f));
+        double fl = 0.0;
+        AV_TRY(stamp_flops(h, h->stamps[i], seen, &fl));
         int c = h->stamps[i].cls;
-        out[3 * c] += ms; out[3 * c + 1] += 1.0; out[3 * c + 2] += h->stamps[i].flops * f;
+        out[3 * c] += ms; out[3 * c + 1] += 1.0; out[3 * c + 2] += fl;
     }
     h->stamps_used = 0;
     return 0;
diff --git a/argsim_amd/csrc/hooks.cpp b/argsim_amd/csrc/hooks.cpp
--- a/argsim_amd/csrc/hooks.cpp
+++ b/argsim_amd/csrc/hooks.cpp
@@ -58,6 +58,32 @@
     h->expect_ptr[0] = was_ptr; h->expect_val[0] = was_val;
     return r;
 }
+int avae_debug_gemm_group(avae_handle h, int n, const int32_t* desc, const void* const* ptrs, const float* alpha, int32_t* grouped_out)
+{
+    if (!h) return 1;
+    if (n < 1 || n > kGemmGroupMax || !desc || !ptrs || !alpha) return fail(h, "avae_debug_gemm_group: 1..6 products, with their descriptors, pointers and scales");
+    GemmCall calls[kGemmGroupMax]; Pair second[kGemmGroupMax];
+    const int* was_ptr[3]; int was_val[3];
+    for (int i = 0; i < 3; ++i) { was_ptr[i] = h->expect_ptr[i]; was_val[i] = h->expect_val[i]; h->expect_ptr[i] = nullptr; h->expect_val[i] = 0; }
+    int slots = 0, grouped[2] = {0, 0};
+    for (int i = 0; i < n; ++i, desc += 13, ptrs += 7) {
+        GemmCall c{static_cast<const float*>(ptrs[0]), desc[5], desc[0] != 0, static_cast<const float*>(ptrs[1]), desc[6], desc[1] != 0,
+                   static_cast<float*>(const_cast<void*>(ptrs[2])), desc[7], desc[2], desc[3], desc[4]};
+        c.alpha = alpha[i]; c.accumulate = desc[8];
+        c.allow_atomic = (desc[9] & 1) != 0; c.wgrad = (desc[9] & 4) != 0;
+        const int* count = static_cast<const int*>(ptrs[3]);
+        if (c.wgrad || (c.a_mc && c.b_nc)) c.depth(count); else c.rows(count);
+        if (desc[10] >= 0) c.form(desc[10], desc[11]);
+        second[i] = Pair{static_cast<const float*>(ptrs[4]), static_cast<const float*>(ptrs[5]), static_cast<float*>(const_cast<void*>(ptrs[6])), nullptr};
+        if (second[i].A) c.pair = &second[i];
+        if (count && desc[12] > 0 && slots < 3) { h->expect_ptr[slots] = count; h->expect_val[slots] = desc[12]; ++slots; }
+        calls[i] = c;
+    }
+    const int r = gemm_group(h, calls, n, grouped);
+    if (grouped_out) { grouped_out[0] = grouped[0]; grouped_out[1] = grouped[1]; }
+    for (int i = 0; i < 3; ++i) { h->expect_ptr[i] = was_ptr[i]; h->expect_val[i] = was_val[i]; }
+    return r;
+}
 int avae_debug_gemm_f32_form(int a_mc, int b_nc, int M, int N, int K, int lda, int ldb, int ldc, int accumulate, int thin, int split_k, int dyn_kind,
                              int expect, int pair, int32_t out[8])
 {
@@ -108,9 +134,8 @@
     for (int i = 0; i < *n; ++i) {
         float ms = 0.f;
         AV_CHECK(hipEventElapsedTime(&ms, h->stamps[i].a, h->stamps[i].b));
-        double f = 1.0;
-        AV_TRY(dyn_fraction(h, h->stamps[i], seen, &f));
-        const double fl = h->stamps[i].flops * f;
+        double fl = 0.0;
+        AV_TRY(stamp_flops(h, h->stamps[i], seen, &fl));
         out[3 * i] = h->stamps[i].cls; out[3 * i + 1] = ms; out[3 * i + 2] = fl;
     }
     return 0;
diff --git a/argsim_amd/csrc/kernels.h b/argsim_amd/csrc/kernels.h
--- a/argsim_amd/csrc/kernels.h
+++ b/argsim_amd/csrc/kernels.h
@@ -23,6 +23,17 @@
 hipError_t gemm_f32(hipStream_t st, bool a_mc, bool b_nc, const GemmArgs& g);
 struct GemmF32Form { int tile; bool fast, db, persist; unsigned gx, gy, gz; hipError_t err; };
 GemmF32Form gemm_f32_form(bool a_mc, bool b_nc, const GemmArgs& g);
+constexpr int kGemmGroupMax = 6;
+struct GemmGroup {
+    GemmArgs m[kGemmGroupMax];
+    int form[kGemmGroupMax], gx[kGemmGroupMax], gy[kGemmGroupMax], count[kGemmGroupMax];
+    int first[kGemmGroupMax + 1];
+    int n;
+};
+enum GemmGroupForm { kGfNN128 = 0, kGfTN128, kGfNT128p, kGfTN64, kGfNN64, kGfTN32, kGfNN32, kGfCount };
+inline bool gemm_group_form_big(int form) { return form <= kGfNT128p; }
+int gemm_f32_group_form(bool a_mc, bool b_nc, const GemmArgs& g);
+hipError_t gemm_f32_group(hipStream_t st, const bool* a_mc, const bool* b_nc, const GemmArgs* g, int n);
 hipError_t gemm_f32s(hipStream_t st, bool a_mc, bool b_nc, const GemmArgs& g);
 hipError_t gemm_bf16_direct(hipStream_t st, bool a_mc, bool b_nc, const GemmArgs& g);
 
diff --git a/argsim_amd/csrc/model.cpp b/argsim_amd/csrc/model.cpp
--- a/argsim_amd/csrc/model.cpp
+++ b/argsim_amd/csrc/model.cpp
@@ -145,6 +145,15 @@
     return gemm_plan(s).launch[0];
 }
 
+static GemmArgs gemm_args(const avae_ctx* h, const GemmCall& c, const GemmLaunch& l)
+{
+    const float* A = c.A + (size_t)l.row0 * c.lda; float* C = c.C + (size_t)l.row0 * c.ldc;
+    const int* dyn = l.dyn ? c.dyn : nullptr; const int dyn_kind = l.dyn ? c.dyn_kind : 0;
+    const Pair* pair = c.pair;
+    return GemmArgs{A, c.B, C, c.bias, l.rows, c.N, c.K, c.lda, c.ldb, c.ldc, c.alpha, l.accumulate, l.split_k, dyn, dyn_kind, dyn_expected(h, dyn, dyn_kind), l.thin,
+                    pair ? pair->A : nullptr, pair ? pair->B : nullptr, pair ? pair->C : nullptr, pair ? pair->bias : nullptr};
+}
+
 static int gemm_launch(avae_ctx* h, const GemmCall& c, const GemmLaunch& l)
 {
     if (c.pair && h->cfg.compute_dtype != 0) {
@@ -154,13 +163,11 @@
         AV_TRY(gemm_launch(h, one, l));
         return gemm_launch(h, two, l);
     }
-    const float* A = c.A + (size_t)l.row0 * c.lda; float* C = c.C + (size_t)l.row0 * c.ldc;
-    const int M = l.rows, N = c.N, K = c.K;
-    const int* dyn = l.dyn ? c.dyn : nullptr; const int dyn_kind = l.dyn ? c.dyn_kind : 0;
-    const Pair* pair = c.pair;
-    GemmArgs g{A, c.B, C, c.bias, M, N, K, c.lda, c.ldb, c.ldc, c.alpha, l.accumulate, l.split_k, dyn, dyn_kind, dyn_expected(h, dyn, dyn_kind), l.thin,
-               pair ? pair->A : nullptr, pair ? pair->B : nullptr, pair ? pair->C : nullptr, pair ? pair->bias : nullptr};
-    Timed t(h, 0, 2.0 * M * N * K * (pair ? 2 : 1), dyn, dyn_kind == 1 ? M : (dyn_kind == 2 ? K : 0));
+    GemmArgs g = gemm_args(h, c, l);
+    const float* A = g.A;
+    const int M = g.M, N = g.N, K = g.K;
+    const int* dyn = g.dyn; const int dyn_kind = g.dyn_kind;
+    Timed t(h, 0, 2.0 * M * N * K * (c.pair ? 2 : 1), dyn, dyn_kind == 1 ? M : (dyn_kind == 2 ? K : 0));
     if (h->cfg.compute_dtype == 1 && h->bf16_direct) {
         AV_CHECK(gemm_bf16_direct(h->stream, c.a_mc, c.b_nc, g));
         return 0;
@@ -184,16 +191,61 @@
     return 0;
 }
 
+static int gemm_clear(avae_ctx* h, const GemmCall& c, const GemmLaunch& l)
+{
+    float* C = c.C + (size_t)l.row0 * c.ldc;
+    if (l.zero == kZeroAll) AV_CHECK(zero_fill(h->stream, C, sizeof(float) * (size_t)l.rows * c.N));
+    if (l.zero == kZeroDynRows) AV_CHECK(zero_rows_dyn(h->stream, C, c.dyn, l.rows, c.N));
+    return 0;
+}
+
 int gemm(avae_ctx* h, const GemmCall& c)
 {
     const GemmPlan p = gemm_plan(gemm_shape(h, c));
     for (int i = 0; i < p.n; ++i) {
-        const GemmLaunch& l = p.launch[i];
-        float* C = c.C + (size_t)l.row0 * c.ldc;
-        if (l.zero == kZeroAll) AV_CHECK(zero_fill(h->stream, C, sizeof(float) * (size_t)l.rows * c.N));
-        if (l.zero == kZeroDynRows) AV_CHECK(zero_rows_dyn(h->stream, C, c.dyn, l.rows, c.N));
-        AV_TRY(gemm_launch(h, c, l));
-    }
+        AV_TRY(gemm_clear(h, c, p.launch[i]));
+        AV_TRY(gemm_launch(h, c, p.launch[i]));
+    }
+    return 0;
+}
+
+int gemm_group(avae_ctx* h, std::initializer_list<GemmCall> calls) { return gemm_group(h, calls.begin(), (int)calls.size()); }
+int gemm_group(avae_ctx* h, const GemmCall* calls, int n, int* grouped)
+{
+    if (grouped) grouped[0] = grouped[1] = 0;
+    struct Planned { const GemmCall* c; GemmLaunch l; GemmArgs g; int cls; };
+    std::vector<Planned> all;
+    int members[2] = {0, 0};
+    if (h->gemm_group && h->cfg.compute_dtype == 0)
+        for (int i = 0; i < n; ++i) {
+            const GemmCall& c = calls[i];
+            if (c.c16) return fail(h, "the fp16 output panel exists in compute_dtype 1 only");
+            const GemmPlan p = gemm_plan(gemm_shape(h, c));
+            for (int k = 0; k < p.n; ++k) {
+                const GemmArgs g = gemm_args(h, c, p.launch[k]);
+                const int form = gemm_f32_group_form(c.a_mc, c.b_nc, g);
+                all.push_back(Planned{&calls[i], p.launch[k], g, form < 0 ? -1 : (gemm_group_form_big(form) ? 0 : 1)});
+                if (form >= 0) ++members[all.back().cls];
+            }
+        }
+    for (Planned& q : all) if (q.cls >= 0 && (members[q.cls] < 2 || members[q.cls] > kGemmGroupMax)) q.cls = -1;
+    if (all.empty() || (members[0] < 2 && members[1] < 2)) {
+        for (int i = 0; i < n; ++i) AV_TRY(gemm(h, calls[i]));
+        return 0;
+    }
+    if (grouped) for (int cls = 0; cls < 2; ++cls) grouped[cls] = members[cls] >= 2 && members[cls] <= kGemmGroupMax ? members[cls] : 0;
+    for (const Planned& q : all) AV_TRY(gemm_clear(h, *q.c, q.l));
+    for (int cls = 0; cls < 2; ++cls) {
+        bool a_mc[kGemmGroupMax], b_nc[kGemmGroupMax]; GemmArgs g[kGemmGroupMax];
+        int k = 0;
+        for (const Planned& q : all) if (q.cls == cls) { a_mc[k] = q.c->a_mc; b_nc[k] = q.c->b_nc; g[k] = q.g; ++k; }
+        if (!k) continue;
+        Timed t(h, 0, 0.0);
+        for (int i = 0; i < k && t.s; ++i)
+            t.s->part[i] = avae_ctx::StampPart{2.0 * g[i].M * g[i].N * g[i].K * (g[i].A2 ? 2 : 1), g[i].dyn, g[i].dyn_kind == 1 ? g[i].M : (g[i].dyn_kind == 2 ? g[i].K : 0)};
+        AV_CHECK(gemm_f32_group(h->stream, a_mc, b_nc, g, k));
+    }
+    for (const Planned& q : all) if (q.cls < 0) AV_TRY(gemm_launch(h, *q.c, q.l));
     return 0;
 }
 
@@ -592,6 +644,15 @@
     h->hook_pending.clear();
 }
 
+enum GemmStage { kStageLogits = 0, kStageOut, kStageDec, kStageDecTable, kStageEncTop, kStageEnc, kStageEncFirst };
+static int stage(avae_ctx* h, int id, const GemmCall* calls, int n)
+{
+    if ((h->gemm_group_stages >> id) & 1) return gemm_group(h, calls, n);
+    for (int i = 0; i < n; ++i) AV_TRY(gemm(h, calls[i]));
+    return 0;
+}
+static int stage(avae_ctx* h, int id, std::initializer_list<GemmCall> calls) { return stage(h, id, calls.begin(), (int)calls.size()); }
+
 static int backward(avae_ctx* h, Ws& w, int B, int Ss, int St, float b_global)
 {
     const int D = h->cfg.dim_emb, V = h->cfg.dim_tgt, R = h->cfg.dim_rep, L = h->cfg.rnn_layers;
@@ -608,12 +669,12 @@
         const GemmCall dE = tn_grad(nullptr, V, w.ho, D, G + h->oE, D, V, D, rt).a16(h->bfP).scaled(isd).depth(w.ntok);
         AV_TRY(tn16_ok(h, V, D) ? gemm_tn16(h, dE) : gemm_bf16_pre(h, dE));
     } else {
-    AV_TRY(gemm(h, nn(w.logits, V, P + h->oE, D, w.dho, D, rt, D, V).scaled(isd).rows(w.ntok).atomic()));
+    AV_TRY(stage(h, kStageLogits, {nn(w.logits, V, P + h->oE, D, w.dho, D, rt, D, V).scaled(isd).rows(w.ntok).atomic()}));
     AV_TRY(gemm(h, tn_grad(w.logits, V, w.ho, D, G + h->oE, D, V, D, rt).scaled(isd).depth(w.ntok)));
     }
-    AV_TRY(gemm(h, tn_grad(w.hc, D, w.dho, D, G + h->oKout, D, D, D, rt).depth(w.ntok)));
     AV_CHECK(colsum(st, w.dho, rt, D, D, G + h->oBout, w.ntok));
-    AV_TRY(gemm(h, nt(w.dho, D, P + h->oKout, D, w.dhc, D, rt, D, D).rows(w.ntok).atomic()));
+    AV_TRY(stage(h, kStageOut, {tn_grad(w.hc, D, w.dho, D, G + h->oKout, D, D, D, rt).depth(w.ntok),
+                                nt(w.dho, D, P + h->oKout, D, w.dhc, D, rt, D, D).rows(w.ntok).atomic()}));
     fire_hook(h, 0);
     const int32_t* const ddyn = w.compact_d ? w.ntgt : nullptr;
     const int32_t* const dmap = w.compact_d ? w.map_tgt : nullptr;
@@ -649,11 +710,14 @@
         if (i == 0 && use_table(h, rt, B)) {
             const int32_t* cnt = id_groups_count(w.grp_tgt, rt, V); const int U = std::min(V, rt);
             AV_CHECK(rows_group_sum(st, w.dew, w.lead, w.dgi_d, rt, 3 * D, V, w.grp_tgt));
-            AV_TRY(gemm(h, tn_grad(w.dew, 3 * D, w.emb_tgt, D, G + p.W, D, 3 * D, D, U).depth(cnt)));
-            if (gh16) AV_TRY(gemm_tn16(h, tn_grad(nullptr, 3 * D, nullptr, D, G + p.R, D, 3 * D, D, rt).a16(w.dgh16_d).b16(w.d_hp16[i]).depth(ddyn)));
-            else
-            AV_TRY(gemm(h, tn_grad(w.dgh_d, 3 * D, w.d_hp[i], D, G + p.R, D, 3 * D, D, rt).depth(ddyn)));
-            AV_TRY(gemm(h, nn(w.dew, 3 * D, P + p.W, D, w.demb_tgt, D, U, D, 3 * D).rows(cnt).atomic()));
+            const GemmCall dW = tn_grad(w.dew, 3 * D, w.emb_tgt, D, G + p.W, D, 3 * D, D, U).depth(cnt);
+            const GemmCall dE = nn(w.dew, 3 * D, P + p.W, D, w.demb_tgt, D, U, D, 3 * D).rows(cnt).atomic();
+            if (gh16) {
+                AV_TRY(gemm(h, dW));
+                AV_TRY(gemm_tn16(h, tn_grad(nullptr, 3 * D, nullptr, D, G + p.R, D, 3 * D, D, rt).a16(w.dgh16_d).b16(w.d_hp16[i]).depth(ddyn)));
+                AV_TRY(gemm(h, dE));
+            } else
+            AV_TRY(stage(h, kStageDecTable, {dW, tn_grad(w.dgh_d, 3 * D, w.d_hp[i], D, G + p.R, D, 3 * D, D, rt).depth(ddyn), dE}));
             AV_CHECK(rows_add_indexed(st, G + h->oE, w.demb_tgt, id_groups_uid(w.grp_tgt, rt, V), cnt, U, D));
         } else if (g16) {
             const float* x = i == 0 ? w.emb_tgt : w.d_hd[i - 1];
@@ -663,12 +727,10 @@
             AV_TRY(gemm_bf16_pre(h, nn(nullptr, 3 * D, P + p.W, D, dx, D, rt, D, 3 * D).a16(w.dgi16_d).rows(ddyn)));
         } else {
         const float* x = i == 0 ? w.emb_tgt : w.d_hd[i - 1];
-        {
-            const Pair dR{w.dgh_d, w.d_hp[i], G + p.R, nullptr};
-            AV_TRY(gemm(h, tn_grad(w.dgi_d, 3 * D, x, D, G + p.W, D, 3 * D, D, rt).depth(ddyn).with(&dR)));
-        }
+        const Pair dR{w.dgh_d, w.d_hp[i], G + p.R, nullptr};
         float* dx = i == 0 ? w.demb_tgt : w.dhd[cur ^ 1];
-        AV_TRY(gemm(h, nn(w.dgi_d, 3 * D, P + p.W, D, dx, D, rt, D, 3 * D).rows(ddyn).atomic()));
+        AV_TRY(stage(h, kStageDec, {tn_grad(w.dgi_d, 3 * D, x, D, G + p.W, D, 3 * D, D, rt).depth(ddyn).with(&dR),
+                                    nn(w.dgi_d, 3 * D, P + p.W, D, dx, D, rt, D, 3 * D).rows(ddyn).atomic()}));
         }
         cur ^= 1;
         fire_hook(h, 1 + (L - 1 - i));
@@ -770,30 +832,30 @@
             AV_CHECK(embed_scatter_add2(st, G + h->oE, w.src_tm, w.demb_src, table ? 0 : rs, w.lead, w.demb_tgt, use_table(h, rt, B) ? 0 : rt, D, V, w.scat));
             fire_hook(h, 2 + 2 * L);
             hook_flush(h);
+        }
+        GemmCall prod[kGemmGroupMax]; int np = 0;
+        if (i == 0) {
             if (table) {
                 const int32_t* cnt = id_groups_count(w.grp_src, rs, V); const int U = std::min(V, rs);
-                AV_TRY(gemm(h, tn_grad(w.dew, 6 * D, w.emb_src, D, G + p.W, D, 6 * D, D, U).depth(cnt)));
+                prod[np++] = tn_grad(w.dew, 6 * D, w.emb_src, D, G + p.W, D, 6 * D, D, U).depth(cnt);
             } else
-            AV_TRY(gemm(h, tn_grad(w.dgi_e, 6 * D, x, In, G + p.W, In, 6 * D, In, rs)));
+            prod[np++] = tn_grad(w.dgi_e, 6 * D, x, In, G + p.W, In, 6 * D, In, rs);
         } else if (top1) {
-            AV_TRY(gemm(h, tn_grad(w.dgi_e, 6 * D, x, In, G + p.W, In, 3 * D, In, rs).depth(cdyn)));
-            AV_TRY(gemm(h, tn_grad(w.dgib, 3 * D, w.xlast, In, G + oWb, In, 3 * D, In, B)));
+            prod[np++] = tn_grad(w.dgi_e, 6 * D, x, In, G + p.W, In, 3 * D, In, rs).depth(cdyn);
+            prod[np++] = tn_grad(w.dgib, 3 * D, w.xlast, In, G + oWb, In, 3 * D, In, B);
         } else
-        AV_TRY(gemm(h, tn_grad(w.dgi_e, 6 * D, x, In, G + p.W, In, 6 * D, In, rs).depth(cdyn)));
+        prod[np++] = tn_grad(w.dgi_e, 6 * D, x, In, G + p.W, In, 6 * D, In, rs).depth(cdyn);
+        const Pair bwd{w.dgh_e + 3 * D, w.e_hp[1][i], G + p.R + (int64_t)3 * D * D, nullptr};
         if (gh16) {
             for (int d = 0; d < a.njobs; ++d)
                 AV_TRY(gemm_tn16(h, tn_grad(nullptr, 6 * D, nullptr, D, G + p.R + (int64_t)d * 3 * D * D, D, 3 * D, D, rs).a16(w.dgh16_e + d * 3 * D).b16(w.e_hp16[d][i]).depth(cdyn)));
-        } else if (top1) AV_TRY(gemm(h, tn_grad(w.dgh_e, 6 * D, w.e_hp[0][i], D, G + p.R, D, 3 * D, D, rs).depth(cdyn)));
-        else {
-            const Pair bwd{w.dgh_e + 3 * D, w.e_hp[1][i], G + p.R + (int64_t)3 * D * D, nullptr};
-            AV_TRY(gemm(h, tn_grad(w.dgh_e, 6 * D, w.e_hp[0][i], D, G + p.R, D, 3 * D, D, rs).depth(cdyn).with(&bwd)));
-        }
+        } else if (top1) prod[np++] = tn_grad(w.dgh_e, 6 * D, w.e_hp[0][i], D, G + p.R, D, 3 * D, D, rs).depth(cdyn);
+        else prod[np++] = tn_grad(w.dgh_e, 6 * D, w.e_hp[0][i], D, G + p.R, D, 3 * D, D, rs).depth(cdyn).with(&bwd);
         if (i > 0)
-        AV_TRY(gemm(h, nn(w.dgi_e, 6 * D, P + p.W, In, dx, In, rs, In, top1 ? 3 * D : 6 * D).rows(cdyn).atomic()));
-        if (top1) {
-            AV_TRY(gemm(h, nn(w.dgib, 3 * D, P + oWb, In, w.dxl, In, B, In, 3 * D).atomic()));
-            AV_CHECK(pick_last_add(st, dx, w.dxl, w.lens_src, B, In, cmap));
-        }
+        prod[np++] = nn(w.dgi_e, 6 * D, P + p.W, In, dx, In, rs, In, top1 ? 3 * D : 6 * D).rows(cdyn).atomic();
+        if (top1) prod[np++] = nn(w.dgib, 3 * D, P + oWb, In, w.dxl, In, B, In, 3 * D).atomic();
+        AV_TRY(stage(h, i == 0 ? kStageEncFirst : (top1 ? kStageEncTop : kStageEnc), prod, np));
+        if (top1) AV_CHECK(pick_last_add(st, dx, w.dxl, w.lens_src, B, In, cmap));
         cur ^= 1;
         fire_hook(h, 2 + L + (L - 1 - i));
     }
diff --git a/argsim_amd/lib.py b/argsim_amd/lib.py
--- a/argsim_amd/lib.py
+++ b/argsim_amd/lib.py
@@ -147,6 +147,7 @@
     'avae_debug_score_plan': (C.c_int, [_P, C.POINTER(C.c_int32)]),
     'avae_debug_team_batch': (C.c_int, [C.c_int32]),
     'avae_debug_gemm_plan': (C.c_int, [_P, C.c_int32, _P]),
+    'avae_debug_gemm_group': (C.c_int, [_P, C.c_int, _P, _P, _P, _P]),
     'avae_debug_gemm_call': (C.c_int, [_P, C.c_int, C.c_int, _P, _P, _P, _P] + [C.c_int] * 6 + [C.c_float, C.c_int, C.c_int, _P, C.c_int, _P, _P, _P, _P]),
     'avae_debug_gemm_forced': (C.c_int, [_P, C.c_int, C.c_int, _P, _P, _P, _P] + [C.c_int] * 6 + [C.c_float, C.c_int, C.c_int, C.c_int, _P, C.c_int, C.c_int,
                                          _P, _P, _P, _P]),
```

Measured after the change: 16060 sentences/sec, median of 6. Within noise of the previous version (+0.4%).
